# AutonomousVehicleLaboratory/vision_semantic_segmentation

Hardware: AMD Instinct MI355X
Metric: fused frames/sec/GPU (1920x1080 + 120k pts) + max|dlog-odds| vs ref (higher is better)
Workload: dtype f16 hi+lo split, MX-FP4 correction passes, fp32 accumulate

## Files before the change

include/avl_hip.h:

```cpp
#ifndef AVL_HIP_H
#define AVL_HIP_H

#include <stdint.h>

#ifdef __cplusplus
extern "C" {
#endif

#define AVL_OK 0
#define AVL_E_ARG (-1)
#define AVL_E_HIP (-2)
#define AVL_E_UNSUPPORTED (-3)

#define AVL_F32 0
#define AVL_F64 1
#define AVL_BF16 2
#define AVL_F16 3

#define AVL_MAX_MAP_CLASSES 16

const char* avl_version(void);
int avl_last_error(char* buf, int len);


int avl_project_points(const void* pts, int n, int dtype, int64_t point_stride, int64_t comp_stride,
                       const double* P_host, const double* T_host, double range_max,
                       int img_w, int img_h, int32_t* out_ixy, uint8_t* out_mask, void* stream);

int64_t avl_project_pcd_scratch_bytes(int n);

int avl_project_pcd(const void* pts, int n, int dtype, int64_t point_stride, int64_t comp_stride,
                    const double* P_host, const double* T_host, double range_max,
                    const uint8_t* image, int img_w, int img_h,
                    double* out_pcd, uint8_t* out_label, int64_t out_ld, int32_t* out_count,
                    void* scratch, void* stream);


typedef struct avl_grid {
    void* map;
    int map_dtype;
    int Hm, Wm, C;
    double off_x, off_y;
    double b00, b10;
    double resolution;
    uint32_t* cell_mask;
    int32_t* touched;
    int32_t touched_cap;
    int32_t* counter;
    int32_t counter_len;
} avl_grid;
#define AVL_COUNTER_INTS 256

int avl_update_map(const avl_grid* g, const double* pcd, const uint8_t* label, int64_t ld,
                   int m_host, const int32_t* m_dev,
                   const uint8_t* label_colors_host, const double* cm_host, uint32_t bonus_classes,
                   void* stream);

int avl_vote_points(const avl_grid* g, const double* pcd, const uint8_t* label, int64_t ld,
                    int m_host, const int32_t* m_dev, const uint8_t* label_colors_host,
                    uint32_t bonus_classes, void* stream);
int avl_grid_apply(const avl_grid* g, const double* cm_host, void* rows, int rows_dtype, void* stream);


#define AVL_SRC_RGB 0
#define AVL_SRC_CLASSMAP 1

int avl_fused_frame(const avl_grid* g, const void* pts, int n, int dtype, int64_t point_stride,
                    int64_t comp_stride, const double* P_host, const double* T_host, double range_max,
                    int src_kind, const uint8_t* src, int src_w, int src_h, int img_w, int img_h,
                    const uint32_t* lut_host, const uint8_t* label_colors_host,
                    const double* cm_host, uint32_t bonus_classes, void* stream);

int avl_fused_frame_path(const avl_grid* g, int n, uint32_t bonus_classes);


#define AVL_MAX_VIEWS 4
int avl_fused_frame_views(const avl_grid* g, const void* pts, int n, int dtype, int64_t point_stride, int64_t comp_stride,
                          int n_views, const double* P_host , const double* T_host, double range_max,
                          int src_kind, const uint8_t* const* src_host ,
                          int src_w, int src_h, int img_w, int img_h,
                          const uint32_t* lut_host, const uint8_t* label_colors_host,
                          const double* cm_host, uint32_t bonus_classes, void* stream);

int avl_fused_frame_views_path(const avl_grid* g, int n, int n_views, uint32_t bonus_classes);

int avl_colorize_labels(const uint8_t* labels, int lw, int lh, const uint8_t* palette_host,
                        uint8_t* out, int out_w, int out_h, void* stream);


int avl_preprocess_image(const uint8_t* bgr, int h, int w, const double* K_host, const double* dist_host, int factor,
                         uint8_t* rgb_out, void* stream);
int avl_preprocess_image_area(const uint8_t* bgr, int h, int w, const double* K_host, const double* dist_host, int out_h, int out_w,
                              uint8_t* rgb_out, void* stream);

#define AVL_STEM_CAMERA_BYTES 64
int avl_stem_camera_set(void* camera_dev, const double* K_host, const double* dist_host, void* stream);

int avl_pack_semantic_cloud(const double* pcd, const uint8_t* label, int64_t ld, int m_host, const int32_t* m_dev,
                            void* out_records, void* stream);

int avl_planar_update(void* map, int map_dtype, int Hm, int Wm, int C, const uint8_t* image, int img_h, int img_w,
                      const double* Hinv_host, int sep, const uint8_t* label_colors_host, int match_colour, void* stream);

int avl_unpack_pointcloud2(const uint8_t* data, int64_t n_points, int point_step, int off_x, int off_y, int off_z, int off_i,
                           float* out_xyzi, int32_t* n_valid, void* stream);

int avl_render_bev_map(const void* map, int map_dtype, int Hm, int Wm, int C, const uint8_t* colors_host,
                       uint8_t* out, void* stream);
int avl_render_bev_map_thresholds(const void* map, int map_dtype, int Hm, int Wm, int C, const uint8_t* colors_host,
                                  const int32_t* priority_host, const double* thresholds_host, uint8_t* out, void* stream);
int avl_grid_box_filter(const void* src, void* dst, int map_dtype, int Hm, int Wm, int C, void* stream);
int avl_eval_map(const uint8_t* color_map, int H, int W, const uint8_t* mask, int mask_ld, const uint8_t* gt, int gt_ld,
                 uint8_t* labels_out, unsigned long long* counts, void* stream);

int avl_upsample_logits(const float* logits, int h, int w, int K, int64_t ld, float* out, int H, int W, void* stream);
int64_t avl_seg_eval_scratch_bytes(int H, int W);
int avl_seg_eval_full_res(const float* logits, int h, int w, int K, int64_t ld, int H, int W, const uint8_t* gt, int ignore_index,
                          uint8_t* labels_out, unsigned long long* confusion, double* loss_out, unsigned long long* counts_out,
                          void* scratch, void* stream);
int avl_upsample_logits_batch(const float* logits, int n, int64_t image_rows, int h, int w, int K, int64_t ld, float* out, int H, int W,
                              void* stream);
int64_t avl_seg_eval_scratch_bytes_batch(int n, int H, int W);
int avl_seg_eval_full_res_batch(const float* logits, int n, int64_t image_rows, int h, int w, int K, int64_t ld, int H, int W,
                                const uint8_t* gt, int ignore_index, uint8_t* labels_out, unsigned long long* confusion, double* loss_out,
                                unsigned long long* counts_out, double* image_loss_out, unsigned long long* image_counts_out,
                                void* scratch, void* stream);


#define AVL_OP_STEM 1
#define AVL_OP_MAXPOOL 2
#define AVL_OP_GEMM 3
#define AVL_OP_GCONV 4
#define AVL_OP_DWCONV 5
#define AVL_OP_BILINEAR 6
#define AVL_OP_GAP 7
#define AVL_OP_GEMV 8
#define AVL_OP_ARGMAX 9
#define AVL_OP_SUBSAMPLE 10
#define AVL_OP_DWPW 11

#define AVL_OP_BOTTLENECK 12

typedef struct avl_seg_op {
    int32_t kind;
    int32_t dtype;
    const void* in;
    const void* in2;
    void* out;
    const void* weight;
    const float* bias;
    int32_t in_h, in_w, in_c, in_ld, in_rows;
    int32_t out_h, out_w, out_c, out_ld, out_rows;
    int32_t in2_ld;
    int32_t ksize, stride, pad, dil, groups;
    int32_t relu;
    int32_t out_f32;
    int32_t w_rows;
    int32_t w_layout;
    int32_t w_split;
    int32_t mx_flags;
    const void* in_lo;
    const void* in2_lo;
    void* out_lo;
    const void* w_mx;
    const void* in_mx;
    void* out_mx;
    const void* in2_mx;
    const void* in3;
    const void* in3_mx;
    int32_t in3_c, in3_ld;
    int32_t batch;
    int32_t bias_per_image;
    int32_t in_format;
    int32_t raw_batch;
} avl_seg_op;

#define AVL_IN_U8_HWC 0
#define AVL_IN_F32_CHW 1

#define AVL_MX_IN_LO 1
#define AVL_MX_RES_LO 2
#define AVL_MX_OUT_LO 4

typedef struct avl_seg_plan avl_seg_plan;

int avl_seg_plan_create(const avl_seg_op* ops_host, int n_ops, avl_seg_plan** out_plan);
void avl_seg_plan_destroy(avl_seg_plan* plan);
int avl_seg_plan_run(avl_seg_plan* plan, void* stream);
int avl_seg_plan_capture(avl_seg_plan* plan, void* stream);
int avl_seg_plan_profile(avl_seg_plan* plan, void* stream, float* ms_host, double* flops_host, double* bytes_host);
int avl_seg_plan_num_ops(const avl_seg_plan* plan);
int avl_seg_plan_nonfinite(avl_seg_plan* plan, void* stream, unsigned long long* counts_host);

#ifdef __cplusplus
}
#endif
#endif
```

vision_semantic_segmentation_amd/csrc/seg_gemm.hip:

```cpp
#include <cstdlib>
#include <cstring>
#include <type_traits>

#include "seg_types.h"

namespace avl {
namespace {

struct GemmArgs {
    const void* A;
    const void* W;
    const float* bias;
    const void* R;
    void* C;
    int lda, ldr, ldc;
    int M, N, K;
    int relu, out_f32;
    int ntiles;
    int nsub;
    long long a_lo_delta;
    const void* R_lo;
    void* C_lo;
};

template <int NSUB> __device__ __forceinline__ bool sub_needs_a(int j) { return NSUB == 1 || j == 0 || (NSUB == 3 && j == 2); }

__device__ __forceinline__ void glds16(const void* g, void* l) {
    __builtin_amdgcn_global_load_lds((const __attribute__((address_space(1))) void*)g,
                                     (__attribute__((address_space(3))) void*)l, 16, 0, 0);
}

template <typename T, int WM, int WN>
__global__ void __launch_bounds__(WM* WN * 64) k_gemm(GemmArgs p) {
    constexpr int NW = WM * WN, BM = WM * 64, BN = WN * 64;
    constexpr int A_BYTES = BM * 128, W_BYTES = BN * 128, BUF = A_BYTES + W_BYTES;
    constexpr int A_INSTR = BM / 8 / NW, W_INSTR = BN / 8 / NW;
    static_assert(A_INSTR >= 1 && W_INSTR >= 1, "tile too small for the wave count");
    extern __shared__ __attribute__((aligned(16))) char lds[];

    const int tid = threadIdx.x, lane = tid & 63;
    const int wave = __builtin_amdgcn_readfirstlane(tid >> 6);
    const int wm = wave / WN, wn = wave % WN;

    int bid = blockIdx.x;
    {
        const int nwg = gridDim.x, xcd = bid & 7, local = bid >> 3, q = nwg >> 3, r = nwg & 7;
        bid = (xcd < r ? xcd * (q + 1) : r * (q + 1) + (xcd - r) * q) + local;
    }
    const int nt = bid % p.ntiles, mt = bid / p.ntiles;
    const int m0 = mt * BM, n0 = nt * BN;

    const char* a_src[A_INSTR];
    const char* w_src[W_INSTR];
#pragma unroll
    for (int i = 0; i < A_INSTR; ++i) {
        const int r = (i * NW + wave) * 8 + (lane >> 3);
        const int c = (lane & 7) ^ (r & 7);
        a_src[i] = static_cast<const char*>(p.A) + (long long)(m0 + r) * p.lda * (int)sizeof(T) + c * 16;
    }
#pragma unroll
    for (int i = 0; i < W_INSTR; ++i) {
        const int r = (i * NW + wave) * 8 + (lane >> 3);
        const int c = (lane & 7) ^ (r & 7);
        w_src[i] = static_cast<const char*>(p.W) + (long long)(n0 + r) * p.K * p.nsub * (int)sizeof(T) + c * 16;
    }
    auto stage = [&](int buf, int kt) {
        char* base = lds + buf * BUF;
        const int kb = kt / p.nsub, j = kt - kb * p.nsub;
        const long long aoff = (long long)kb * 128 + (j == 2 ? p.a_lo_delta : 0);
#pragma unroll
        for (int i = 0; i < A_INSTR; ++i) glds16(a_src[i] + aoff, base + (i * NW + wave) * 1024);
#pragma unroll
        for (int i = 0; i < W_INSTR; ++i) glds16(w_src[i] + (long long)kt * 128, base + A_BYTES + (i * NW + wave) * 1024);
    };

    const int fr = lane & 15, kq = lane >> 4;
    int a_row[4], w_row[4];
#pragma unroll
    for (int mi = 0; mi < 4; ++mi) a_row[mi] = wm * 64 + mi * 16 + fr;
#pragma unroll
    for (int nj = 0; nj < 4; ++nj) w_row[nj] = wn * 64 + (fr >> 2) * 16 + nj * 4 + (fr & 3);

    f32x4 acc[4][4];
#pragma unroll
    for (int mi = 0; mi < 4; ++mi)
#pragma unroll
        for (int nj = 0; nj < 4; ++nj) acc[mi][nj] = f32x4{0.f, 0.f, 0.f, 0.f};

    const int nk = p.K * (int)sizeof(T) / 128 * p.nsub;
    stage(0, 0);
    int cur = 0;
    for (int kt = 0; kt < nk; ++kt) {
        asm volatile("s_waitcnt vmcnt(0)" ::: "memory");
        __syncthreads();
        if (kt + 1 < nk) stage(cur ^ 1, kt + 1);
        const char* ab = lds + cur * BUF;
        const char* wb = ab + A_BYTES;
        if constexpr (sizeof(T) == 2) {
#pragma unroll
            for (int kk = 0; kk < 2; ++kk) {
                const int chunk = kk * 4 + kq;
                typedef typename Half16<T>::v8 v8;
                v8 af[4], wf[4];
#pragma unroll
                for (int mi = 0; mi < 4; ++mi)
                    af[mi] = *reinterpret_cast<const v8*>(ab + a_row[mi] * 128 + ((chunk ^ (a_row[mi] & 7)) << 4));
#pragma unroll
                for (int nj = 0; nj < 4; ++nj)
                    wf[nj] = *reinterpret_cast<const v8*>(wb + w_row[nj] * 128 + ((chunk ^ (w_row[nj] & 7)) << 4));
#pragma unroll
                for (int mi = 0; mi < 4; ++mi)
#pragma unroll
                    for (int nj = 0; nj < 4; ++nj) acc[mi][nj] = Half16<T>::mfma(wf[nj], af[mi], acc[mi][nj]);
            }
        } else {
            f32x4 af[4][2], wf[4][2];
#pragma unroll
            for (int h = 0; h < 2; ++h) {
                const int chunk = kq * 2 + h;
#pragma unroll
                for (int mi = 0; mi < 4; ++mi)
                    af[mi][h] = *reinterpret_cast<const f32x4*>(ab + a_row[mi] * 128 + ((chunk ^ (a_row[mi] & 7)) << 4));
#pragma unroll
                for (int nj = 0; nj < 4; ++nj)
                    wf[nj][h] = *reinterpret_cast<const f32x4*>(wb + w_row[nj] * 128 + ((chunk ^ (w_row[nj] & 7)) << 4));
            }
#pragma unroll
            for (int s = 0; s < 8; ++s)
#pragma unroll
                for (int mi = 0; mi < 4; ++mi)
#pragma unroll
                    for (int nj = 0; nj < 4; ++nj)
                        acc[mi][nj] = __builtin_amdgcn_mfma_f32_16x16x4f32(wf[nj][s >> 2][s & 3], af[mi][s >> 2][s & 3],
                                                                           acc[mi][nj], 0, 0, 0);
        }
        cur ^= 1;
    }

    const int nbase = n0 + wn * 64 + kq * 16;
    float bias[16];
#pragma unroll
    for (int j = 0; j < 4; ++j) {
        const float4 b = *reinterpret_cast<const float4*>(p.bias + nbase + 4 * j);
        bias[4 * j] = b.x; bias[4 * j + 1] = b.y; bias[4 * j + 2] = b.z; bias[4 * j + 3] = b.w;
    }
    unsigned char* const labels = p.out_f32 ? static_cast<unsigned char*>(p.C_lo) : nullptr;
    if (labels) {
#pragma unroll
        for (int mi = 0; mi < 4; ++mi) {
            const int m = m0 + wm * 64 + mi * 16 + fr;
            float best = acc[mi][0][0] + bias[0];
            int bi = nbase;
#pragma unroll
            for (int i = 1; i < 16; ++i) {
                const float val = acc[mi][i >> 2][i & 3] + bias[i];
                if (nbase + i < p.N && (val > best || (val != val && best == best))) { best = val; bi = nbase + i; }
            }
            const float ob = __shfl_down(best, 16);
            const int oi = __shfl_down(bi, 16);
            if (nbase + 16 < p.N && (ob > best || (ob != ob && best == best))) { best = ob; bi = oi; }
            if (kq == 0 && m < p.M) labels[m] = (unsigned char)bi;
        }
    }
#pragma unroll
    for (int mi = 0; mi < 4; ++mi) {
        const int m = m0 + wm * 64 + mi * 16 + fr;
        if (m >= p.M || nbase >= p.N) continue;
        float v[16];
#pragma unroll
        for (int nj = 0; nj < 4; ++nj)
#pragma unroll
            for (int r = 0; r < 4; ++r) v[nj * 4 + r] = acc[mi][nj][r] + bias[nj * 4 + r];
        const bool full = nbase + 16 <= p.N;
        if (p.R) {
            const T* rp = static_cast<const T*>(p.R) + (long long)m * p.ldr + nbase;
            if (full) {
                float r0[8], r1[8];
                Vec8<T>::load(rp, r0);
                Vec8<T>::load(rp + 8, r1);
#pragma unroll
                for (int i = 0; i < 8; ++i) { v[i] += r0[i]; v[8 + i] += r1[i]; }
            } else {
                for (int i = 0; i < 16; ++i)
                    if (nbase + i < p.N) v[i] += to_f32(rp[i]);
            }
        }
        if (p.relu) {
#pragma unroll
            for (int i = 0; i < 16; ++i) v[i] = fmaxf(v[i], 0.f);
        }
        if (p.out_f32) {
            float* cp = static_cast<float*>(p.C) + (long long)m * p.ldc + nbase;
            for (int i = 0; i < 16; ++i)
                if (nbase + i < p.N) cp[i] = v[i];
        }
        if (!p.out_f32) {
            T* cp = static_cast<T*>(p.C) + (long long)m * p.ldc + nbase;
            if (full) {
                float lo[8], hi[8];
#pragma unroll
                for (int i = 0; i < 8; ++i) { lo[i] = v[i]; hi[i] = v[8 + i]; }
                Vec8<T>::store(cp, lo);
                Vec8<T>::store(cp + 8, hi);
            } else {
                for (int i = 0; i < 16; ++i)
                    if (nbase + i < p.N) cp[i] = from_f32<T>(v[i]);
            }
        }
    }
}

template <typename H, int WM, int WN, int MI, int STAGES, int NSUB = 1, int IO = 0, int AST = STAGES>
__global__ void __launch_bounds__(WM* WN * 64) k_gemm_ring(GemmArgs p, int mtiles) {
    typedef typename Half16<H>::v8 v8;
    constexpr int NW = WM * WN, BM = WM * MI * 16, BN = WN * 64;
    constexpr int A_BYTES = BM * 128, W_BYTES = BN * 128;
    constexpr int W_REGION = AST * A_BYTES;
    static_assert(AST == STAGES || (NSUB == 2 && AST == 2), "activation ring too short for this pass pattern");
    constexpr int A_INSTR = BM / 8 / NW, W_INSTR = BN / 8 / NW;
    extern __shared__ __attribute__((aligned(16))) char lds[];

    const int tid = threadIdx.x, lane = tid & 63;
    const int wave = __builtin_amdgcn_readfirstlane(tid >> 6);
    const int wm = wave / WN, wn = wave % WN;
    const int nwg = gridDim.x;
    int vb;
    {
        const int bid = blockIdx.x, xcd = bid & 7, local = bid >> 3, q = nwg >> 3, r = nwg & 7;
        vb = (xcd < r ? xcd * (q + 1) : r * (q + 1) + (xcd - r) * q) + local;
    }
    const int total = mtiles * p.ntiles;
    const int nkb = p.K / 64;
    const unsigned lds_base = lds_addr(lds);

    const int srow = lane >> 3, schunk = lane & 7;
    const char* a_src[A_INSTR];
    const char* w_src[W_INSTR];
    int pt = vb, pk = 0;
    int issued = 0, issued_a = 0;
    auto set_tile = [&](int t) {
        const int nt = t % p.ntiles, mt = t / p.ntiles;
#pragma unroll
        for (int i = 0; i < A_INSTR; ++i) {
            const int r = (i * NW + wave) * 8 + srow;
            a_src[i] = static_cast<const char*>(p.A) + (long long)(mt * BM + r) * p.lda * 2 + ((schunk ^ (r & 7)) << 4);
        }
#pragma unroll
        for (int i = 0; i < W_INSTR; ++i) {
            const int r = (i * NW + wave) * 8 + srow;
            const int key = ((r >> 1) & 1) | (((r >> 4) & 3) << 1);
            w_src[i] = static_cast<const char*>(p.W) + (long long)(nt * BN + r) * p.K * (2 * NSUB) + ((schunk ^ key) << 4);
        }
    };
    auto issue_part = [&](int h, int np, int jj) {
        const bool na = sub_needs_a<NSUB>(jj);
        if (na) {
            const unsigned abase = lds_base + (issued_a % AST) * A_BYTES + wave * 1024;
            const long long aoff = (long long)pk * 128 + ((NSUB == 3 && jj == 2) ? p.a_lo_delta : 0);
#pragma unroll
            for (int i = 0; i < A_INSTR; ++i)
                if (i * np / A_INSTR == h) glds16_asm(a_src[i] + aoff, abase + i * NW * 1024);
        }
        const unsigned wbase = lds_base + W_REGION + (issued % STAGES) * W_BYTES + wave * 1024;
        const long long woff = (long long)(pk * NSUB + jj) * 128;
#pragma unroll
        for (int i = 0; i < W_INSTR; ++i)
            if (i * np / W_INSTR == h) glds16_asm(w_src[i] + woff, wbase + i * NW * 1024);
        if (h == np - 1) {
            ++issued;
            if (na) ++issued_a;
            if (jj == NSUB - 1) {
                if (++pk == nkb) {
                    pk = 0;
                    pt += nwg;
                    if (pt < total) set_tile(pt);
                }
            }
        }
    };
    if (pt < total) set_tile(pt);
#pragma unroll
    for (int i = 0; i < STAGES - 1; ++i)
        if (pt < total) issue_part(0, 1, i % NSUB);

    const int fr = lane & 15, kq = lane >> 4;
    int a_off[MI], w_off[4], a_key[MI], w_key[4];
#pragma unroll
    for (int mi = 0; mi < MI; ++mi) {
        const int row = wm * (MI * 16) + mi * 16 + fr;
        a_off[mi] = row * 128;
        a_key[mi] = row & 7;
    }
#pragma unroll
    for (int nj = 0; nj < 4; ++nj) {
        const int row = wn * 64 + (fr >> 2) * 16 + nj * 4 + (fr & 3);
        w_off[nj] = W_REGION + row * 128;
        w_key[nj] = ((row >> 1) & 1) | (((row >> 4) & 3) << 1);
    }
    f32x4 acc[MI][4];
    auto init_acc = [&](int t) {
        const int nb = (t % p.ntiles) * BN + wn * 64 + kq * 16;
#pragma unroll
        for (int nj = 0; nj < 4; ++nj) {
            const float4 b = *reinterpret_cast<const float4*>(p.bias + nb + 4 * nj);
#pragma unroll
            for (int mi = 0; mi < MI; ++mi) acc[mi][nj] = f32x4{b.x, b.y, b.z, b.w};
        }
    };
    if (vb < total) init_acc(vb);

    int g = 0;
    int ca = -1;
    for (int t = vb; t < total; t += nwg) {
        const int nt = t % p.ntiles, mt = t / p.ntiles;
        for (int q = 0, j = 0; q < nkb * NSUB; ++q, ++g, j = (NSUB == 1 || j + 1 == NSUB) ? 0 : j + 1) {
            if (sub_needs_a<NSUB>(j)) ++ca;
            const int jn = (j + STAGES - 1) % NSUB;
            if (STAGES >= 3 && issued > g + 1) {
                if (sub_needs_a<NSUB>((j + 1) % NSUB)) asm volatile("s_waitcnt vmcnt(%0)" ::"n"(A_INSTR + W_INSTR) : "memory");
                else asm volatile("s_waitcnt vmcnt(%0)" ::"n"(W_INSTR) : "memory");
            } else asm volatile("s_waitcnt vmcnt(0)" ::: "memory");
            __builtin_amdgcn_s_barrier();
            const bool feed = pt < total;
            const char* abase = lds + (ca % AST) * A_BYTES;
            const char* wbase = lds + (g % STAGES) * W_BYTES;
            auto rd_w = [&](int kk, int nj) { return *reinterpret_cast<const v8*>(wbase + w_off[nj] + (((kk * 4 + kq) ^ w_key[nj]) << 4)); };
            auto rd_a = [&](int kk, int mi) { return *reinterpret_cast<const v8*>(abase + a_off[mi] + (((kk * 4 + kq) ^ a_key[mi]) << 4)); };
            constexpr int HALF = MI / 2;
            const bool early = MI == 8 && NW >= 8 && wave >= NW / 2;
            if (feed && early) { issue_part(0, 2, jn); issue_part(1, 2, jn); }
            v8 wa[4], wb[4], af[MI];
#pragma unroll
            for (int nj = 0; nj < 4; ++nj) wa[nj] = rd_w(0, nj);
#pragma unroll
            for (int mi = 0; mi < MI; ++mi) af[mi] = rd_a(0, mi);
            __builtin_amdgcn_sched_barrier(0);
#pragma unroll
            for (int mi = 0; mi < HALF; ++mi)
#pragma unroll
                for (int nj = 0; nj < 4; ++nj) acc[mi][nj] = Half16<H>::mfma(wa[nj], af[mi], acc[mi][nj]);
            __builtin_amdgcn_sched_barrier(0);
            if (feed && !early) issue_part(0, 2, jn);
#pragma unroll
            for (int nj = 0; nj < 4; ++nj) wb[nj] = rd_w(1, nj);
            __builtin_amdgcn_sched_barrier(0);
#pragma unroll
            for (int mi = HALF; mi < MI; ++mi)
#pragma unroll
                for (int nj = 0; nj < 4; ++nj) acc[mi][nj] = Half16<H>::mfma(wa[nj], af[mi], acc[mi][nj]);
            __builtin_amdgcn_sched_barrier(0);
#pragma unroll
            for (int mi = 0; mi < HALF; ++mi) af[mi] = rd_a(1, mi);
            if (feed && !early) issue_part(1, 2, jn);
            __builtin_amdgcn_sched_barrier(0);
#pragma unroll
            for (int mi = 0; mi < HALF; ++mi)
#pragma unroll
                for (int nj = 0; nj < 4; ++nj) acc[mi][nj] = Half16<H>::mfma(wb[nj], af[mi], acc[mi][nj]);
            __builtin_amdgcn_sched_barrier(0);
#pragma unroll
            for (int mi = HALF; mi < MI; ++mi) af[mi] = rd_a(1, mi);
            __builtin_amdgcn_sched_barrier(0);
#pragma unroll
            for (int mi = HALF; mi < MI; ++mi)
#pragma unroll
                for (int nj = 0; nj < 4; ++nj) acc[mi][nj] = Half16<H>::mfma(wb[nj], af[mi], acc[mi][nj]);
        }
        const int nbase = nt * BN + wn * 64 + kq * 16;
        const bool ncol_ok = nbase + 16 <= p.N;
        constexpr int EB = IO ? 2 : 4;
        const bool rsplit = IO && p.R_lo != nullptr, csplit = IO && p.C_lo != nullptr;
#pragma unroll
        for (int b0 = 0; b0 < MI; b0 += EB) {
            v8 res[EB][2], resl[IO ? EB : 1][2];
            if (p.R) {
#pragma unroll
                for (int e = 0; e < EB; ++e) {
                    const int m = mt * BM + wm * (MI * 16) + (b0 + e) * 16 + fr;
                    if (m < p.M && ncol_ok) {
                        const H* rp = static_cast<const H*>(p.R) + (long long)m * p.ldr + nbase;
                        res[e][0] = *reinterpret_cast<const v8*>(rp);
                        res[e][1] = *reinterpret_cast<const v8*>(rp + 8);
                        if constexpr (IO != 0) {
                            if (rsplit) {
                                const H* rl = static_cast<const H*>(p.R_lo) + (long long)m * p.ldr + nbase;
                                resl[e][0] = *reinterpret_cast<const v8*>(rl);
                                resl[e][1] = *reinterpret_cast<const v8*>(rl + 8);
                            }
                        }
                    }
                }
            }
#pragma unroll
            for (int e = 0; e < EB; ++e) {
                const int mi = b0 + e;
                const int m = mt * BM + wm * (MI * 16) + mi * 16 + fr;
                if (m < p.M && ncol_ok) {
                    float v[16];
#pragma unroll
                    for (int nj = 0; nj < 4; ++nj)
#pragma unroll
                        for (int r = 0; r < 4; ++r) v[nj * 4 + r] = acc[mi][nj][r];
                    if (p.R) {
                        if constexpr (IO != 0) {
                            if (rsplit) {
#pragma unroll
                                for (int i = 0; i < 8; ++i) {
                                    v[i] += (float)res[e][0][i] + (float)resl[e][0][i];
                                    v[8 + i] += (float)res[e][1][i] + (float)resl[e][1][i];
                                }
                            } else {
#pragma unroll
                                for (int i = 0; i < 8; ++i) { v[i] += (float)res[e][0][i]; v[8 + i] += (float)res[e][1][i]; }
                            }
                        } else {
#pragma unroll
                            for (int i = 0; i < 8; ++i) { v[i] += (float)res[e][0][i]; v[8 + i] += (float)res[e][1][i]; }
                        }
                    }
                    if (p.relu) {
#pragma unroll
                        for (int i = 0; i < 16; ++i) v[i] = fmaxf(v[i], 0.f);
                    }
                    H* cp = static_cast<H*>(p.C) + (long long)m * p.ldc + nbase;
                    float lo[8], hi[8];
#pragma unroll
                    for (int i = 0; i < 8; ++i) { lo[i] = v[i]; hi[i] = v[8 + i]; }
                    Vec8<H>::store(cp, lo);
                    Vec8<H>::store(cp + 8, hi);
                    if constexpr (IO != 0) {
                        if (csplit) {
#pragma unroll
                            for (int i = 0; i < 8; ++i) { lo[i] = v[i] - (float)(H)v[i]; hi[i] = v[8 + i] - (float)(H)v[8 + i]; }
                            H* cl = static_cast<H*>(p.C_lo) + (long long)m * p.ldc + nbase;
                            Vec8<H>::store(cl, lo);
                            Vec8<H>::store(cl + 8, hi);
                        }
                    }
                }
            }
        }
        if (t + nwg < total) init_acc(t + nwg);
    }
}

template <typename H, int WM, int WN, int MI, int STAGES, int NSUB = 1, int IO = 0, int AST = STAGES>
int launch_ring(const GemmArgs& a0, int M, hipStream_t s) {
    constexpr int BM = WM * MI * 16, BN = WN * 64, LDS = (AST * BM + STAGES * BN) * 128;
    static_assert(LDS <= 160 * 1024, "ring does not fit LDS");
    AVL_HIP_CHECK(hipFuncSetAttribute(reinterpret_cast<const void*>(&k_gemm_ring<H, WM, WN, MI, STAGES, NSUB, IO, AST>),
                                      hipFuncAttributeMaxDynamicSharedMemorySize, LDS));
    GemmArgs a = a0;
    a.ntiles = (a.N + BN - 1) / BN;
    const int mtiles = (M + BM - 1) / BM;
    const int total = mtiles * a.ntiles;
    const int grid = total < 256 ? total : 256;
    hipLaunchKernelGGL((k_gemm_ring<H, WM, WN, MI, STAGES, NSUB, IO, AST>), dim3(grid), dim3(WM * WN * 64), LDS, s, a, mtiles);
    AVL_LAUNCH_CHECK();
    return AVL_OK;
}

template <typename T, int WM, int WN>
int launch_cfg(const GemmArgs& a, int mtiles, hipStream_t s) {
    constexpr int LDS = 2 * (WM * 64 + WN * 64) * 128;
    AVL_HIP_CHECK(hipFuncSetAttribute(reinterpret_cast<const void*>(&k_gemm<T, WM, WN>),
                                      hipFuncAttributeMaxDynamicSharedMemorySize, LDS));
    hipLaunchKernelGGL((k_gemm<T, WM, WN>), dim3(mtiles * a.ntiles), dim3(WM * WN * 64), LDS, s, a);
    AVL_LAUNCH_CHECK();
    return AVL_OK;
}

struct MxArgs {
    GemmArgs g;
    const char* Aq[2];
    const char* As[2];
    const char* Wq[2];
    const char* Ws[2];
    int ldaq;
    long long a_srows, w_srows;
    char* Cq[2];
    char* Cs[2];
    int ldcq;
    long long c_srows;
    int nmx;
    const char* Rq;
    const char* Rs;
    int ldrq;
    long long r_srows;
    int nmb1;
    const void* A2;
    int lda2, ldaq2;
    const char* Aq2[2];
    const char* As2[2];
    long long a_srows2;
    int stagger;
};

template <int IO, int MI>
__device__ __forceinline__ void mx_epilogue(const MxArgs& q, f32x4 (&acc)[MI][4], int nt, int mt, int wm, int wn, int fr, int kq) {
    typedef f16 H;
    typedef typename Half16<H>::v8 v8;
    constexpr int BM = 2 * MI * 16, BN = 256;
    const GemmArgs& p = q.g;
    const int nbase = nt * BN + wn * 64 + kq * 16;
    const bool ncol_ok = nbase + 16 <= p.N;
    const bool rsplit = p.R_lo != nullptr, csplit = p.C_lo != nullptr;
    const unsigned m0 = (unsigned)(mt * BM + wm * (MI * 16) + fr);
    const unsigned sc_r = (unsigned)(nbase >> 8) * (unsigned)q.r_srows * 8u + (unsigned)((nbase >> 5) & 7);
    const unsigned sc_c = (unsigned)(nbase >> 8) * (unsigned)q.c_srows * 8u + (unsigned)((nbase >> 5) & 7);
    v8 nr0 = {}, nr1 = {};
    uint2 npk = make_uint2(0u, 0u);
    unsigned nsb = 127u;
    auto load_res = [&](int mi) {
        const unsigned m = m0 + mi * 16;
        if (p.R && (int)m < p.M && ncol_ok) {
            const H* rp = static_cast<const H*>(p.R) + (m * (unsigned)p.ldr + (unsigned)nbase);
            nr0 = *reinterpret_cast<const v8*>(rp);
            nr1 = *reinterpret_cast<const v8*>(rp + 8);
            if (q.Rq) {
                npk = *reinterpret_cast<const uint2*>(q.Rq + (m * (unsigned)q.ldrq + (unsigned)(nbase / 2)));
                nsb = (unsigned char)q.Rs[sc_r + m * 8u];
            }
        }
    };
    load_res(0);
#pragma unroll
    for (int mi = 0; mi < MI; ++mi) {
        const unsigned m = m0 + mi * 16;
        const bool live = (int)m < p.M && ncol_ok;
        const v8 r0 = nr0, r1 = nr1;
        const uint2 pk = npk;
        const unsigned sb = nsb;
        if (mi + 1 < MI) load_res(mi + 1);
        float v[16];
#pragma unroll
        for (int nj = 0; nj < 4; ++nj)
#pragma unroll
            for (int r = 0; r < 4; ++r) v[nj * 4 + r] = acc[mi][nj][r];
        if (p.R && live) {
            float rl[16];
#pragma unroll
            for (int i = 0; i < 16; ++i) rl[i] = 0.f;
            if (rsplit) {
                const H* rlp = static_cast<const H*>(p.R_lo) + (m * (unsigned)p.ldr + (unsigned)nbase);
                const v8 l0 = *reinterpret_cast<const v8*>(rlp), l1 = *reinterpret_cast<const v8*>(rlp + 8);
#pragma unroll
                for (int i = 0; i < 8; ++i) { rl[i] = (float)l0[i]; rl[8 + i] = (float)l1[i]; }
            } else if (q.Rq) {
                typedef float v2f __attribute__((ext_vector_type(2)));
                const float sc = __uint_as_float(sb << 23);
#define AVL_FP4_DEC(w, sel, o) { const v2f d = __builtin_amdgcn_cvt_scalef32_pk_f32_fp4(w, sc, sel); rl[o] = d.x; rl[o + 1] = d.y; }
                AVL_FP4_DEC(pk.x, 0, 0) AVL_FP4_DEC(pk.x, 1, 2) AVL_FP4_DEC(pk.x, 2, 4) AVL_FP4_DEC(pk.x, 3, 6)
                AVL_FP4_DEC(pk.y, 0, 8) AVL_FP4_DEC(pk.y, 1, 10) AVL_FP4_DEC(pk.y, 2, 12) AVL_FP4_DEC(pk.y, 3, 14)
#undef AVL_FP4_DEC
            }
#pragma unroll
            for (int i = 0; i < 8; ++i) { v[i] += (float)r0[i] + rl[i]; v[8 + i] += (float)r1[i] + rl[8 + i]; }
        }
        if (p.relu) {
#pragma unroll
            for (int i = 0; i < 16; ++i) v[i] = fmaxf(v[i], 0.f);
        }
        v8 h0, h1;
#pragma unroll
        for (int i = 0; i < 8; ++i) { h0[i] = (H)v[i]; h1[i] = (H)v[8 + i]; }
        float hi[16], lo[16];
#pragma unroll
        for (int i = 0; i < 8; ++i) {
            hi[i] = (float)h0[i];
            hi[8 + i] = (float)h1[i];
            lo[i] = v[i] - hi[i];
            lo[8 + i] = v[8 + i] - hi[8 + i];
        }
        const unsigned coff = m * (unsigned)p.ldc + (unsigned)nbase;
        if (live) {
            H* cp = static_cast<H*>(p.C) + coff;
            *reinterpret_cast<v8*>(cp) = h0;
            *reinterpret_cast<v8*>(cp + 8) = h1;
        }
        if (csplit) {
            v8 l0, l1;
#pragma unroll
            for (int i = 0; i < 8; ++i) { l0[i] = (H)lo[i]; l1[i] = (H)lo[8 + i]; }
            if (live) {
                H* cl = static_cast<H*>(p.C_lo) + coff;
                *reinterpret_cast<v8*>(cl) = l0;
                *reinterpret_cast<v8*>(cl + 8) = l1;
            }
#pragma unroll
            for (int i = 0; i < 8; ++i) { lo[i] = (float)l0[i]; lo[8 + i] = (float)l1[i]; }
        }
        if constexpr (IO != 0) {
#pragma unroll
            for (int pl = 0; pl < 2; ++pl) {
                if (q.Cq[pl] == nullptr) continue;
                unsigned pq[2];
                const unsigned sq = quantize_fp4_block(pl == 0 ? hi : lo, pq);
                if (live) {
                    *reinterpret_cast<uint2*>(q.Cq[pl] + (m * (unsigned)q.ldcq + (unsigned)(nbase / 2))) = make_uint2(pq[0], pq[1]);
                    if ((kq & 1) == 0) q.Cs[pl][sc_c + m * 8u] = (char)sq;
                }
            }
        }
    }
}

template <int IO, int MI>
__global__ void __launch_bounds__(512) k_gemm_ring_mx(MxArgs q, int mtiles) {
    typedef f16 H;
    typedef typename Half16<H>::v8 v8;
    typedef int v8i __attribute__((ext_vector_type(8)));
    constexpr int WM = 2, WN = 4, STAGES = 2;
    constexpr int NW = WM * WN, BM = WM * MI * 16, BN = WN * 64;
    constexpr int A_BYTES = BM * 128, W_BYTES = BN * 128;
    constexpr int W_REGION = STAGES * A_BYTES, S_REGION = W_REGION + STAGES * W_BYTES;
    constexpr int S_BYTES = 4096;
    constexpr int A_INSTR = BM / 8 / NW, W_INSTR = BN / 8 / NW;
    extern __shared__ __attribute__((aligned(16))) char lds[];
    const GemmArgs& p = q.g;

    const int tid = threadIdx.x, lane = tid & 63;
    const int wave = __builtin_amdgcn_readfirstlane(tid >> 6);
    const int wm = wave / WN, wn = wave % WN;
    const int nwg = gridDim.x;
    int vb;
    {
        const int bid = blockIdx.x, xcd = bid & 7, local = bid >> 3, qq = nwg >> 3, r = nwg & 7;
        vb = (xcd < r ? xcd * (qq + 1) : r * (qq + 1) + (xcd - r) * qq) + local;
    }
    const int total = mtiles * p.ntiles;
    const int nmb = p.K / 256;
    const int nsub = 4 + q.nmx;
    const unsigned lds_base = lds_addr(lds);

    const int srow = lane >> 3, schunk = lane & 7;
    const unsigned ct = (unsigned)((schunk ^ srow) << 4);
    const unsigned a_lane16 = (unsigned)srow * (unsigned)(p.lda * 2) + ct, a_laneq = (unsigned)srow * (unsigned)q.ldaq + ct;
    const unsigned a_lane16_2 = (unsigned)srow * (unsigned)(q.lda2 * 2) + ct, a_laneq_2 = (unsigned)srow * (unsigned)q.ldaq2 + ct;
    unsigned w_off16[W_INSTR], w_offq[W_INSTR];
#pragma unroll
    for (int i = 0; i < W_INSTR; ++i) {
        const int r = (i * NW + wave) * 8 + srow;
        const int key = ((r >> 1) & 1) | (((r >> 4) & 3) << 1);
        w_off16[i] = (unsigned)r * (unsigned)(p.K * 2) + ((schunk ^ key) << 4);
        w_offq[i] = (unsigned)r * (unsigned)(p.K / 2) + ((schunk ^ key) << 4);
    }
    int pt = vb, pmb = 0, pj = 0, issued = 0;
    auto issue = [&]() {
        const int nt = pt % p.ntiles, mt = pt / p.ntiles;
        const unsigned abase = lds_base + (issued % STAGES) * A_BYTES + wave * 1024;
        const unsigned wbase = lds_base + W_REGION + (issued % STAGES) * W_BYTES + wave * 1024;
        const bool second = pmb >= q.nmb1;
        const int mbl = second ? pmb - q.nmb1 : pmb;
        if (pj < 4) {
            const long long rowb = second ? (long long)q.lda2 * 2 : (long long)p.lda * 2;
            const char* sa = static_cast<const char*>(second ? q.A2 : p.A) + ((long long)mt * BM + wave * 8) * rowb + (long long)(mbl * 4 + pj) * 128;
            const char* sw = static_cast<const char*>(p.W) + (long long)nt * BN * p.K * 2 + (long long)(pmb * 4 + pj) * 128;
            const unsigned al = second ? a_lane16_2 : a_lane16;
#pragma unroll
            for (int i = 0; i < A_INSTR; ++i) glds16_saddr(sa + (long long)i * (NW * 8) * rowb, al, abase + i * NW * 1024);
#pragma unroll
            for (int i = 0; i < W_INSTR; ++i) glds16_saddr(sw, w_off16[i], wbase + i * NW * 1024);
        } else {
            const int t = pj - 4;
            const long long rowb = second ? q.ldaq2 : q.ldaq;
            const char* sa = (second ? q.Aq2[t] : q.Aq[t]) + ((long long)mt * BM + wave * 8) * rowb + (long long)mbl * 128;
            const char* sw = q.Wq[t] + (long long)nt * BN * (p.K / 2) + (long long)pmb * 128;
            const unsigned al = second ? a_laneq_2 : a_laneq;
#pragma unroll
            for (int i = 0; i < A_INSTR; ++i) glds16_saddr(sa + (long long)i * (NW * 8) * rowb, al, abase + i * NW * 1024);
#pragma unroll
            for (int i = 0; i < W_INSTR; ++i) glds16_saddr(sw, w_offq[i], wbase + i * NW * 1024);
            if (wave < 4 && (wave >= 2 || wave * 128 < BM)) {
                const char* as = second ? q.As2[t] + ((long long)mbl * q.a_srows2 + (long long)mt * BM) * 8
                                        : q.As[t] + ((long long)mbl * q.a_srows + (long long)mt * BM) * 8;
                const char* ss = wave < 2 ? as + wave * 1024
                                          : q.Ws[t] + ((long long)pmb * q.w_srows + (long long)nt * BN) * 8 + (wave - 2) * 1024;
                glds16_saddr(ss, (unsigned)lane * 16u, lds_base + S_REGION + (issued % STAGES) * S_BYTES + wave * 1024);
            }
        }
        ++issued;
        if (++pj == nsub) {
            pj = 0;
            if (++pmb == nmb) { pmb = 0; pt += nwg; }
        }
    };
    if (pt < total) issue();

    const int fr = lane & 15, kq = lane >> 4;
    const int a_row0 = wm * (MI * 16) + fr;
    int w_off[4], w_key[4];
#pragma unroll
    for (int nj = 0; nj < 4; ++nj) {
        const int row = wn * 64 + (fr >> 2) * 16 + nj * 4 + (fr & 3);
        w_off[nj] = W_REGION + row * 128;
        w_key[nj] = ((row >> 1) & 1) | (((row >> 4) & 3) << 1);
    }
    const int a_key = a_row0 & 7;
    f32x4 acc[MI][4];
    auto init_acc = [&](int t) {
        const int nb = (t % p.ntiles) * BN + wn * 64 + kq * 16;
#pragma unroll
        for (int nj = 0; nj < 4; ++nj) {
            const float4 b = *reinterpret_cast<const float4*>(p.bias + nb + 4 * nj);
#pragma unroll
            for (int mi = 0; mi < MI; ++mi) acc[mi][nj] = f32x4{b.x, b.y, b.z, b.w};
        }
    };
    if (vb < total) init_acc(vb);

    int g = 0;
    static_assert(NW == 8, "the DMA stagger assumes waves w and w + 4 on one SIMD");
    const int late = (wave >= 4 || q.stagger == 0) ? 0 : 1;
    for (int t = vb; t < total; t += nwg) {
        const int nt = t % p.ntiles, mt = t / p.ntiles;
        for (int mb = 0; mb < nmb; ++mb) {
            for (int j = 0; j < 4; ++j, ++g) {
                asm volatile("s_waitcnt vmcnt(0)" ::: "memory");
                __builtin_amdgcn_s_barrier();
                const char* abase = lds + (g % STAGES) * A_BYTES + a_row0 * 128;
                const char* wbase = lds + (g % STAGES) * W_BYTES;
#pragma unroll
                for (int kk = 0; kk < 2; ++kk) {
                    if (kk == late && pt < total) issue();
                    v8 wf[4];
#pragma unroll
                    for (int nj = 0; nj < 4; ++nj) wf[nj] = *reinterpret_cast<const v8*>(wbase + w_off[nj] + (((kk * 4 + kq) ^ w_key[nj]) << 4));
                    const int achunk = ((kk * 4 + kq) ^ a_key) << 4;
                    v8 af = *reinterpret_cast<const v8*>(abase + achunk);
#pragma unroll
                    for (int mi = 0; mi < MI; ++mi) {
                        const v8 cur = af;
                        if (mi + 1 < MI) af = *reinterpret_cast<const v8*>(abase + (mi + 1) * 2048 + achunk);
#pragma unroll
                        for (int nj = 0; nj < 4; ++nj) acc[mi][nj] = Half16<H>::mfma(wf[nj], cur, acc[mi][nj]);
                    }
                }
            }
            for (int u = 0; u < q.nmx; ++u, ++g) {
                asm volatile("s_waitcnt vmcnt(0)" ::: "memory");
                __builtin_amdgcn_s_barrier();
                const char* abase = lds + (g % STAGES) * A_BYTES + a_row0 * 128;
                const char* wbase = lds + (g % STAGES) * W_BYTES;
                const char* sbase = lds + (g % STAGES) * S_BYTES + S_REGION;
#pragma unroll
                for (int kk = 0; kk < 2; ++kk) {
                    if (kk == late && pt < total) issue();
                    int4 wf[4];
                    int ws[4];
#pragma unroll
                    for (int nj = 0; nj < 4; ++nj) {
                        wf[nj] = *reinterpret_cast<const int4*>(wbase + w_off[nj] + (((kk * 4 + kq) ^ w_key[nj]) << 4));
                        {
                            const uint2 w8 = *reinterpret_cast<const uint2*>(sbase + 2048 + (wn * 4 + (fr >> 2)) * 128 + ((fr & 3) * 4 + kq) * 8);
                            ws[nj] = (int)(((nj < 2 ? w8.x : w8.y) >> (8 * ((nj & 1) * 2 + kk))) & 0xffu);
                        }
                    }
                    const int achunk = ((kk * 4 + kq) ^ a_key) << 4;
                    int4 af = *reinterpret_cast<const int4*>(abase + achunk);
                    unsigned asw = *reinterpret_cast<const unsigned*>(sbase + a_row0 * 8 + kk * 4);
#pragma unroll
                    for (int mi = 0; mi < MI; ++mi) {
                        const int4 cur = af;
                        const int as = (int)((asw >> (8 * kq)) & 0xffu);
                        if (mi + 1 < MI) {
                            af = *reinterpret_cast<const int4*>(abase + (mi + 1) * 2048 + achunk);
                            asw = *reinterpret_cast<const unsigned*>(sbase + (a_row0 + (mi + 1) * 16) * 8 + kk * 4);
                        }
                        const v8i xa = {cur.x, cur.y, cur.z, cur.w, 0, 0, 0, 0};
#pragma unroll
                        for (int nj = 0; nj < 4; ++nj) {
                            const v8i wa = {wf[nj].x, wf[nj].y, wf[nj].z, wf[nj].w, 0, 0, 0, 0};
                            acc[mi][nj] = __builtin_amdgcn_mfma_scale_f32_16x16x128_f8f6f4(wa, xa, acc[mi][nj], 4, 4, 0, ws[nj], 0, as);
                        }
                    }
                }
            }
        }
        mx_epilogue<IO, MI>(q, acc, nt, mt, wm, wn, fr, kq);
        if (t + nwg < total) init_acc(t + nwg);
    }
}

template <int IO, int MI, int LATE>
__global__ void __launch_bounds__(512) k_gemm_mx_pipe(MxArgs q, int mtiles) {
    typedef f16 H;
    typedef typename Half16<H>::v8 v8;
    typedef int v8i __attribute__((ext_vector_type(8)));
    constexpr int WM = 2, WN = 4, STAGES = 2;
    constexpr int NW = WM * WN, BM = WM * MI * 16, BN = WN * 64;
    constexpr int A_BYTES = BM * 128, W_BYTES = BN * 128;
    constexpr int W_REGION = STAGES * A_BYTES, S_REGION = W_REGION + STAGES * W_BYTES;
    constexpr int S_BYTES = 4096;
    constexpr int A_INSTR = BM / 8 / NW, W_INSTR = BN / 8 / NW;
    constexpr int NS = 2 * MI, D = 3, EV = NS - D;
    constexpr int EW = MI == 8 ? 5 : EV;
    extern __shared__ __attribute__((aligned(16))) char lds[];
    const GemmArgs& p = q.g;

    const int tid = threadIdx.x, lane = tid & 63;
    const int wave = __builtin_amdgcn_readfirstlane(tid >> 6);
    const int wm = wave / WN, wn = wave % WN;
    const int nwg = gridDim.x;
    int vb;
    {
        const int bid = blockIdx.x, xcd = bid & 7, local = bid >> 3, qq = nwg >> 3, r = nwg & 7;
        vb = (xcd < r ? xcd * (qq + 1) : r * (qq + 1) + (xcd - r) * qq) + local;
    }
    const int ntiles = p.ntiles, nmx = q.nmx;
    const int total = mtiles * ntiles;
    const int nmb = p.K / 256;
    const int nsub = 4 + nmx;
    const unsigned lds_base = lds_addr(lds);

    auto lane_now = [&]() __attribute__((always_inline)) {
        unsigned l;
        asm volatile("v_mbcnt_lo_u32_b32 %0, -1, 0\n\tv_mbcnt_hi_u32_b32 %0, -1, %0" : "=v"(l));
        return l;
    };
    int pt = vb, pmb = 0, pj = 0, issued = 0, pmbl = 0;
    long long cur_rowb16 = 0, cur_rowbq = 0, cur_asrows = 0;
    const char *cur_a16 = nullptr, *cur_aq = nullptr, *cur_as = nullptr, *cur_w16 = nullptr, *cur_wq = nullptr, *cur_ws = nullptr;
    long long cur_aps = 0, cur_wps = 0;
    int p_mt = 0;
    auto set_input = [&](bool second) __attribute__((always_inline)) {
        const long long rows0 = (long long)p_mt * BM + wave * 8;
        if (!second) {
            cur_rowb16 = (long long)p.lda * 2; cur_rowbq = q.ldaq; cur_asrows = q.a_srows;
            cur_a16 = static_cast<const char*>(p.A) + rows0 * cur_rowb16;
            cur_aq = q.Aq[0] + rows0 * cur_rowbq;
            cur_as = q.As[0] + (long long)p_mt * BM * 8;
            cur_aps = q.Aq[1] - q.Aq[0];
        } else {
            cur_rowb16 = (long long)q.lda2 * 2; cur_rowbq = q.ldaq2; cur_asrows = q.a_srows2;
            cur_a16 = static_cast<const char*>(q.A2) + rows0 * cur_rowb16;
            cur_aq = q.Aq2[0] + rows0 * cur_rowbq;
            cur_as = q.As2[0] + (long long)p_mt * BM * 8;
            cur_aps = q.Aq2[1] - q.Aq2[0];
        }
        pmbl = 0;
    };
    auto set_tile = [&]() __attribute__((always_inline)) {
        const int nt_ = pt % ntiles;
        p_mt = pt / ntiles;
        cur_w16 = static_cast<const char*>(p.W) + (long long)nt_ * BN * p.K * 2;
        cur_wq = q.Wq[0] + (long long)nt_ * BN * (p.K / 2);
        cur_ws = q.Ws[0] + (long long)nt_ * BN * 8;
        cur_wps = q.Wq[1] - q.Wq[0];
        set_input(false);
    };
    auto issue_w = [&]() __attribute__((always_inline)) {
        const unsigned wbase = lds_base + W_REGION + (issued & 1) * W_BYTES + wave * 1024;
        const unsigned l = lane_now(), srow = l >> 3, cw = ((l & 7u) ^ (((srow >> 1) & 1u) | (((unsigned)(wave >> 1) & 3u) << 1))) << 4;
        const unsigned wr0 = (unsigned)wave * 8u + srow;
        if (pj < 4) {
            const char* sw = cur_w16 + (long long)(pmb * 4 + pj) * 128;
            const unsigned wl = wr0 * (unsigned)(p.K * 2) + cw;
#pragma unroll
            for (int i = 0; i < W_INSTR; ++i)
                glds16_saddr(sw + (long long)i * (NW * 8) * p.K * 2, wl, wbase + i * NW * 1024);
        } else {
            const char* sw = cur_wq + (pj == 4 ? 0 : cur_wps) + (long long)pmb * 128;
            const unsigned wl = wr0 * (unsigned)(p.K / 2) + cw;
#pragma unroll
            for (int i = 0; i < W_INSTR; ++i)
                glds16_saddr(sw + (long long)i * (NW * 8) * (p.K / 2), wl, wbase + i * NW * 1024);
        }
    };
    auto issue_a = [&]() __attribute__((always_inline)) {
        const unsigned abase = lds_base + (issued & 1) * A_BYTES + wave * 1024;
        const unsigned l = lane_now(), srow = l >> 3, ct = ((l & 7u) ^ srow) << 4;
        if (pj < 4) {
            const char* sa = cur_a16 + (long long)(pmbl * 4 + pj) * 128;
            const unsigned al = srow * (unsigned)cur_rowb16 + ct;
#pragma unroll
            for (int i = 0; i < A_INSTR; ++i)
                glds16_saddr(sa + (long long)i * (NW * 8) * cur_rowb16, al, abase + i * NW * 1024);
        } else {
            const long long ta = pj == 4 ? 0 : cur_aps, tw = pj == 4 ? 0 : cur_wps;
            const char* sa = cur_aq + ta + (long long)pmbl * 128;
            const unsigned a_lq = srow * (unsigned)cur_rowbq + ct;
#pragma unroll
            for (int i = 0; i < A_INSTR; ++i)
                glds16_saddr(sa + (long long)i * (NW * 8) * cur_rowbq, a_lq, abase + i * NW * 1024);
            if (wave < 4 && (wave >= 2 || wave * 128 < BM)) {
                const char* ss = wave < 2 ? cur_as + ta + (long long)pmbl * cur_asrows * 8 + wave * 1024
                                          : cur_ws + tw + (long long)pmb * q.w_srows * 8 + (wave - 2) * 1024;
                glds16_saddr(ss, l * 16u, lds_base + S_REGION + (issued & 1) * S_BYTES + wave * 1024);
            }
        }
        ++issued;
        if (++pj == nsub) {
            pj = 0;
            ++pmbl;
            if (++pmb == nmb) {
                pmb = 0;
                pt += nwg;
                if (pt < total) set_tile();
            } else if (pmb == q.nmb1) set_input(true);
        }
    };
    if (pt < total) set_tile();
    static_assert(NW == 8, "the DMA stagger assumes waves w and w + 4 on one SIMD");
    const bool early = wave >= 4 || q.stagger == 0;
    if (pt < total) { issue_w(); issue_a(); }
    if (pt < total) { issue_w(); issue_a(); }

    const int fr = lane & 15, kq = lane >> 4;
    const int a_row0 = wm * (MI * 16) + fr;
    const int wrow0 = wn * 64 + (fr >> 2) * 16 + (fr & 3);
    const int wkey_r = ((wrow0 >> 1) & 1) | (((wrow0 >> 4) & 3) << 1);
    const unsigned a_v0 = (unsigned)(a_row0 * 128 + ((kq ^ (a_row0 & 7)) << 4));
    const unsigned w_v0 = (unsigned)(W_REGION + wrow0 * 128 + ((kq ^ wkey_r) << 4));
    const unsigned sa_v = (unsigned)(S_REGION + a_row0 * 8 + kq);
    const unsigned sw_v = (unsigned)(S_REGION + 2048 + (wn * 4 + (fr >> 2)) * 128 + ((fr & 3) * 4 + kq) * 8);

    f32x4 acc[MI][4];
    auto init_acc = [&](int t) {
        const int nb = (t % ntiles) * BN + wn * 64 + kq * 16;
#pragma unroll
        for (int nj = 0; nj < 4; ++nj) {
            const float4 b = *reinterpret_cast<const float4*>(p.bias + nb + 4 * nj);
#pragma unroll
            for (int mi = 0; mi < MI; ++mi) acc[mi][nj] = f32x4{b.x, b.y, b.z, b.w};
        }
    };
    if (vb < total) init_acc(vb);

    int4 Af[NS], Wf[2][4];
    unsigned As[NS];
    uint2 Wsc = make_uint2(0u, 0u), Wsn = make_uint2(0u, 0u);
    auto rdA = [&](const char* slot, int kk, int mi) { return *reinterpret_cast<const int4*>(slot + (a_v0 ^ (unsigned)(kk * 64)) + mi * 2048); };
    auto rdW = [&](const char* slot, int kk, int nj) { return *reinterpret_cast<const int4*>(slot + (w_v0 ^ (unsigned)(kk * 64)) + nj * 512); };
    auto rdAs = [&](const char* slot, int kk, int mi) { return (unsigned)*reinterpret_cast<const unsigned char*>(slot + sa_v + mi * 128 + kk * 4); };
    auto rdWs = [&](const char* slot) { return *reinterpret_cast<const uint2*>(slot + sw_v); };

    int g = 0;
    bool w_sent = false;
    auto step = [&](auto kind_c, auto s_c, const bool next_q) __attribute__((always_inline)) {
        constexpr int KIND = decltype(kind_c)::value, S = decltype(s_c)::value;
        constexpr int kk = S / MI, mi = S % MI;
        const char* ab = lds + (g & 1) * A_BYTES;
        const char* wb = lds + (g & 1) * W_BYTES;
        const char* sb = lds + (g & 1) * S_BYTES;
        const char* abn = lds + ((g + 1) & 1) * A_BYTES;
        const char* wbn = lds + ((g + 1) & 1) * W_BYTES;
        const char* sbn = lds + ((g + 1) & 1) * S_BYTES;
        auto readA = [&](int t) {
            Af[t] = rdA(ab, t / MI, t % MI);
            if (KIND == 1) As[t] = rdAs(sb, t / MI, t % MI);
        };
        auto readAn = [&](int t) {
            Af[t] = rdA(abn, t / MI, t % MI);
            As[t] = rdAs(sbn, t / MI, t % MI);
        };
        if (EW != EV && S == EW) {
            if (LATE == 0 && !early && g > 0 && pt < total) issue_a();
            if (KIND == 0) asm volatile("s_waitcnt lgkmcnt(1)\n\ts_barrier" ::: "memory");
            else asm volatile("s_waitcnt lgkmcnt(2)\n\ts_barrier" ::: "memory");
            __builtin_amdgcn_sched_barrier(0);
            if (early && pt < total) { issue_w(); w_sent = true; }
        }
        if (EW != EV && LATE != 0 && !early && S == EW + LATE && pt < total) {
            issue_w();
            w_sent = true;
        }
        if (S == EV) {
            if (EW != EV && LATE == 0 && !early && pt < total) {
                issue_w();
                w_sent = true;
            }
            if (EW != EV && w_sent) asm volatile("s_waitcnt vmcnt(%0)\n\ts_waitcnt lgkmcnt(0)\n\ts_barrier" ::"n"(W_INSTR) : "memory");
            else asm volatile("s_waitcnt vmcnt(0)\n\ts_waitcnt lgkmcnt(0)\n\ts_barrier" ::: "memory");
            w_sent = false;
            __builtin_amdgcn_sched_barrier(0);
            if (early && pt < total) { if (EW == EV) issue_w(); issue_a(); }
#pragma unroll
            for (int nj = 0; nj < 4; ++nj) Wf[0][nj] = rdW(wbn, 0, nj);
            Wsn = rdWs(sbn);
            readAn(0);
        }
        if (!early && (EW == EV || LATE != 0) && S == EV + LATE && pt < total) {
            if (EW == EV) issue_w();
            issue_a();
        }
        if (S + D < NS) readA(S + D);
        if (S >= EV && S + 1 < NS) readAn(S - EV + 1);
        if constexpr (MI == 8 && S < 4) Wf[1][S] = rdW(wb, 1, S);
        if constexpr (MI == 4 && S < 2) { Wf[1][2 * S] = rdW(wb, 1, 2 * S); Wf[1][2 * S + 1] = rdW(wb, 1, 2 * S + 1); }
        if (KIND == 0) {
            const v8 af = __builtin_bit_cast(v8, Af[S]);
#pragma unroll
            for (int nj = 0; nj < 4; ++nj) acc[mi][nj] = Half16<H>::mfma(__builtin_bit_cast(v8, Wf[kk][nj]), af, acc[mi][nj]);
        } else {
            const v8i xa = {Af[S].x, Af[S].y, Af[S].z, Af[S].w, 0, 0, 0, 0};
            const int as = (int)As[S];
#define AVL_QMFMA(NJ)                                                                                                              \
    do {                                                                                                                           \
        const v8i wa = {Wf[kk][NJ].x, Wf[kk][NJ].y, Wf[kk][NJ].z, Wf[kk][NJ].w, 0, 0, 0, 0};                                       \
        const int ws = (int)((NJ) < 2 ? Wsc.x : Wsc.y);                                                                            \
        acc[mi][NJ] = __builtin_amdgcn_mfma_scale_f32_16x16x128_f8f6f4(wa, xa, acc[mi][NJ], 4, 4, ((NJ) & 1) * 2 + kk, ws, 0, as);      \
    } while (0)
            AVL_QMFMA(0); AVL_QMFMA(1); AVL_QMFMA(2); AVL_QMFMA(3);
#undef AVL_QMFMA
        }
        __builtin_amdgcn_sched_barrier(0);
    };
    auto substep = [&](auto kind_c, const bool next_q) __attribute__((always_inline)) {
#define AVL_STEP(N) step(kind_c, std::integral_constant<int, N>(), next_q)
        AVL_STEP(0); AVL_STEP(1); AVL_STEP(2); AVL_STEP(3); AVL_STEP(4); AVL_STEP(5); AVL_STEP(6); AVL_STEP(7);
        if constexpr (NS == 16) { AVL_STEP(8); AVL_STEP(9); AVL_STEP(10); AVL_STEP(11); AVL_STEP(12); AVL_STEP(13); AVL_STEP(14); AVL_STEP(15); }
#undef AVL_STEP
        Wsc = Wsn;
        ++g;
    };
    typedef std::integral_constant<int, 0> F16;
    typedef std::integral_constant<int, 1> FP4;

    asm volatile("s_waitcnt vmcnt(0)" ::: "memory");
    __builtin_amdgcn_s_barrier();
    for (int t = vb; t < total; t += nwg) {
        const int nt = t % ntiles, mt = t / ntiles;
        {
            const char* ab = lds + (g & 1) * A_BYTES;
            const char* wb = lds + (g & 1) * W_BYTES;
#pragma unroll
            for (int nj = 0; nj < 4; ++nj) Wf[0][nj] = rdW(wb, 0, nj);
#pragma unroll
            for (int s = 0; s < D; ++s) Af[s] = rdA(ab, 0, s);
        }
        for (int mb = 0; mb < nmb; ++mb) {
            for (int j = 0; j < 4; ++j) substep(F16(), j == 3);
            for (int u = 0; u < nmx; ++u) substep(FP4(), u + 1 < nmx);
        }
        mx_epilogue<IO, MI>(q, acc, nt, mt, wm, wn, fr, kq);
        if (t + nwg < total) init_acc(t + nwg);
    }
}

template <int IO, int MI>
int launch_ring_mx_t(const MxArgs& a0, hipStream_t s) {
    constexpr int BM = 2 * MI * 16, LDS = 2 * (BM + 256) * 128 + 2 * 4096;
    MxArgs a = a0;
    a.stagger = 1;
    a.g.ntiles = a.g.N / 256;
    const int mtiles = (a.g.M + BM - 1) / BM;
    const int total = mtiles * a.g.ntiles;
    const int grid = total < 256 ? total : 256;
    if (a.g.K >= 1024) {
        constexpr int LATE = MI == 8 ? 0 : 1;
        AVL_HIP_CHECK(hipFuncSetAttribute(reinterpret_cast<const void*>(&k_gemm_mx_pipe<IO, MI, LATE>), hipFuncAttributeMaxDynamicSharedMemorySize, LDS));
        hipLaunchKernelGGL((k_gemm_mx_pipe<IO, MI, LATE>), dim3(grid), dim3(512), LDS, s, a, mtiles);
    } else {
        AVL_HIP_CHECK(hipFuncSetAttribute(reinterpret_cast<const void*>(&k_gemm_ring_mx<IO, MI>), hipFuncAttributeMaxDynamicSharedMemorySize, LDS));
        hipLaunchKernelGGL((k_gemm_ring_mx<IO, MI>), dim3(grid), dim3(512), LDS, s, a, mtiles);
    }
    AVL_LAUNCH_CHECK();
    return AVL_OK;
}

int launch_ring_mx(const MxArgs& a, int m_image, bool quantize_out, hipStream_t s) {
    const long long t256 = (long long)((m_image + 255) / 256) * (a.g.N / 256);
    const bool small = t256 < 192 || (t256 > 256 && t256 < 384);
    if (small) return quantize_out ? launch_ring_mx_t<1, 4>(a, s) : launch_ring_mx_t<0, 4>(a, s);
    return quantize_out ? launch_ring_mx_t<1, 8>(a, s) : launch_ring_mx_t<0, 8>(a, s);
}

struct TileCfg { int bm, bn; };
inline TileCfg pick_tile(const avl_seg_op& op);
inline bool ring_eligible(const avl_seg_op& op) {
    const int M = op.out_h * op.out_w * op_batch(op);
    return is_half(op.dtype) && op.w_layout != 1 && op.out_c > 64 && !op.out_f32 && op.out_c % 128 == 0 && op.in_rows >= (M + 255) / 256 * 256;
}
inline TileCfg pick_tile(const avl_seg_op& op) {
    if (op.out_c <= 64) return {256, 64};
    return {128, 128};
}

}

static avl_seg_op gemm_image_op(const avl_seg_op& op, int n) {
    avl_seg_op v = op;
    const long long m = (long long)op.out_h * op.out_w * n;
    const int es = elem_size(op.dtype), oes = op.out_f32 ? 4 : es;
    auto at = [](const void* p, long long bytes) -> const void* { return p ? static_cast<const char*>(p) + bytes : p; };
    v.in = at(op.in, m * op.in_ld * es);
    v.in_lo = at(op.in_lo, m * op.in_ld * es);
    v.in2 = at(op.in2, m * op.in2_ld * es);
    v.in2_lo = at(op.in2_lo, m * op.in2_ld * es);
    v.out = const_cast<void*>(at(op.out, m * op.out_ld * oes));
    v.out_lo = const_cast<void*>(at(op.out_lo, m * op.out_ld * es));
    if (op.out_f32) v.out_mx = const_cast<void*>(at(op.out_mx, m));
    v.bias = op.bias + (long long)n * op.w_rows;
    v.in_rows = (int)(op.in_rows - m);
    v.out_rows = (int)(op.out_rows - m);
    v.batch = 1;
    v.bias_per_image = 0;
    return v;
}

int validate_gemm(const avl_seg_op& op) {
    const int es = elem_size(op.dtype);
    AVL_REQUIRE(is_half(op.dtype) || op.dtype == AVL_F32, "GEMM dtype %d", op.dtype);
    AVL_REQUIRE(op.in && op.out && op.weight && op.bias, "GEMM has NULL buffers");
    AVL_REQUIRE(op.w_layout >= 0 && op.w_layout <= 4, "GEMM w_layout %d (0 = by shape, 1 .. 4 = a forced 16-bit tile configuration)", op.w_layout);
    AVL_REQUIRE(op.w_layout == 0 || is_half(op.dtype), "GEMM w_layout %d forces a tile configuration of the 16-bit kernels: dtype %d", op.w_layout, op.dtype);
    if (op.bias_per_image && op_batch(op) > 1) {
        AVL_REQUIRE(op.w_split != 2 && !op.in3, "GEMM: a per-image bias is not supported by the MX GEMM");
        for (int n = 0; n < op.batch; ++n) {
            const avl_seg_op v = gemm_image_op(op, n);
            AVL_REQUIRE(v.in_rows >= (op.out_h * op.out_w + 255) / 256 * 256,
                        "GEMM with a per-image bias: image %d has %d input rows behind its first (the last image needs whole 256-row tiles)", n, v.in_rows);
            const int rc = validate_gemm(v);
            if (rc) return rc;
        }
        return AVL_OK;
    }
    const int M = op.out_h * op.out_w * op_batch(op), K = op.in_c, N = op.out_c;
    AVL_REQUIRE(M > 0 && N > 0 && K > 0, "GEMM M/N/K = %d/%d/%d", M, N, K);
    AVL_REQUIRE(op.in_h * op.in_w == op.out_h * op.out_w, "GEMM in/out pixel counts differ (%d vs %d)", op.in_h * op.in_w, op.out_h * op.out_w);
    AVL_REQUIRE((K * es) % 128 == 0, "GEMM K = %d is not a multiple of %d", K, 128 / es);
    AVL_REQUIRE(op.in_ld >= K && (op.in_ld * es) % 16 == 0, "GEMM in_ld %d", op.in_ld);
    AVL_REQUIRE(op.out_ld >= N, "GEMM out_ld %d < N %d", op.out_ld, N);
    const TileCfg t = pick_tile(op);
    const int mtiles = (M + t.bm - 1) / t.bm, ntiles = (N + t.bn - 1) / t.bn;
    AVL_REQUIRE(op.in_rows >= mtiles * t.bm, "GEMM reads %d rows, input has %d allocated", mtiles * t.bm, op.in_rows);
    AVL_REQUIRE(op.w_rows >= ntiles * t.bn, "GEMM reads %d weight rows, %d allocated", ntiles * t.bn, op.w_rows);
    AVL_REQUIRE(op.out_rows >= M, "GEMM writes %d rows, output has %d", M, op.out_rows);
    if (!op.out_f32) AVL_REQUIRE((op.out_ld * es) % 16 == 0 && N % 16 == 0, "GEMM out_ld %d / N %d not 16-aligned", op.out_ld, N);
    if (op.in2) AVL_REQUIRE(op.in2_ld >= N && (op.in2_ld * es) % 16 == 0, "GEMM residual ld %d", op.in2_ld);
    if (op.out_f32) AVL_REQUIRE(!op.out_lo, "GEMM: an fp32 output has no low plane");
    if (op.out_f32 && op.out_mx)
        AVL_REQUIRE(N <= 32 && !op.in2 && !op.relu && op.w_split != 2 && t.bn == 64 && !ring_eligible(op),
                    "GEMM: an arg-max output (out_f32 with out_mx = uint8 labels[rows]) needs N <= 32, no residual, no ReLU (N %d)", N);
    if (op.w_split == 2) {
        AVL_REQUIRE(op.dtype == AVL_F16 && op.w_mx && op.in_mx, "MX GEMM needs AVL_F16 activations and the w_mx / in_mx bundles");
        AVL_REQUIRE(K % 256 == 0 && N % 256 == 0 && op.w_rows % 256 == 0 && op.w_rows >= N, "MX GEMM: K %d, N %d, w_rows %d must be multiples of 256", K, N, op.w_rows);
        AVL_REQUIRE(op.in_ld == K && op.in_rows % 256 == 0 && op.in_rows >= M, "MX GEMM input must be dense rows padded to 256 (ld %d, rows %d)", op.in_ld, op.in_rows);
        AVL_REQUIRE(!op.out_f32 && op.out_ld >= N && (op.out_ld * 2) % 16 == 0, "MX GEMM output");
        AVL_REQUIRE(!op.out_mx || op.out_ld == N, "MX GEMM can only quantise a dense output (out_ld %d, N %d)", op.out_ld, N);
        AVL_REQUIRE(!(op.mx_flags & AVL_MX_RES_LO) || (op.in2 && op.in2_mx && !op.in2_lo && op.in2_ld == N),
                    "AVL_MX_RES_LO needs in2, in2_mx (bundle of a dense [out_rows][N] residual) and no in2_lo");
        AVL_REQUIRE(!(op.mx_flags & AVL_MX_OUT_LO) || op.out_mx, "AVL_MX_OUT_LO without out_mx");
        AVL_REQUIRE(!(op.mx_flags & AVL_MX_IN_LO) || !op.in_lo, "AVL_MX_IN_LO together with in_lo");
        if (op.in3) {
            AVL_REQUIRE(op.in3_mx && op.in3_c > 0 && op.in3_c % 256 == 0 && op.in3_ld == op.in3_c,
                        "second GEMM input: in3_mx, in3_c %d (multiple of 256), dense rows (in3_ld %d)", op.in3_c, op.in3_ld);
            AVL_REQUIRE(!op.in_lo || (op.mx_flags & AVL_MX_IN_LO), "a second GEMM input needs both inputs' lo parts in their bundles (AVL_MX_IN_LO) or none");
            AVL_REQUIRE((reinterpret_cast<uintptr_t>(op.in3) | reinterpret_cast<uintptr_t>(op.in3_mx)) % 16 == 0, "second GEMM input must be 16-byte aligned");
        }
        AVL_REQUIRE((long long)op.in_rows * K * 2 < 0xffffff00LL && (long long)op.w_rows * K * 2 < 0xffffff00LL, "MX GEMM operand larger than 4 GB");
        AVL_REQUIRE((long long)op.out_rows * op.out_ld * 2 < (1LL << 31) && (!op.in2 || (long long)op.out_rows * op.in2_ld * 2 < (1LL << 31)) &&
                    (long long)(N / 256 + 1) * op.out_rows * 8 < (1LL << 31), "MX GEMM output / residual plane beyond 2 GB (32-bit epilogue addressing)");
        AVL_REQUIRE((reinterpret_cast<uintptr_t>(op.w_mx) | reinterpret_cast<uintptr_t>(op.in_mx) | reinterpret_cast<uintptr_t>(op.out_mx) |
                     reinterpret_cast<uintptr_t>(op.in_lo) | reinterpret_cast<uintptr_t>(op.in2_lo) | reinterpret_cast<uintptr_t>(op.out_lo)) % 16 == 0,
                    "MX GEMM bundles / low planes must be 16-byte aligned");
    } else if (op.w_split || op.in_lo || op.in2_lo || op.out_lo) {
        AVL_REQUIRE(op.dtype == AVL_F16 && op.w_split == 1, "split (hi + lo) operands need AVL_F16 activations and w_split = 1");
        AVL_REQUIRE(!op.in2_lo || op.in2, "in2_lo without in2");
        AVL_REQUIRE((reinterpret_cast<uintptr_t>(op.in_lo) | reinterpret_cast<uintptr_t>(op.in2_lo) | reinterpret_cast<uintptr_t>(op.out_lo)) % 16 == 0,
                    "GEMM low planes must be 16-byte aligned");
        if (op.in2_lo || op.out_lo)
            AVL_REQUIRE(ring_eligible(op), "split residual / output need the ring GEMM (N %% 128 == 0, 16-bit output, rows padded to 256)");
    }
    AVL_REQUIRE((reinterpret_cast<uintptr_t>(op.in) | reinterpret_cast<uintptr_t>(op.weight) | reinterpret_cast<uintptr_t>(op.out) |
                 reinterpret_cast<uintptr_t>(op.bias) | reinterpret_cast<uintptr_t>(op.in2)) % 16 == 0,
                "GEMM buffers must be 16-byte aligned");
    return AVL_OK;
}

int launch_gemm(const avl_seg_op& op, hipStream_t s) {
    if (op.bias_per_image && op_batch(op) > 1) {
        for (int n = 0; n < op.batch; ++n) {
            const int rc = launch_gemm(gemm_image_op(op, n), s);
            if (rc) return rc;
        }
        return AVL_OK;
    }
    AVL_REQUIRE(op.w_layout != 5, "GEMM w_layout 5 is not supported");
    GemmArgs a;
    a.A = op.in; a.W = op.weight; a.bias = op.bias; a.R = op.in2; a.C = op.out;
    a.lda = op.in_ld; a.ldr = op.in2_ld; a.ldc = op.out_ld;
    a.M = op.out_h * op.out_w * op_batch(op); a.N = op.out_c; a.K = op.in_c;
    a.relu = op.relu; a.out_f32 = op.out_f32;
    const int m_image = op.out_h * op.out_w;
    if (op.w_split == 2) {
        MxArgs mx;
        memset(&mx, 0, sizeof(mx));
        a.nsub = 1;
        a.a_lo_delta = 0;
        a.R_lo = op.in2_lo; a.C_lo = op.out_lo;
        mx.g = a;
        const long long K1 = op.in_c, K2 = op.in3 ? op.in3_c : 0;
        auto abundle = [&](const void* base, long long rows, long long kk, const char** plane, const char** scales) {
            const char* b = static_cast<const char*>(base);
            const long long P = rows * (kk / 2), S = (kk / 256) * rows * 8;
            plane[0] = b; scales[0] = b + P; plane[1] = b + P + S; scales[1] = b + 2 * P + S;
        };
        abundle(op.in_mx, op.in_rows, K1, mx.Aq, mx.As);
        mx.nmb1 = (int)(K1 / 256);
        mx.lda2 = mx.g.lda; mx.ldaq2 = (int)(K1 / 2);
        if (K2) {
            a.K = (int)(K1 + K2);
            mx.g.K = a.K;
            mx.A2 = op.in3; mx.lda2 = op.in3_ld; mx.ldaq2 = (int)(K2 / 2);
            abundle(op.in3_mx, op.in_rows, K2, mx.Aq2, mx.As2);
            mx.a_srows2 = op.in_rows;
        }
        {
            const long long KT = K1 + K2;
            const char* b = static_cast<const char*>(op.w_mx);
            const long long P = (long long)op.w_rows * (KT / 2), S = (KT / 256) * op.w_rows * 8;
            mx.Wq[0] = b; mx.Ws[0] = b + P; mx.Wq[1] = b + P + S; mx.Ws[1] = b + 2 * P + S;
        }
        mx.ldaq = (int)(K1 / 2);
        mx.a_srows = op.in_rows;
        mx.w_srows = op.w_rows;
        mx.nmx = (op.in_lo || (op.mx_flags & AVL_MX_IN_LO)) ? 2 : 1;
        if (op.mx_flags & AVL_MX_RES_LO) {
            const char* b = static_cast<const char*>(op.in2_mx);
            const long long rows = op.out_rows, P = rows * (a.N / 2), S = (long long)(a.N / 256) * rows * 8;
            mx.Rq = b + P + S; mx.Rs = b + 2 * P + S;
            mx.ldrq = a.N / 2;
            mx.r_srows = rows;
        }
        if (op.out_mx) {
            char* b = static_cast<char*>(op.out_mx);
            const long long rows = op.out_rows, P = rows * (a.N / 2), S = (long long)(a.N / 256) * rows * 8;
            mx.Cq[0] = b; mx.Cs[0] = b + P;
            if (op.out_lo || (op.mx_flags & AVL_MX_OUT_LO)) { mx.Cq[1] = b + P + S; mx.Cs[1] = b + 2 * P + S; }
            mx.ldcq = a.N / 2;
            mx.c_srows = rows;
        }
        return launch_ring_mx(mx, m_image, op.out_mx != nullptr, s);
    }
    a.nsub = op.w_split ? (op.in_lo ? 3 : 2) : 1;
    a.a_lo_delta = op.in_lo ? static_cast<const char*>(op.in_lo) - static_cast<const char*>(op.in) : 0;
    a.R_lo = op.in2_lo;
    a.C_lo = op.out_f32 ? op.out_mx : op.out_lo;
    const TileCfg t = pick_tile(op);
    const int mtiles = (a.M + t.bm - 1) / t.bm;
    a.ntiles = (a.N + t.bn - 1) / t.bn;
    if (ring_eligible(op)) {
        const bool can256 = a.N % 256 == 0 && op.w_rows % 256 == 0;
        int v = op.w_layout;
        if (v == 0) v = (can256 && ((m_image + 255) / 256) * (a.N / 256) >= 192) ? 3 : 2;
        if (a.nsub == 2) {
            if (v == 3 && can256) return launch_ring<f16, 2, 4, 8, 3, 2, 1, 2>(a, a.M, s);
            return launch_ring<f16, 4, 2, 4, 3, 2, 1>(a, a.M, s);
        }
        if (a.nsub == 3) {
            if (v == 3 && can256) return launch_ring<f16, 2, 4, 8, 2, 3, 1>(a, a.M, s);
            return launch_ring<f16, 4, 2, 4, 3, 3, 1>(a, a.M, s);
        }
        const bool bf = op.dtype == AVL_BF16;
        if (v == 3 && can256) return bf ? launch_ring<bf16, 2, 4, 8, 2>(a, a.M, s) : launch_ring<f16, 2, 4, 8, 2>(a, a.M, s);
        if (v == 4) return bf ? launch_ring<bf16, 2, 2, 8, 3>(a, a.M, s) : launch_ring<f16, 2, 2, 8, 3>(a, a.M, s);
        return bf ? launch_ring<bf16, 4, 2, 4, 3>(a, a.M, s) : launch_ring<f16, 4, 2, 4, 3>(a, a.M, s);
    }
    if (op.dtype == AVL_BF16) {
        if (t.bn == 64) return launch_cfg<bf16, 4, 1>(a, mtiles, s);
        return launch_cfg<bf16, 2, 2>(a, mtiles, s);
    }
    if (op.dtype == AVL_F16) {
        if (t.bn == 64) return launch_cfg<f16, 4, 1>(a, mtiles, s);
        return launch_cfg<f16, 2, 2>(a, mtiles, s);
    }
    if (t.bn == 64) return launch_cfg<float, 4, 1>(a, mtiles, s);
    return launch_cfg<float, 2, 2>(a, mtiles, s);
}

}
```

vision_semantic_segmentation_amd/csrc/seg_plan.hip:

```cpp
#include <vector>

#include "seg_types.h"

struct avl_seg_plan {
    std::vector<avl_seg_op> ops;
    std::vector<hipEvent_t> ev;
    hipGraph_t graph = nullptr;
    hipGraphExec_t exec = nullptr;
};

namespace avl {
namespace {

int validate(const avl_seg_op& op, int index) {
    int rc;
    if (op.batch < 0) rc = set_error(AVL_E_ARG, "batch %d (0 or 1 = one image)", op.batch);
    else if (op.bias_per_image && op.kind != AVL_OP_GEMM) rc = set_error(AVL_E_ARG, "bias_per_image is a GEMM field");
    else if (op.in_format != AVL_IN_U8_HWC && op.in_format != AVL_IN_F32_CHW) rc = set_error(AVL_E_ARG, "in_format %d is not an AVL_IN_* value", op.in_format);
    else if (op.in_format != AVL_IN_U8_HWC && op.kind != AVL_OP_STEM) rc = set_error(AVL_E_ARG, "in_format %d is a stem field (other ops leave it 0)", op.in_format);
    else if (op.in_format == AVL_IN_F32_CHW && op.in2)
        rc = set_error(AVL_E_UNSUPPORTED, op.raw_batch ? "in_format AVL_IN_F32_CHW with raw_batch = 1: a batch of raw frames is uint8 [batch][src_h][src_w][3]"
                                                       : "in_format AVL_IN_F32_CHW with a pre-processing stem (in2 set): that stem reads the raw uint8 frame");
    else if (op.raw_batch != 0 && op.raw_batch != 1) rc = set_error(AVL_E_ARG, "raw_batch %d (0 = one raw frame, 1 = every image of the batch is a raw frame)", op.raw_batch);
    else if (op.raw_batch && op.kind != AVL_OP_STEM) rc = set_error(AVL_E_ARG, "raw_batch is a stem field (other ops leave it 0)");
    else if (op.raw_batch && !op.in2) rc = set_error(AVL_E_ARG, "raw_batch needs a pre-processing stem: in2 (the camera blocks) is NULL");
    else if (op.kind == AVL_OP_GEMM) rc = validate_gemm(op);
    else if (op.kind == AVL_OP_DWPW) rc = validate_dwpw(op);
    else if (op.kind == AVL_OP_BOTTLENECK) rc = validate_bottleneck(op);
    else rc = validate_conv_op(op);
    if (rc != AVL_OK) {
        char msg[400];
        snprintf(msg, sizeof(msg), "%s", err_buf());
        return set_error(rc, "op %d (kind %d): %s", index, op.kind, msg);
    }
    return AVL_OK;
}

int launch(const avl_seg_op& op, hipStream_t s) {
    if (op.kind == AVL_OP_GEMM) return launch_gemm(op, s);
    if (op.kind == AVL_OP_DWPW) return launch_dwpw(op, s);
    if (op.kind == AVL_OP_BOTTLENECK) return launch_bottleneck(op, s);
    return launch_conv_op(op, s);
}

static double act_bytes(double es, bool lo_plane, bool mx, bool mx_lo) {
    double b = es + (lo_plane ? es : 0.0);
    if (mx) b += (mx_lo ? 2.0 : 1.0) * (0.5 + 1.0 / 32.0);
    return b;
}

void work(const avl_seg_op& op, double& flops, double& bytes) {
    const double es = elem_size(op.dtype), nb = op_batch(op);
    const double in_pix = (double)op.in_h * op.in_w * nb, out_pix = (double)op.out_h * op.out_w * nb;
    const double e_in = act_bytes(es, op.in_lo != nullptr, op.in_mx != nullptr, (op.mx_flags & AVL_MX_IN_LO) || op.in_lo);
    const double e_out = act_bytes(es, op.out_lo != nullptr, op.out_mx != nullptr, (op.mx_flags & AVL_MX_OUT_LO) || op.out_lo);
    flops = 0;
    bytes = in_pix * op.in_c * e_in + out_pix * op.out_c * e_out;
    switch (op.kind) {
        case AVL_OP_STEM:
            flops = 2.0 * out_pix * 64 * 147;
            bytes = (op.in2 ? (double)op.in_rows : in_pix) * (op.in_format == AVL_IN_F32_CHW ? 12 : 3) + out_pix * 64 * es;
            break;
        case AVL_OP_GEMM:
            flops = 2.0 * out_pix * op.out_c * (op.in_c + (op.in3 ? op.in3_c : 0));
            {
                const double k_all = op.in_c + (op.in3 ? op.in3_c : 0);
                const double e_w = op.w_split == 2 ? es + 2.0 * (0.5 + 1.0 / 32.0) : es * (op.w_split ? 2.0 : 1.0);
                const double e_res = act_bytes(es, op.in2_lo != nullptr, (op.mx_flags & AVL_MX_RES_LO) != 0, false);
                bytes += (double)op.out_c * k_all * e_w + (op.in2 ? out_pix * op.out_c * e_res : 0.0) + (op.in3 ? in_pix * op.in3_c * e_in : 0.0);
            }
            if (op.out_f32) {
                bytes += out_pix * op.out_c * (4 - es);
                if (op.out_mx) bytes += out_pix - out_pix * op.out_c * (0.5 + 1.0 / 32.0);
            }
            break;
        case AVL_OP_GCONV:
            flops = 2.0 * out_pix * op.out_c * (op.in_c / op.groups) * 9;
            bytes += (double)op.out_c * (op.in_c / op.groups) * 9 * es * (op.w_split ? 2.0 : 1.0);
            break;
        case AVL_OP_DWCONV:
            flops = 2.0 * out_pix * op.out_c * op.ksize * op.ksize;
            break;
        case AVL_OP_DWPW:
            flops = 2.0 * out_pix * op.in_c * 9 + 2.0 * out_pix * op.out_c * op.in_c;
            bytes += (double)op.out_c * op.in_c * es;
            if (op.out_f32) {
                flops += 2.0 * out_pix * op.out_c * op.in3_c;
                bytes += out_pix * (op.in3_c * 4.0 + 1.0) - out_pix * op.out_c * e_out;
            }
            break;
        case AVL_OP_BILINEAR:
            flops = 8.0 * out_pix * op.out_c;
            break;
        case AVL_OP_BOTTLENECK: {
            const double width = op.in3_c, cg = width / op.groups;
            const double macs = op.in_c * width + width * cg * 9 + width * op.out_c + (op.w_layout ? (double)op.in_c * op.out_c : 0.0);
            flops = 2.0 * out_pix * macs;
            bytes += 2.0 * es * macs;
            break;
        }
        case AVL_OP_GAP:
            flops = in_pix * op.in_c;
            bytes = in_pix * op.in_c * es;
            break;
        case AVL_OP_GEMV:
            flops = 2.0 * op.in_c * op.out_c * nb;
            bytes = 4.0 * op.in_c * op.out_c + 4.0 * (op.in_c + op.out_c) * nb;
            break;
        case AVL_OP_ARGMAX:
            bytes = in_pix * op.in_c * 4 + in_pix;
            break;
        default:
            break;
    }
}

}
}

extern "C" int avl_seg_plan_create(const avl_seg_op* ops_host, int n_ops, avl_seg_plan** out_plan) {
    AVL_REQUIRE(ops_host && n_ops > 0 && out_plan, "avl_seg_plan_create: bad arguments");
    for (int i = 0; i < n_ops; ++i) {
        int rc = avl::validate(ops_host[i], i);
        if (rc) return rc;
    }
    avl_seg_plan* p = new avl_seg_plan();
    p->ops.assign(ops_host, ops_host + n_ops);
    *out_plan = p;
    return AVL_OK;
}

extern "C" void avl_seg_plan_destroy(avl_seg_plan* plan) {
    if (!plan) return;
    if (plan->exec) (void)hipGraphExecDestroy(plan->exec);
    if (plan->graph) (void)hipGraphDestroy(plan->graph);
    for (hipEvent_t e : plan->ev) (void)hipEventDestroy(e);
    delete plan;
}

extern "C" int avl_seg_plan_num_ops(const avl_seg_plan* plan) { return plan ? (int)plan->ops.size() : 0; }

extern "C" int avl_seg_plan_capture(avl_seg_plan* plan, void* stream) {
    AVL_REQUIRE(plan && stream, "avl_seg_plan_capture needs a plan and a non-NULL stream");
    hipStream_t s = avl::as_stream(stream);
    if (plan->exec) { (void)hipGraphExecDestroy(plan->exec); plan->exec = nullptr; }
    if (plan->graph) { (void)hipGraphDestroy(plan->graph); plan->graph = nullptr; }
    AVL_HIP_CHECK(hipStreamBeginCapture(s, hipStreamCaptureModeThreadLocal));
    int rc = AVL_OK;
    for (const avl_seg_op& op : plan->ops) {
        rc = avl::launch(op, s);
        if (rc) break;
    }
    hipGraph_t g = nullptr;
    hipError_t e = hipStreamEndCapture(s, &g);
    if (rc) { if (g) (void)hipGraphDestroy(g); return rc; }
    if (e != hipSuccess) return avl::set_error(AVL_E_HIP, "hipStreamEndCapture failed: %s", hipGetErrorString(e));
    plan->graph = g;
    AVL_HIP_CHECK(hipGraphInstantiate(&plan->exec, plan->graph, nullptr, nullptr, 0));
    return AVL_OK;
}

extern "C" int avl_seg_plan_run(avl_seg_plan* plan, void* stream) {
    AVL_REQUIRE(plan, "plan is NULL");
    hipStream_t s = avl::as_stream(stream);
    if (plan->exec) {
        AVL_HIP_CHECK(hipGraphLaunch(plan->exec, s));
        return AVL_OK;
    }
    for (const avl_seg_op& op : plan->ops) {
        int rc = avl::launch(op, s);
        if (rc) return rc;
    }
    return AVL_OK;
}

extern "C" int avl_seg_plan_profile(avl_seg_plan* plan, void* stream, float* ms_host, double* flops_host, double* bytes_host) {
    AVL_REQUIRE(plan && ms_host, "avl_seg_plan_profile: bad arguments");
    hipStream_t s = avl::as_stream(stream);
    const size_t n = plan->ops.size();
    while (plan->ev.size() < 2 * n) {
        hipEvent_t e;
        AVL_HIP_CHECK(hipEventCreate(&e));
        plan->ev.push_back(e);
    }
    for (size_t i = 0; i < n; ++i) {
        AVL_HIP_CHECK(hipEventRecord(plan->ev[2 * i], s));
        int rc = avl::launch(plan->ops[i], s);
        if (rc) return rc;
        AVL_HIP_CHECK(hipEventRecord(plan->ev[2 * i + 1], s));
    }
    AVL_HIP_CHECK(hipStreamSynchronize(s));
    for (size_t i = 0; i < n; ++i) {
        AVL_HIP_CHECK(hipEventElapsedTime(&ms_host[i], plan->ev[2 * i], plan->ev[2 * i + 1]));
        double f, b;
        avl::work(plan->ops[i], f, b);
        if (flops_host) flops_host[i] = f;
        if (bytes_host) bytes_host[i] = b;
    }
    return AVL_OK;
}

namespace avl {
namespace {
template <typename T>
__global__ void k_count_nonfinite(const T* x, long long rows, int cols, int ld, unsigned long long* counter) {
    const long long n = rows * cols;
    unsigned long long bad = 0;
    for (long long i = (long long)blockIdx.x * blockDim.x + threadIdx.x; i < n; i += (long long)gridDim.x * blockDim.x) {
        const float v = (float)x[(i / cols) * ld + (i % cols)];
        bad += (__builtin_isfinite(v) ? 0u : 1u);
    }
    for (int o = 32; o > 0; o >>= 1) bad += __shfl_down(bad, o, 64);
    if ((threadIdx.x & 63) == 0 && bad) atomicAdd(counter, bad);
}
template <typename T>
void count_plane(const void* ptr, long long rows, int cols, int ld, unsigned long long* counter, hipStream_t s) {
    if (!ptr || rows <= 0 || cols <= 0) return;
    hipLaunchKernelGGL((k_count_nonfinite<T>), dim3(512), dim3(256), 0, s, static_cast<const T*>(ptr), rows, cols, ld, counter);
}
}
}

extern "C" int avl_seg_plan_nonfinite(avl_seg_plan* plan, void* stream, unsigned long long* counts_host) {
    AVL_REQUIRE(plan && counts_host, "avl_seg_plan_nonfinite: bad arguments");
    hipStream_t s = avl::as_stream(stream);
    hipStreamCaptureStatus cap = hipStreamCaptureStatusNone;
    AVL_HIP_CHECK(hipStreamIsCapturing(s, &cap));
    AVL_REQUIRE(cap == hipStreamCaptureStatusNone, "avl_seg_plan_nonfinite synchronises the stream: not while it is being captured");
    const size_t n = plan->ops.size();
    unsigned long long* dev = nullptr;
    AVL_HIP_CHECK(hipMalloc(reinterpret_cast<void**>(&dev), n * sizeof(unsigned long long)));
    int rc = AVL_OK;
    hipError_t e = hipMemsetAsync(dev, 0, n * sizeof(unsigned long long), s);
    for (size_t i = 0; i < n && rc == AVL_OK && e == hipSuccess; ++i) {
        const avl_seg_op& op = plan->ops[i];
        rc = avl::launch(op, s);
        if (rc) break;
        if (op.kind == AVL_OP_ARGMAX) continue;
        const long long rows = (op.kind == AVL_OP_GAP || op.kind == AVL_OP_GEMV) ? avl::op_batch(op) : (long long)op.out_h * op.out_w * avl::op_batch(op);
        const bool f32 = op.dtype == AVL_F32 || op.out_f32 || op.kind == AVL_OP_GAP || op.kind == AVL_OP_GEMV;
        if (f32) avl::count_plane<float>(op.out, rows, (op.kind == AVL_OP_DWPW && op.out_f32) ? op.in3_c : op.out_c, op.out_ld, dev + i, s);
        else if (op.dtype == AVL_F16) {
            avl::count_plane<avl::f16>(op.out, rows, op.out_c, op.out_ld, dev + i, s);
            avl::count_plane<avl::f16>(op.out_lo, rows, op.out_c, op.out_ld, dev + i, s);
        } else avl::count_plane<avl::bf16>(op.out, rows, op.out_c, op.out_ld, dev + i, s);
        e = hipGetLastError();
    }
    if (rc == AVL_OK && e == hipSuccess) e = hipMemcpyAsync(counts_host, dev, n * sizeof(unsigned long long), hipMemcpyDeviceToHost, s);
    if (rc == AVL_OK && e == hipSuccess) e = hipStreamSynchronize(s);
    (void)hipFree(dev);
    if (rc) return rc;
    if (e != hipSuccess) return avl::set_error(AVL_E_HIP, "avl_seg_plan_nonfinite: %s", hipGetErrorString(e));
    return AVL_OK;
}

namespace avl {
int launch_preprocess(const unsigned char*, int, int, const double*, const double*, int, unsigned char*, hipStream_t);
int launch_set_camera(void*, const double*, const double*, hipStream_t);
int launch_preprocess_area(const unsigned char*, int, int, const double*, const double*, int, int, unsigned char*, hipStream_t);
}
extern "C" int avl_preprocess_image_area(const uint8_t* bgr, int h, int w, const double* K_host, const double* dist_host, int out_h, int out_w,
                                         uint8_t* rgb_out, void* stream) {
    AVL_REQUIRE(bgr && rgb_out && h > 0 && w > 0, "bad image buffers");
    AVL_REQUIRE(out_h > 0 && out_w > 0 && out_h <= h && out_w <= w, "INTER_AREA shrinks: output %d x %d from %d x %d", out_h, out_w, h, w);
    AVL_REQUIRE((K_host == nullptr) == (dist_host == nullptr), "K_host and dist_host go together");
    return avl::launch_preprocess_area(bgr, h, w, K_host, dist_host, out_h, out_w, rgb_out, avl::as_stream(stream));
}
extern "C" int avl_stem_camera_set(void* camera_dev, const double* K_host, const double* dist_host, void* stream) {
    AVL_REQUIRE(camera_dev && reinterpret_cast<uintptr_t>(camera_dev) % 4 == 0, "bad camera block");
    AVL_REQUIRE((K_host == nullptr) == (dist_host == nullptr), "K_host and dist_host go together");
    return avl::launch_set_camera(camera_dev, K_host, dist_host, avl::as_stream(stream));
}
extern "C" int avl_preprocess_image(const uint8_t* bgr, int h, int w, const double* K_host, const double* dist_host, int factor,
                                    uint8_t* rgb_out, void* stream) {
    AVL_REQUIRE(bgr && rgb_out && h > 0 && w > 0, "bad image buffers");
    AVL_REQUIRE(factor >= 1 && h / factor > 0 && w / factor > 0, "downscale factor %d", factor);
    AVL_REQUIRE((K_host == nullptr) == (dist_host == nullptr), "K_host and dist_host go together");
    return avl::launch_preprocess(bgr, h, w, K_host, dist_host, factor, rgb_out, avl::as_stream(stream));
}
```

vision_semantic_segmentation_amd/network.py:

```python
import collections
import ctypes as C
import hashlib
import math

import numpy as np
import torch

from . import _lib

BN_EPS = 1e-5

OP_STEM, OP_MAXPOOL, OP_GEMM, OP_GCONV, OP_DWCONV, OP_BILINEAR, OP_GAP, OP_GEMV, OP_ARGMAX, OP_SUBSAMPLE, OP_DWPW, OP_BOTTLENECK = range(1, 13)
OP_NAMES = {1: "stem", 2: "maxpool", 3: "gemm", 4: "gconv", 5: "dwconv", 6: "bilinear", 7: "gap", 8: "gemv", 9: "argmax", 10: "subsample", 11: "dwpw",
            12: "bottleneck"}


class AvlSegOp(C.Structure):
    _fields_ = [
        ("kind", C.c_int32), ("dtype", C.c_int32),
        ("in_", C.c_void_p), ("in2", C.c_void_p), ("out", C.c_void_p), ("weight", C.c_void_p), ("bias", C.c_void_p),
        ("in_h", C.c_int32), ("in_w", C.c_int32), ("in_c", C.c_int32), ("in_ld", C.c_int32), ("in_rows", C.c_int32),
        ("out_h", C.c_int32), ("out_w", C.c_int32), ("out_c", C.c_int32), ("out_ld", C.c_int32), ("out_rows", C.c_int32),
        ("in2_ld", C.c_int32),
        ("ksize", C.c_int32), ("stride", C.c_int32), ("pad", C.c_int32), ("dil", C.c_int32), ("groups", C.c_int32),
        ("relu", C.c_int32), ("out_f32", C.c_int32), ("w_rows", C.c_int32), ("w_layout", C.c_int32), ("w_split", C.c_int32), ("mx_flags", C.c_int32),
        ("in_lo", C.c_void_p), ("in2_lo", C.c_void_p), ("out_lo", C.c_void_p),
        ("w_mx", C.c_void_p), ("in_mx", C.c_void_p), ("out_mx", C.c_void_p), ("in2_mx", C.c_void_p),
        ("in3", C.c_void_p), ("in3_mx", C.c_void_p), ("in3_c", C.c_int32), ("in3_ld", C.c_int32),
        ("batch", C.c_int32), ("bias_per_image", C.c_int32),
        ("in_format", C.c_int32),
        ("raw_batch", C.c_int32),
    ]


AVL_IN_U8_HWC, AVL_IN_F32_CHW = 0, 1
INPUT_FORMATS = {"u8_hwc": AVL_IN_U8_HWC, "f32_nchw": AVL_IN_F32_CHW}


AVL_MX_IN_LO, AVL_MX_RES_LO, AVL_MX_OUT_LO = 1, 2, 4


_vp, _i = C.c_void_p, C.c_int
_lib._register_seg({
    "avl_seg_plan_create": (_i, [C.POINTER(AvlSegOp), _i, C.POINTER(C.c_void_p)]),
    "avl_seg_plan_destroy": (None, [_vp]),
    "avl_seg_plan_run": (_i, [_vp, _vp]),
    "avl_seg_plan_capture": (_i, [_vp, _vp]),
    "avl_seg_plan_profile": (_i, [_vp, _vp, _vp, _vp, _vp]),
    "avl_seg_plan_num_ops": (_i, [_vp]),
    "avl_seg_plan_nonfinite": (_i, [_vp, _vp, _vp]),
})


PLANES = (64, 128, 256, 512)
EXPANSION = 4
BACKBONES = {
    "resnet50": ((3, 4, 6, 3), 1, 64),
    "resnet101": ((3, 4, 23, 3), 1, 64),
    "resnet152": ((3, 8, 36, 3), 1, 64),
    "resnext50_32x4d": ((3, 4, 6, 3), 32, 4),
    "resnext101_32x8d": ((3, 4, 23, 3), 32, 8),
    "wide_resnet50_2": ((3, 4, 6, 3), 1, 128),
    "wide_resnet101_2": ((3, 4, 23, 3), 1, 128),
}
DEFAULT_BACKBONE = "resnext50_32x4d"
UNBUILDABLE_BACKBONES = ("ResNet", "resnet18", "resnet34")
LAYERS, GROUPS, WIDTH_PER_GROUP = BACKBONES[DEFAULT_BACKBONE]


def backbone_arch(name):
    if name in BACKBONES:
        return BACKBONES[name]
    if name in UNBUILDABLE_BACKBONES:
        raise NotImplementedError("MODEL.BACKBONE %r is a BasicBlock ResNet: the reference's MyResNet (backbone/resnet.py:17-18) "
                                  "hard-codes 2048 output and 256 low-level channels, so it cannot build either; supported: %s"
                                  % (name, ", ".join(sorted(BACKBONES))))
    raise NotImplementedError("MODEL.BACKBONE %r is not supported; supported: %s" % (name, ", ".join(sorted(BACKBONES))))


REFINE_KERNEL_SIZES = (1, 2, 3, 4, 5, 6, 7)


def refine_kernel_sizes(refine_kernel_size, refine_channels):
    n = len(refine_channels)
    if refine_kernel_size is None:
        return (3,) * n
    ks = tuple(int(k) for k in refine_kernel_size)
    if len(ks) != n:
        if all(k == 3 for k in ks):
            return (3,) * n
        raise ValueError("MODEL.DECODER.REFINE_KERNEL_SIZE %s has %d entries, REFINE_CHANNELS %d: one kernel size per refine block "
                         "(decoder.py:20)" % (list(ks), len(ks), n))
    bad = [k for k in ks if k not in REFINE_KERNEL_SIZES]
    if bad:
        raise ValueError("MODEL.DECODER.REFINE_KERNEL_SIZE %s: depthwise kernels are built for sizes %s" % (list(ks), ", ".join(map(str, REFINE_KERNEL_SIZES))))
    return ks


def _bn_keys(prefix, c):
    return [(prefix + ".weight", (c,)), (prefix + ".bias", (c,)), (prefix + ".running_mean", (c,)),
            (prefix + ".running_var", (c,))]


def state_spec(num_classes=19, in_channels=3, aspp_out=256, atrous_channels=(256, 256, 256, 256), low_level_out=256,
               refine_channels=(256, 256), backbone=DEFAULT_BACKBONE, refine_kernel_size=None):
    refine_kernel_size = refine_kernel_sizes(refine_kernel_size, refine_channels)
    layers, groups, wpg = backbone_arch(backbone)
    spec = [("backbone.conv1.weight", (64, in_channels, 7, 7))] + _bn_keys("backbone.bn1", 64)
    inplanes = 64
    for li, (planes, nblocks) in enumerate(zip(PLANES, layers), start=1):
        width = int(planes * (wpg / 64.0)) * groups
        for b in range(nblocks):
            p = "backbone.layer%d.%d" % (li, b)
            spec += [(p + ".conv1.weight", (width, inplanes, 1, 1))] + _bn_keys(p + ".bn1", width)
            spec += [(p + ".conv2.weight", (width, width // groups, 3, 3))] + _bn_keys(p + ".bn2", width)
            spec += [(p + ".conv3.weight", (planes * EXPANSION, width, 1, 1))] + _bn_keys(p + ".bn3", planes * EXPANSION)
            if b == 0:
                spec += [(p + ".downsample.0.weight", (planes * EXPANSION, inplanes, 1, 1))] + _bn_keys(p + ".downsample.1", planes * EXPANSION)
            inplanes = planes * EXPANSION
    feat, low = inplanes, PLANES[0] * EXPANSION
    spec += [("aspp.module_pyramid.0.conv.weight", (atrous_channels[0], feat, 1, 1))] + _bn_keys("aspp.module_pyramid.0.bn", atrous_channels[0])
    for i in range(1, len(atrous_channels)):
        p = "aspp.module_pyramid.%d" % i
        spec += [(p + ".depthwise_cnn.conv.weight", (feat, 1, 3, 3))] + _bn_keys(p + ".depthwise_cnn.bn", feat)
        spec += [(p + ".pointwise_cnn.conv.weight", (atrous_channels[i], feat, 1, 1))] + _bn_keys(p + ".pointwise_cnn.bn", atrous_channels[i])
    spec += [("aspp.global_avg_pool.1.conv.weight", (256, feat, 1, 1))] + _bn_keys("aspp.global_avg_pool.1.bn", 256)
    spec += [("aspp.conv.conv.weight", (aspp_out, sum(atrous_channels) + 256, 1, 1))] + _bn_keys("aspp.conv.bn", aspp_out)
    spec += [("decoder.low_level_conv.conv.weight", (low_level_out, low, 1, 1))] + _bn_keys("decoder.low_level_conv.bn", low_level_out)
    cin = low_level_out + aspp_out
    for i, rc in enumerate(refine_channels):
        p = "decoder.refine_layers.%d" % i
        k = refine_kernel_size[i]
        spec += [(p + ".depthwise_cnn.conv.weight", (cin, 1, k, k))] + _bn_keys(p + ".depthwise_cnn.bn", cin)
        spec += [(p + ".pointwise_cnn.conv.weight", (rc, cin, 1, 1))] + _bn_keys(p + ".pointwise_cnn.bn", rc)
        cin = rc
    p = "decoder.refine_layers.%d" % len(refine_channels)
    spec += [(p + ".conv.weight", (num_classes, cin, 1, 1)), (p + ".conv.bias", (num_classes,))]
    return spec


def random_state_dict(seed=0, **kw):
    g = torch.Generator().manual_seed(seed)
    backbone = kw.get("backbone", DEFAULT_BACKBONE)
    depth = sum(backbone_arch(backbone)[0])
    st = {}
    for key, shape in state_spec(**kw):
        if key.endswith("running_var"):
            t = torch.rand(shape, generator=g) * 0.5 + 0.75
        elif key.endswith("running_mean"):
            t = torch.randn(shape, generator=g) * 0.1
        elif key.endswith(".weight") and len(shape) == 1:
            t = torch.rand(shape, generator=g) * 0.4 + 0.8
            if ".bn3." in key or "downsample.1" in key:
                t = t * 0.6
                if backbone != DEFAULT_BACKBONE and depth > 16 and ".bn3." in key:
                    t = t * math.sqrt(16.0 / depth)
        elif key.endswith(".bias"):
            t = torch.randn(shape, generator=g) * 0.05
        else:
            fan_in = shape[1] * shape[2] * shape[3]
            t = torch.randn(shape, generator=g) * math.sqrt(2.0 / fan_in)
        st[key] = t.to(torch.float32)
    return st


def load_checkpoint(path):
    ckpt = torch.load(path, map_location="cpu", weights_only=True)
    state = ckpt["model"] if isinstance(ckpt, dict) and "model" in ckpt else ckpt
    return {(k[7:] if k.startswith("module.") else k): v.to(torch.float32) for k, v in state.items()
            if not k.endswith("num_batches_tracked")}


def check_state_dict(state, **kw):
    missing = [k for k, s in state_spec(**kw) if k not in state or tuple(state[k].shape) != tuple(s)]
    if missing:
        raise KeyError("state dict lacks / mis-shapes %d tensors, e.g. %s" % (len(missing), missing[:3]))
    bad = [k for k, _ in state_spec(**kw) if not bool(torch.isfinite(state[k]).all())]
    if bad:
        raise ValueError("state dict holds Inf / NaN in %d tensors, e.g. %s" % (len(bad), bad[:3]))



def fold_bn(state, conv_key, bn_prefix):
    w = state[conv_key].to(torch.float64)
    if bn_prefix is None:
        b = state.get(conv_key[:-6] + "bias")
        return w, (b.to(torch.float64) if b is not None else torch.zeros(w.shape[0], dtype=torch.float64))
    s = state[bn_prefix + ".weight"].to(torch.float64) / torch.sqrt(state[bn_prefix + ".running_var"].to(torch.float64) + BN_EPS)
    b = state[bn_prefix + ".bias"].to(torch.float64) - state[bn_prefix + ".running_mean"].to(torch.float64) * s
    return w * s.view(-1, 1, 1, 1), b


def pack_stem_mfma(w):
    out = torch.zeros((4, 6, 16, 32), dtype=torch.float64)
    for nj in range(4):
        for i in range(16):
            n = (i >> 2) * 16 + nj * 4 + (i & 3)
            for st in range(6):
                for k in range(32):
                    q, j = st * 4 + k // 8, k % 8
                    t = (q % 3) * 8 + j
                    if q < 21 and t < 21:
                        out[nj, st, i, k] = w[n, t % 3, q // 3, t // 3]
    return out.reshape(-1)


def pack_gconv_windows(w, groups):
    C_ = w.shape[0]
    cg = C_ // groups
    nwin = C_ // 32
    dense = torch.zeros((nwin, 32, 9, 32), dtype=torch.float64)
    wt = w.reshape(C_, cg, 9)
    co = torch.arange(C_)
    win, col = co // 32, co % 32
    gbase = (col // cg) * cg
    for ci in range(cg):
        dense[win, col, :, gbase + ci] = wt[co, ci, :]
    i = torch.arange(16)
    out = torch.empty((nwin, 2, 9, 16, 32), dtype=torch.float64)
    for nj in range(2):
        rows = (i >> 2) * 8 + nj * 4 + (i & 3)
        out[:, nj] = dense[:, rows].permute(0, 2, 1, 3)
    return out.reshape(-1)


def gconv_dense_windows(w, groups):
    C_ = w.shape[0]
    cg = C_ // groups
    nwin = C_ // 32
    dense = torch.zeros((nwin, 32, 9, 32), dtype=torch.float64)
    wt = w.reshape(C_, cg, 9).to(torch.float64)
    co = torch.arange(C_)
    win, col = co // 32, co % 32
    gbase = (col // cg) * cg
    for ci in range(cg):
        dense[win, col, :, gbase + ci] = wt[co, ci, :]
    return dense


def pack_gconv_mx(w, groups):
    whi, wlo = split_f16(w)
    nwin = w.shape[0] // 32
    frag_hi = pack_gconv_windows(whi.to(torch.float64), groups).to(torch.float16)
    i = torch.arange(16)
    w4 = torch.zeros((nwin, 2, 2, 3, 64, 16), dtype=torch.uint8)
    w4s = torch.zeros((nwin, 64, 12), dtype=torch.uint8)
    for pair, part in ((0, wlo), (1, whi)):
        dense = gconv_dense_windows(part.to(torch.float64), groups)
        for nj in range(2):
            rows = (i >> 2) * 8 + nj * 4 + (i & 3)
            d = torch.zeros((nwin, 16, 12, 32), dtype=torch.float64)
            d[:, :, :9] = dense[:, rows]
            codes, sbyte = fp4_quant_blocks(d.reshape(nwin, 16, 3, 4, 32))
            w4[:, nj, pair] = codes.permute(0, 2, 3, 1, 4).reshape(nwin, 3, 64, 16)
            sb = sbyte.permute(0, 3, 1, 2).reshape(nwin, 64, 3).to(torch.uint8)
            w4s[:, :, nj * 6 + pair * 3:nj * 6 + pair * 3 + 3] = sb
    return frag_hi, torch.cat([w4.reshape(-1), w4s.reshape(-1)])


def pack_conv3x3(w, groups, elem=8, split=False):
    C_, cg = w.shape[0], w.shape[1]
    assert C_ == cg * groups and cg % 64 == 0 and elem in (4, 8)
    ck = 8 * elem
    i, kq, h, e = torch.arange(16), torch.arange(4), torch.arange(2), torch.arange(elem)
    rows = torch.stack([(i >> 2) * 8 + nj * 4 + (i & 3) for nj in range(2)])
    rows = (torch.arange(cg // 32).view(-1, 1, 1) * 32 + rows).reshape(-1)
    cols = ((4 * h.view(2, 1, 1) + kq.view(1, 4, 1)) * elem + e.view(1, 1, elem))
    cols = (torch.arange(cg // ck).view(-1, 1, 1, 1) * ck + cols).reshape(-1)
    parts = list(split_f16(w)) if split else [w.to(torch.float64)]
    out = []
    for part in parts:
        wt = part.reshape(groups, cg, cg, 9).permute(0, 3, 1, 2)
        m = wt[:, :, rows][:, :, :, cols]
        m = m.reshape(groups, 9, cg // 32, 2, 16, cg // ck, 2, 4, elem)
        out.append(m.permute(0, 5, 1, 2, 3, 6, 7, 4, 8))
    return torch.stack(out, dim=5).reshape(-1).contiguous()


def pack_dw_f32(w, b):
    c = w.shape[0]
    assert c % 64 == 0
    out = torch.empty((c // 64, 8, 10, 8), dtype=torch.float32)
    out[:, :, 0:9, :] = w.reshape(c // 64, 8, 8, 9).permute(0, 1, 3, 2).to(torch.float32)
    out[:, :, 9, :] = b.to(torch.float32).reshape(c // 64, 8, 8)
    return out.view(torch.int32).reshape(-1)


def pack_dw_pairs(w, b, act_dtype):
    c = w.shape[0]
    assert c % 64 == 0
    w9 = w.reshape(c, 9).to(torch.float32)
    w16 = torch.cat([w9, torch.zeros((c, 1), dtype=torch.float32)], dim=1).to(act_dtype)
    bits = w16.view(torch.int16).to(torch.int32) & 0xFFFF
    pairs = bits[:, 0::2] | (bits[:, 1::2] << 16)
    bias_bits = b.to(torch.float32).view(torch.int32)
    out = torch.empty((c // 64, 8, 6, 8), dtype=torch.int32)
    pc = pairs.reshape(c // 64, 8, 8, 5)
    out[:, :, :5, :] = pc.permute(0, 1, 3, 2)
    out[:, :, 5, :] = bias_bits.reshape(c // 64, 8, 8)
    return out.reshape(-1)


def dwpw_tile_order(h, w, dilation, tile=128):
    n = (h * w + tile - 1) // tile
    period = dilation * w
    keys = sorted(range(n), key=lambda t: ((tile * t + tile // 2) % period, t))
    return torch.tensor(keys, dtype=torch.int32)


def dwpw_block_order(h, w, band=4):
    ty, tx = (h + 7) // 8, (w + 15) // 16
    order = [r * tx + c for b in range(0, ty, band) for c in range(tx) for r in range(b, min(b + band, ty))]
    return torch.tensor(order, dtype=torch.int32)


def _round_up(x, m):
    return (x + m - 1) // m * m


def split_f16(w):
    hi = w.to(torch.float16)
    lo = (w - hi.to(torch.float64)).to(torch.float16)
    return hi, lo


def pack_split_rows(w, nsub):
    rows, k = w.shape
    assert k % 64 == 0 and nsub in (2, 3)
    hi, lo = split_f16(w)
    parts = [hi.reshape(rows, k // 64, 1, 64), lo.reshape(rows, k // 64, 1, 64)]
    if nsub == 3:
        parts.append(parts[0])
    return torch.cat(parts, dim=2).reshape(rows, k * nsub).contiguous()


def _mfma_a_fragments(m):
    rows, k = m.shape
    return m.reshape(rows // 16, 16, k // 32, 4, 8).permute(0, 2, 3, 1, 4).reshape(rows // 16, k // 32, 64, 8)


def pack_bottleneck(w1, w2, w3, wd, groups):
    width, cin = w1.shape
    cout = w3.shape[0]
    cg = width // groups
    assert width % 16 == 0 and cin % 32 == 0 and cout in (256, 512) and 16 % cg == 0

    def pair(m):
        hi, lo = split_f16(m)
        return torch.stack([_mfma_a_fragments(hi), _mfma_a_fragments(lo)], dim=2)

    p1 = pair(w1.to(torch.float64))
    nwin = width // 16
    dense = torch.zeros((nwin, 16, 10, 16), dtype=torch.float64)
    wt = w2.reshape(width, cg, 9).to(torch.float64)
    co = torch.arange(width)
    win, col = co // 16, co % 16
    gbase = (col // cg) * cg
    for ci in range(cg):
        dense[win, col, :9, gbase + ci] = wt[co, ci, :]
    p2 = pair(dense.reshape(nwin * 16, 160))
    w3k = w3.to(torch.float64) if wd is None else torch.cat([w3.to(torch.float64), wd.to(torch.float64)], dim=1)
    i = torch.arange(16)
    nj_ = cout // 128
    rows = torch.cat([16 * nj_ * wv + (i >> 2) * 4 * nj_ + nj * 4 + (i & 3) for wv in range(8) for nj in range(nj_)])
    p3 = pair(w3k[rows])
    ks3 = w3k.shape[1] // 32
    p3 = p3.reshape(8, nj_, ks3, 2, 64, 8).permute(0, 2, 1, 3, 4, 5)
    return p1.reshape(-1).contiguous(), p2.reshape(-1).contiguous(), p3.reshape(-1).contiguous()


_FP4_GRID = torch.tensor([0.0, 0.5, 1.0, 1.5, 2.0, 3.0, 4.0, 6.0], dtype=torch.float64)


def fp4_quant_blocks(b):
    b = b.to(torch.float64)
    amax = b.abs().amax(dim=-1)
    e = (torch.floor(torch.log2(amax.clamp_min(2.0 ** -200))).to(torch.int64) + 127).clamp_min(0)
    sbyte = torch.where(e >= 3, e - 2, torch.ones_like(e))
    mant = amax.to(torch.float32).view(torch.int32).to(torch.int64) & 0x7FFFFF
    sbyte = (sbyte + (mant > 0x500000).to(torch.int64)).clamp(1, 254)
    scale = torch.exp2((sbyte - 127).to(torch.float64)).unsqueeze(-1)
    mag = (b.abs() / scale).clamp_max(6.0)
    mid = (_FP4_GRID[1:] + _FP4_GRID[:-1]) / 2
    code = torch.bucketize(mag, mid, right=False)
    tie = mag == mid[code.clamp(0, 6)]
    code = torch.where(tie & (code % 2 == 1), code + 1, code)
    code = code.clamp(0, 7) | ((b < 0).to(torch.int64) << 3)
    code = code.reshape(*code.shape[:-1], 16, 2)
    return (code[..., 0] | (code[..., 1] << 4)).to(torch.uint8), sbyte


def mx_quant_fp4(w):
    rows, k = w.shape
    assert k % 256 == 0
    packed, sbyte = fp4_quant_blocks(w.reshape(rows, k // 32, 32))
    scales = sbyte.reshape(rows, k // 256, 8).permute(1, 0, 2).contiguous().to(torch.uint8)
    return packed.reshape(rows, k // 2), scales


def mx_dequant_fp4(packed, scales):
    rows, k2 = packed.shape
    p = packed.to(torch.int64)
    code = torch.stack([p & 15, p >> 4], dim=2).reshape(rows, k2 * 2)
    val = _FP4_GRID[code & 7] * torch.where((code & 8) != 0, -1.0, 1.0)
    sc = scales.permute(1, 0, 2).reshape(rows, -1).to(torch.float64)
    return (val.reshape(rows, -1, 32) * torch.exp2(sc - 127).unsqueeze(2)).reshape(rows, k2 * 2)


def mx_bundle_bytes(rows, c):
    return rows * (c // 2) + (c // 256) * rows * 8


def permute_w_scales(scales):
    nb, rows, _ = scales.shape
    assert rows % 16 == 0
    s = scales.reshape(nb, rows // 16, 4, 4, 2, 4)
    return s.permute(0, 1, 3, 5, 2, 4).contiguous().reshape(nb, rows, 8)


def pack_mx_weights(w):
    hi, lo = split_f16(w)
    ql, sl = mx_quant_fp4(lo.to(torch.float64))
    qh, sh = mx_quant_fp4(hi.to(torch.float64))
    return hi, torch.cat([ql.reshape(-1), permute_w_scales(sl).reshape(-1), qh.reshape(-1), permute_w_scales(sh).reshape(-1)])


_PACK_CACHE = {}
_PACK_CACHE_BYTES = [0]
PACK_CACHE_LIMIT = 3 << 30


def state_digest(state):
    h = hashlib.blake2b(digest_size=16)
    for k in sorted(state):
        t = state[k]
        if torch.is_tensor(t) and t.is_floating_point():
            h.update(("%s %s %s;" % (k, t.dtype, tuple(t.shape))).encode())
            h.update(t.detach().cpu().contiguous().reshape(-1).view(torch.uint8).numpy())
    return h.hexdigest()


def _cached_pack(key, fn):
    hit = _PACK_CACHE.get(key)
    if hit is not None:
        return hit
    out = fn()
    ts = out if isinstance(out, (tuple, list)) else (out,)
    nbytes = sum(t.numel() * t.element_size() for t in ts if torch.is_tensor(t))
    if _PACK_CACHE_BYTES[0] + nbytes > PACK_CACHE_LIMIT:
        _PACK_CACHE.clear()
        _PACK_CACHE_BYTES[0] = 0
    _PACK_CACHE[key] = out
    _PACK_CACHE_BYTES[0] += nbytes
    return out


class Act(object):
    __slots__ = ("hi", "lo", "pool_key", "mx", "mx_valid", "lo_fp4")

    def __init__(self, hi, lo=None, pool_key=None, mx=None):
        self.hi, self.lo, self.pool_key = hi, lo, pool_key
        self.mx = mx
        self.mx_valid = False
        self.lo_fp4 = False

    @property
    def shape(self):
        return self.hi.shape

    def mx_ready(self, ch):
        return self.mx is not None and self.mx_valid and self.hi.shape[1] == ch


def _zero_pad(t, n, dim=0):
    shape = list(t.shape)
    shape[dim] = n - shape[dim]
    return torch.cat([t.to(torch.float64), torch.zeros(shape, dtype=torch.float64)], dim=dim)


Block = collections.namedtuple("Block", "p hw ohw cin width cout s d has_ds trunk_lo")


class SegNet(object):

    ROW_PAD = 256
    MIXED_OPTS = ("conv1_split", "conv2_split", "mx", "trunk_fp4", "fuse_ds", "gconv_mx", "dw_exact", "layer1_lo", "fuse_block", "full_split", "fuse_decoder", "fuse_classifier")

    def __init__(self, state, height, width, precision="bf16", device=None, num_classes=19, output_stride=8, fuse_dwpw=True, raw_frame=None,
                 part=None, backbone=DEFAULT_BACKBONE, batch=1, input_format="u8_hwc", raw_batch=False, **mixed_opts):
        if input_format not in INPUT_FORMATS:
            raise ValueError("SegNet: input_format %r (known: %s)" % (input_format, ", ".join(INPUT_FORMATS)))
        if input_format != "u8_hwc" and (raw_frame is not None or part is not None):
            raise NotImplementedError("SegNet: input_format %r is the network input itself; a raw_frame plan (pre-processing stem) or a "
                                      "sub-plan (part) takes no such input" % input_format)
        self.input_format = input_format
        batch = int(batch)
        if batch < 1:
            raise ValueError("SegNet: batch %d < 1" % batch)
        self.raw_batch = bool(raw_batch)
        if self.raw_batch and raw_frame is None:
            raise ValueError("SegNet: raw_batch=True asks for a batch of raw camera frames and needs raw_frame=(src_h, src_w)")
        if self.raw_batch and (part is not None or input_format != "u8_hwc"):
            raise NotImplementedError("SegNet: raw_batch=True takes uint8 camera frames through the whole network; not with part=%r or "
                                      "input_format %r" % (part, input_format))
        if batch > 1 and raw_frame is not None and not self.raw_batch:
            raise NotImplementedError("SegNet: a raw_frame plan (pre-processing stem) takes one camera frame unless raw_batch=True; "
                                      "batch %d" % batch)
        if batch > 1 and part is not None:
            raise NotImplementedError("SegNet: sub-plans (part=%r) take one image; batch %d" % (part, batch))
        self.batch = batch
        assert output_stride in (8, 16), "deeplab_v3_plus.py:30-36 / backbone/build.py:11-16 know output strides 8 (the reference configuration, base_cfg.py:106) and 16"
        self.output_stride = int(output_stride)
        self.backbone = backbone
        self.layers, self.groups, self.width_per_group = backbone_arch(backbone)
        assert precision in ("bf16", "f16", "f32", "mixed")
        self.device = torch.device("cuda", torch.cuda.current_device()) if device is None else torch.device(device)
        self.H, self.W = int(height), int(width)
        self.raw_frame = None if raw_frame is None else (int(raw_frame[0]), int(raw_frame[1]))
        if self.raw_frame is not None:
            f = self.raw_frame[1] // self.W
            if f < 1 or (self.raw_frame[0] // f, self.raw_frame[1] // f) != (self.H, self.W):
                raise ValueError("raw_frame %r does not scale to %dx%d by an integer factor" % (self.raw_frame, self.H, self.W))
        self.precision = precision
        self.mixed = precision == "mixed"
        unknown = sorted(set(mixed_opts) - set(self.MIXED_OPTS))
        if unknown:
            raise TypeError("SegNet: unknown mixed-mode option(s) %s (known: %s)" % (unknown, ", ".join(self.MIXED_OPTS)))
        self.mixed_conv1_split = self.mixed and mixed_opts.get("conv1_split", True)
        self.mixed_conv2_split = self.mixed and mixed_opts.get("conv2_split", True)
        self.mixed_mx = self.mixed and mixed_opts.get("mx", True)
        self.mixed_trunk_fp4 = mixed_opts.get("trunk_fp4", True)
        self.mixed_fuse_ds = mixed_opts.get("fuse_ds", True)
        self.mixed_fuse_classifier = mixed_opts.get("fuse_classifier", True)
        self.mixed_fuse_decoder = mixed_opts.get("fuse_decoder", True)
        self.mixed_dw_exact = mixed_opts.get("dw_exact", True)
        self.mixed_layer1_lo = mixed_opts.get("layer1_lo", True)
        self.mixed_fuse_block = self.mixed and mixed_opts.get("fuse_block", True)
        self.full_split = self.mixed and bool(mixed_opts.get("full_split", False))
        if self.full_split:
            self.mixed_mx = False
            self.mixed_trunk_fp4 = False
            self.mixed_layer1_lo = True
            self.mixed_fuse_block = False
        self.mixed_gconv_mx = mixed_opts.get("gconv_mx", True) and not self.full_split
        self.act_dtype = {"bf16": torch.bfloat16, "f16": torch.float16, "f32": torch.float32, "mixed": torch.float16}[precision]
        self.avl_dtype = {"bf16": _lib.AVL_BF16, "f16": _lib.AVL_F16, "f32": _lib.AVL_F32, "mixed": _lib.AVL_F16}[precision]
        self.half = precision != "f32"
        self.fuse_dwpw = bool(fuse_dwpw)
        self.num_classes = num_classes
        self._keep = []
        self._free = {}
        self.ops = []
        self.op_names = []
        self._plan = C.c_void_p()
        self._fp = state_digest(state)
        self.part = part
        if part is None:
            self._check_decoder_size(state)
            self._build(state)
        else:
            self._build_part(state)
        arr = (AvlSegOp * len(self.ops))(*self.ops)
        _lib.check(_lib.lib().avl_seg_plan_create(arr, len(self.ops), C.byref(self._plan)), "avl_seg_plan_create")

    def __del__(self):
        try:
            if self._plan:
                _lib.lib().avl_seg_plan_destroy(self._plan)
        except Exception:
            pass

    def _check_decoder_size(self, state):
        shrink, i = 0, 0
        while ("decoder.refine_layers.%d.depthwise_cnn.conv.weight" % i) in state:
            shrink += state["decoder.refine_layers.%d.depthwise_cnn.conv.weight" % i].shape[-1] - 1
            i += 1
        low = lambda n: ((n + 6 - 7) // 2 + 1 + 2 - 3) // 2 + 1
        if min(low(self.H), low(self.W)) - shrink >= 1:
            return
        need = 1
        while low(need) - shrink < 1:
            need += 1
        raise ValueError("SegNet: a %dx%d input is too small for the decoder: its low-level map is %dx%d and the refine blocks' depthwise "
                         "convs take %d pixels off each side; the smallest input that works is %dx%d"
                         % (self.H, self.W, low(self.H), low(self.W), shrink, max(need, self.H), max(need, self.W)))

    def _act(self, rows, ch, split=False, mx=False, lo_fp4=False):
        prow = _round_up(rows * self.batch, self.ROW_PAD) + (self.ROW_PAD if self.batch > 1 else 0)
        mx = bool(mx and self.mixed_mx and ch % 256 == 0)
        lo_fp4 = bool(lo_fp4 and mx)
        split = bool(split and not lo_fp4)
        key = (prow, ch, bool(split), mx, lo_fp4)
        if self._free.get(key):
            a = self._free[key].pop()
            a.mx_valid = False
            return a
        if split:
            t = torch.zeros((2, prow, ch), dtype=self.act_dtype, device=self.device)
            a = Act(t[0], t[1], key)
        else:
            t = torch.zeros((prow, ch), dtype=self.act_dtype, device=self.device)
            a = Act(t, None, key)
        self._keep.append(t)
        if mx:
            a.mx = torch.zeros(2 * mx_bundle_bytes(prow, ch), dtype=torch.uint8, device=self.device)
            self._keep.append(a.mx)
        a.lo_fp4 = lo_fp4
        return a

    def _release(self, a):
        self._free.setdefault(a.pool_key, []).append(a)

    def _dev(self, t, dtype):
        t = t.to(dtype).contiguous().to(self.device)
        self._keep.append(t)
        return t

    def _op(self, name, kind, **f):
        op = AvlSegOp()
        op.kind = kind
        op.dtype = self.avl_dtype
        op.batch = self.batch
        for k, v in f.items():
            setattr(op, k, v)
        self.ops.append(op)
        self.op_names.append(name)

    @staticmethod
    def _view(t, col=0):
        t = t.hi if isinstance(t, Act) else t
        return t.data_ptr() + col * t.element_size(), t.shape[1], t.shape[0]

    @staticmethod
    def _lo(a, col=0):
        return 0 if (not isinstance(a, Act) or a.lo is None) else a.lo.data_ptr() + col * a.lo.element_size()

    def _mx_gemm(self, src, cin, cout):
        return self.mixed_mx and cin % 256 == 0 and cout % 256 == 0 and (src is None or (isinstance(src, Act) and src.mx_ready(cin)))

    @staticmethod
    def _writes_mx(dst, cout, dst_col=0, flags=0):
        if isinstance(dst, Act) and dst.mx is not None and dst_col == 0 and dst.hi.shape[1] == cout:
            dst.mx_valid = True
            return dict(out_mx=dst.mx.data_ptr(), mx_flags=flags | (AVL_MX_OUT_LO if dst.lo_fp4 else 0))
        return dict(mx_flags=flags)

    def _gemm(self, name, src, hw, cin, w, b, dst, dst_col=0, relu=True, res=None, out_f32=False, bias_dev=None,
              read_lo=True, src2=None, w2=None, b2=None, labels=None, bias_per_image=False):
        h, wd = hw
        cout = w.shape[0]
        w_rows = _round_up(cout, 256)
        wp = _zero_pad(w.reshape(cout, cin), w_rows)
        if src2 is not None:
            wp = torch.cat([wp, _zero_pad(w2, w_rows)], dim=1)
            b = b + b2
        in_lo = self._lo(src) if (self.mixed and read_lo) else 0
        use_mx = not out_f32 and self._mx_gemm(src, cin, cout)
        assert src2 is None or use_mx, "%s: a second input needs the MX GEMM" % name
        if use_mx:
            whi, bundle = _cached_pack((self._fp, self.backbone, name, "mx", tuple(wp.shape)), lambda: pack_mx_weights(wp))
            wdev, w_mx = self._dev(whi, torch.float16), self._dev(bundle, torch.uint8)
        elif self.mixed:
            nsub = 3 if in_lo else 2
            wdev = self._dev(_cached_pack((self._fp, self.backbone, name, "split", nsub, tuple(wp.shape)), lambda: pack_split_rows(wp, nsub)), torch.float16)
        else:
            wdev = self._dev(wp, self.act_dtype)
        if bias_dev is None:
            bias_dev = self._dev(_zero_pad(b, w_rows), torch.float32)
        ip, ild, irows = self._view(src)
        op_, old, orows = self._view(dst, dst_col)
        f = dict(in_=ip, out=op_, weight=wdev.data_ptr(), bias=bias_dev.data_ptr(), in_h=h, in_w=wd, in_c=cin, in_ld=ild,
                 in_rows=irows, out_h=h, out_w=wd, out_c=cout, out_ld=old, out_rows=orows, relu=int(relu), out_f32=int(out_f32),
                 w_rows=w_rows, ksize=1, stride=1, dil=1, groups=1)
        if res is not None:
            rp, rld, _ = self._view(res)
            f.update(in2=rp, in2_ld=rld)
        if self.mixed:
            f.update(w_split=1, in_lo=in_lo, out_lo=self._lo(dst, dst_col), in2_lo=self._lo(res))
        if use_mx:
            flags = AVL_MX_IN_LO if (src.lo_fp4 and read_lo) else 0
            f.update(w_split=2, w_mx=w_mx.data_ptr(), in_mx=src.mx.data_ptr())
            if src2 is not None:
                assert src2.mx_ready(w2.shape[1]) and src2.lo_fp4 == src.lo_fp4 and src2.lo is None and src.lo is None
                f.update(in3=src2.hi.data_ptr(), in3_mx=src2.mx.data_ptr(), in3_c=src2.hi.shape[1], in3_ld=src2.hi.shape[1])
            if isinstance(res, Act) and res.lo_fp4:
                f.update(in2_mx=res.mx.data_ptr())
                flags |= AVL_MX_RES_LO
            f.update(self._writes_mx(dst, cout, dst_col, flags))
        else:
            for t_, what in ((src if read_lo else None, "input"), (res, "residual"), (dst, "output")):
                if isinstance(t_, Act) and t_.lo_fp4:
                    raise RuntimeError("%s: the %s keeps its lo part as FP4 only, which needs the MX GEMM" % (name, what))
        if labels is not None:
            assert out_f32 and not use_mx and res is None and not relu
            f["out_mx"] = labels.data_ptr()
        if bias_per_image and self.batch > 1:
            assert not use_mx and bias_dev.shape == (self.batch, w_rows)
            f["bias_per_image"] = 1
        self._op(name, OP_GEMM, **f)

    def _bottleneck(self, st, blk, x, y):
        p, cin, width, cout = blk.p, blk.cin, blk.width, blk.cout
        w1, b1 = fold_bn(st, p + ".conv1.weight", p + ".bn1")
        w2, b2 = fold_bn(st, p + ".conv2.weight", p + ".bn2")
        w3, b3 = fold_bn(st, p + ".conv3.weight", p + ".bn3")
        wd = None
        if blk.has_ds:
            wd, bd = fold_bn(st, p + ".downsample.0.weight", p + ".downsample.1")
            wd, b3 = wd.reshape(cout, cin), b3 + bd
        p1, p2, p3 = (self._dev(t, torch.float16) for t in _cached_pack(
            (self._fp, self.backbone, p, "bottleneck"), lambda: pack_bottleneck(w1.reshape(width, cin), w2, w3.reshape(cout, width), wd, self.groups)))
        bias = self._dev(torch.cat([b1, b2, b3]), torch.float32)
        ip, ild, irows = self._view(x)
        op_, old, orows = self._view(y)
        mx = dict(in_mx=x.mx.data_ptr(), **self._writes_mx(y, cout, flags=AVL_MX_IN_LO)) if x.lo_fp4 else {}
        self._op(p, OP_BOTTLENECK, **mx, in_=ip, in_lo=self._lo(x), out=op_, out_lo=self._lo(y), weight=p1.data_ptr(), in2=p2.data_ptr(), in3=p3.data_ptr(),
                 in3_c=width, bias=bias.data_ptr(), in_h=blk.hw[0], in_w=blk.hw[1], in_c=cin, in_ld=ild, in_rows=irows, out_h=blk.hw[0], out_w=blk.hw[1],
                 out_c=cout, out_ld=old, out_rows=orows, ksize=3, stride=1, pad=1, dil=1, groups=self.groups, relu=1, w_layout=int(wd is not None),
                 w_split=int(wd is not None))

    def _dwpw(self, name, src, hw, cin, w_dw, b_dw, w_pw, b_pw, dst, dst_col, dilation, padding=None, classifier=None):
        h, wd = hw
        padding = dilation if padding is None else padding
        oh, ow = h + 2 * padding - 2 * dilation, wd + 2 * padding - 2 * dilation
        cout = w_pw.shape[0]
        w_rows = _round_up(cout, 256)
        wp = _zero_pad(w_pw.reshape(cout, cin), w_rows)
        wdev = self._dev(pack_split_rows(wp, 2), torch.float16) if self.mixed else self._dev(wp, self.act_dtype)
        bdev = self._dev(_zero_pad(b_pw, w_rows), torch.float32)
        exact = self.mixed and self.mixed_dw_exact
        in_lo = self._lo(src) if exact else 0
        dwp = pack_dw_f32(w_dw, b_dw) if exact else pack_dw_pairs(w_dw, b_dw, self.act_dtype)
        blocks = bool(in_lo) and dilation == 1
        params = torch.cat([dwp, dwpw_block_order(oh, ow) if blocks else dwpw_tile_order(oh, ow, dilation)]).to(self.device)
        self._keep.append(params)
        ip, ild, irows = self._view(src)
        f = dict(in_=ip, in_lo=in_lo, in2=params.data_ptr(), weight=wdev.data_ptr(), bias=bdev.data_ptr(), in_h=h, in_w=wd, in_c=cin, in_ld=ild,
                 in_rows=irows, out_h=oh, out_w=ow, out_c=cout, relu=1, w_rows=w_rows, ksize=3, stride=1, pad=padding, dil=dilation, groups=cin,
                 w_split=(3 if exact else int(self.mixed)), w_layout=int(blocks))
        if classifier is not None:
            wc, bc, logits, labels = classifier
            ncls = wc.shape[0]
            assert in_lo and cout == 256 and ncls <= 32 and wc.shape[1] == cout
            wcd = self._dev(torch.stack(split_f16(_zero_pad(wc, 32))), torch.float16)
            bcd = self._dev(_zero_pad(bc, 32), torch.float32)
            f.update(in2_lo=bcd.data_ptr(), in3=wcd.data_ptr(), in3_c=ncls, out=logits.data_ptr(), out_mx=labels.data_ptr(), out_f32=1, out_ld=ncls,
                     out_rows=logits.shape[0])
        else:
            op_, old, orows = self._view(dst, dst_col)
            f.update(out=op_, out_ld=old, out_rows=orows, out_lo=self._lo(dst, dst_col) if self.mixed else 0)
        self._op(name, OP_DWPW, **f)

    def _spatial(self, name, kind, src, in_hw, cin, dst, out_hw, cout, weight=None, bias=None, **extra):
        ip, ild, irows = self._view(src)
        op_, old, orows = self._view(dst)
        f = dict(in_=ip, out=op_, in_h=in_hw[0], in_w=in_hw[1], in_c=cin, in_ld=ild, in_rows=irows, out_h=out_hw[0],
                 out_w=out_hw[1], out_c=cout, out_ld=old, out_rows=orows)
        if weight is not None:
            f["weight"] = weight.data_ptr()
        if bias is not None:
            f["bias"] = bias.data_ptr()
        f.update(extra)
        self._op(name, kind, **f)

    def _build(self, st):
        x, hw = self._emit_stem(st)
        dilated = (False, False, True, True) if self.output_stride == 8 else (False, False, False, True)
        cin, dilation, low = 64, 1, None
        for li, (planes, nblocks, stride, dilate) in enumerate(zip(PLANES, self.layers, (1, 2, 2, 2), dilated), start=1):
            width = int(planes * (self.width_per_group / 64.0)) * self.groups
            cg = width // self.groups
            assert cg % 64 == 0 or (cg <= 32 and 32 % cg == 0), "%s: %d channels per group" % (self.backbone, cg)
            previous_dilation = dilation
            if dilate:
                dilation, stride = dilation * stride, 1
            for bi in range(nblocks):
                s, d = (stride, previous_dilation) if bi == 0 else (1, dilation)
                p = "backbone.layer%d.%d" % (li, bi)
                ohw = ((hw[0] - 1) // s + 1, (hw[1] - 1) // s + 1)
                trunk_lo = self.mixed_layer1_lo or li != 1 or bi == nblocks - 1
                blk = Block(p, hw, ohw, cin, width, planes * EXPANSION, s, d, (p + ".downsample.0.weight") in st, trunk_lo)
                y = self._emit_block(st, blk, x)
                if x is not low:
                    self._release(x)
                x, hw, cin = y, ohw, blk.cout
            if li == 1:
                low, low_hw, low_c = x, hw, cin
        aspp, aspp_out = self._emit_aspp(st, x, hw, cin)
        self._emit_decoder(st, aspp, hw, aspp_out, low, low_hw, low_c)

    def _emit_stem(self, st):
        H, W = self.H, self.W
        dev = self.device
        f32_in = self.input_format == "f32_nchw"
        shape = (3, H, W) if f32_in else ((H, W, 3) if self.raw_frame is None else self.raw_frame + (3,))
        self.image = torch.zeros(((self.batch,) if self.batch > 1 else ()) + shape, dtype=torch.float32 if f32_in else torch.uint8, device=dev)
        self.zero_page = torch.zeros(64, dtype=torch.uint8, device=dev)
        self.camera_block = torch.zeros(_lib.AVL_STEM_CAMERA_BYTES * (self.batch if self.raw_batch else 1), dtype=torch.uint8, device=dev)
        self._keep += [self.image, self.zero_page, self.camera_block]

        h2, w2 = (H + 6 - 7) // 2 + 1, (W + 6 - 7) // 2 + 1
        w, b = fold_bn(st, "backbone.conv1.weight", "backbone.bn1")
        if self.full_split:
            whi, wlo = split_f16(w)
            w_stem, stem_layout = self._dev(torch.cat([pack_stem_mfma(whi.to(torch.float64)), pack_stem_mfma(wlo.to(torch.float64))]), torch.float16), 1
        elif self.half:
            w_stem, stem_layout = self._dev(pack_stem_mfma(w), self.act_dtype), 1
        else:
            w_stem, stem_layout = self._dev(w.permute(2, 3, 1, 0).reshape(-1), torch.float32), 0
        b_stem = self._dev(b, torch.float32)
        stem = self._act(h2 * w2, 64, split=self.full_split)
        raw = {} if self.raw_frame is None else dict(in2=self.camera_block.data_ptr(), in2_ld=self.raw_frame[1], raw_batch=int(self.raw_batch))
        self._op("backbone.conv1", OP_STEM, in_=self.image.data_ptr(), out=stem.hi.data_ptr(), weight=w_stem.data_ptr(),
                 bias=b_stem.data_ptr(), in_h=H, in_w=W, in_c=3, in_ld=3, in_rows=self.image.numel() // 3, out_h=h2, out_w=w2,
                 out_c=64, out_ld=64, out_rows=stem.shape[0], ksize=7, stride=2, pad=3, dil=1, groups=1, relu=1, w_layout=stem_layout,
                 w_split=int(self.full_split), out_lo=self._lo(stem), in_format=INPUT_FORMATS[self.input_format], **raw)
        h4, w4 = (h2 + 2 - 3) // 2 + 1, (w2 + 2 - 3) // 2 + 1
        x = self._act(h4 * w4, 64, split=self.full_split)
        self._spatial("backbone.maxpool", OP_MAXPOOL, stem, (h2, w2), 64, x, (h4, w4), 64, ksize=3, stride=2, pad=1, dil=1,
                      in_lo=self._lo(stem), out_lo=self._lo(x))
        self._release(stem)
        return x, (h4, w4)

    def _emit_block(self, st, blk, x):
        route = self._fused_route(blk, x)
        if route is None:
            return self._emit_block_unfused(st, blk, x)
        mx = route == "layer2"
        y = self._act(blk.ohw[0] * blk.ohw[1], blk.cout, split=blk.trunk_lo, mx=mx, lo_fp4=mx)
        self._bottleneck(st, blk, x, y)
        return y

    def _fused_route(self, blk, x):
        if not (self.mixed_fuse_block and blk.s == 1 and blk.d == 1 and self.groups == 32 and x.hi.shape[1] == blk.cin):
            return None
        cg = blk.width // self.groups
        if (blk.width == 128 and blk.cout == 256 and blk.cin in (64, 256) and 16 % cg == 0 and blk.has_ds == (blk.cin == 64)
                and (blk.cin == 256 or x.lo is None)):
            return "layer1"
        if blk.width == 256 and blk.cout == 512 and blk.cin == 512 and cg == 8 and not blk.has_ds and x.lo_fp4 and x.mx_ready(blk.cin):
            return "layer2"
        return None

    def _emit_block_unfused(self, st, blk, x):
        p, hw, ohw, cin, width, cout = blk.p, blk.hw, blk.ohw, blk.cin, blk.width, blk.cout
        dense = (width // self.groups) % 64 == 0
        w, b = fold_bn(st, p + ".conv1.weight", p + ".bn1")
        t1_c = _round_up(width, 128) if self.full_split else width
        conv1_mx = self.mixed_gconv_mx and not dense and self._mx_gemm(x, cin, t1_c)
        t1 = self._act(hw[0] * hw[1], t1_c, split=self.full_split, mx=conv1_mx, lo_fp4=conv1_mx)
        self._gemm(p + ".conv1", x, hw, cin, _zero_pad(w, t1_c), _zero_pad(b, t1_c), t1, read_lo=self.mixed_conv1_split)
        wg, bg, conv2 = self._conv2_weights(st, blk, t1, dense)
        t2_fp4 = self.mixed_conv2_split and self.mixed_trunk_fp4 and conv2["w_layout"] == 1 and self._mx_gemm(None, width, cout)
        t2 = self._act(ohw[0] * ohw[1], width, split=self.mixed_conv2_split, mx=not dense, lo_fp4=t2_fp4)
        conv2.update(ksize=3, pad=blk.d, dil=blk.d, groups=self.groups, relu=1, in_lo=self._lo(t1))
        if self.full_split:
            assert conv2["w_layout"] in (1, 2) and conv2["w_split"] == 1 and t1.lo is not None, "full_split needs the MFMA grouped conv with split weights"
        if self.full_split and blk.s != 1 and not dense:
            t2f = self._act(hw[0] * hw[1], width, split=True)
            self._spatial(p + ".conv2", OP_GCONV, t1, hw, width, t2f, hw, width, wg, bg, stride=1, out_lo=self._lo(t2f), **conv2)
            self._spatial(p + ".conv2.sub", OP_SUBSAMPLE, t2f, hw, width, t2, ohw, width, stride=blk.s)
            self._spatial(p + ".conv2.sub[lo]", OP_SUBSAMPLE, t2f.lo, hw, width, t2.lo, ohw, width, stride=blk.s)
            self._release(t2f)
        else:
            conv2.update(self._writes_mx(t2, width, flags=conv2.get("mx_flags", 0)))
            self._spatial(p + ".conv2", OP_GCONV, t1, hw, width, t2, ohw, width, wg, bg, stride=blk.s, out_lo=self._lo(t2), **conv2)
        self._release(t1)
        idn = self._emit_identity(st, blk, x, t2)
        w, b = fold_bn(st, p + ".conv3.weight", p + ".bn3")
        trunk_fp4 = self.mixed_trunk_fp4 and self._mx_gemm(t2, width, cout)
        y = self._act(ohw[0] * ohw[1], cout, split=self.mixed and blk.trunk_lo, mx=True, lo_fp4=trunk_fp4)
        if idn is None:
            wd, bd = fold_bn(st, p + ".downsample.0.weight", p + ".downsample.1")
            self._gemm(p + ".conv3+downsample", t2, ohw, width, w, b, y, relu=True, src2=x, w2=wd.reshape(cout, cin), b2=bd)
        else:
            self._gemm(p + ".conv3", t2, ohw, width, w, b, y, relu=True, res=idn)
        self._release(t2)
        if idn is not x and idn is not None:
            self._release(idn)
        return y

    def _conv2_weights(self, st, blk, t1, dense):
        p, width, groups = blk.p, blk.width, self.groups
        w, b = fold_bn(st, p + ".conv2.weight", p + ".bn2")
        key = (self._fp, self.backbone, p + ".conv2")
        f = dict(w_split=int(self.mixed))
        if dense:
            if self.mixed:
                wg = self._dev(_cached_pack(key + ("dense_split",), lambda: pack_conv3x3(w, groups, 8, split=True)), torch.float16)
            else:
                wg = self._dev(_cached_pack(key + ("dense", self.half), lambda: pack_conv3x3(w, groups, 8 if self.half else 4)), self.act_dtype)
            f["w_layout"] = 2
        elif t1.mx_ready(width):
            frag_hi, bundle = _cached_pack(key + ("gconv_mx",), lambda: pack_gconv_mx(w, groups))
            wg, wb = self._dev(frag_hi.reshape(-1), torch.float16), self._dev(bundle, torch.uint8)
            f.update(w_layout=1, w_split=2, w_mx=wb.data_ptr(), in_mx=t1.mx.data_ptr(), mx_flags=AVL_MX_IN_LO)
        elif self.half and width % 64 == 0:
            if self.mixed:
                nwin = width // 32
                wg = self._dev(torch.cat([pack_gconv_windows(part.to(torch.float64), groups).reshape(nwin, 2, 9, 16, 32) for part in split_f16(w)],
                                         dim=2).reshape(-1), torch.float16)
            else:
                wg = self._dev(pack_gconv_windows(w, groups), self.act_dtype)
            f["w_layout"] = 1
        else:
            cg = width // groups
            wg = self._dev(w.reshape(groups, cg, cg, 3, 3).permute(0, 3, 4, 2, 1).reshape(-1), torch.float32)
            f["w_layout"] = 0
        return wg, self._dev(b, torch.float32), f

    def _emit_identity(self, st, blk, x, t2):
        p, ohw, cin, cout = blk.p, blk.ohw, blk.cin, blk.cout
        if not blk.has_ds:
            return x
        if (blk.s == 1 and self.mixed_fuse_ds and x.lo_fp4 and t2.lo_fp4 and self._mx_gemm(x, cin, cout)
                and self._mx_gemm(t2, blk.width, cout)):
            return None
        w, b = fold_bn(st, p + ".downsample.0.weight", p + ".downsample.1")
        src = x
        if blk.s != 1:
            keep_lo = self.mixed_conv1_split and x.lo is not None
            src = self._act(ohw[0] * ohw[1], cin, split=keep_lo)
            self._spatial(p + ".downsample.sub", OP_SUBSAMPLE, x, blk.hw, cin, src, ohw, cin, stride=blk.s)
            if keep_lo:
                self._spatial(p + ".downsample.sub[lo]", OP_SUBSAMPLE, x.lo, blk.hw, cin, src.lo, ohw, cin, stride=blk.s)
        idn = self._act(ohw[0] * ohw[1], cout, split=self.mixed and blk.trunk_lo)
        self._gemm(p + ".downsample", src, ohw, cin, w, b, idn, relu=False, read_lo=self.mixed_conv1_split)
        if src is not x:
            self._release(src)
        return idn

    def _part_input(self, rows, ch):
        a = self._act(rows, ch, split=self.mixed)

        def put(x):
            m = x.permute(1, 2, 0).reshape(rows, ch).to(torch.float64)
            hi = m.to(self.act_dtype)
            a.hi[:rows].copy_(hi.to(self.device))
            if a.lo is not None:
                a.lo[:rows].copy_((m - hi.to(torch.float64)).to(self.act_dtype).to(self.device))
        return a, put

    def _build_part(self, st):
        H, W = self.H, self.W
        self.zero_page = torch.zeros(64, dtype=torch.uint8, device=self.device)
        self._keep.append(self.zero_page)
        feat, self.set_feature = self._part_input(H * W, self.part[1])
        if self.part[0] == "aspp":
            self.part_out, self.part_out_c = self._emit_aspp(st, feat, (H, W), self.part[1])
            self.out_h, self.out_w = H, W
        else:
            low, self.set_low = self._part_input(4 * H * W, self.part[2])
            self._emit_decoder(st, feat, (H, W), self.part[1], low, (2 * H, 2 * W), self.part[2])

    def part_output(self):
        a, rows = self.part_out, self.out_h * self.out_w
        y = a.hi[:rows, :self.part_out_c].float()
        if a.lo is not None:
            y = y + a.lo[:rows, :self.part_out_c].float()
        return y.reshape(self.out_h, self.out_w, self.part_out_c).permute(2, 0, 1)

    def _emit_aspp(self, st, feat, fhw, fc):
        dev = self.device
        M = fhw[0] * fhw[1]
        dil = (1, 12, 24, 36) if self.output_stride == 8 else (1, 6, 12, 18)
        branches = []
        i = 0
        while ("aspp.module_pyramid.%d.conv.weight" % i) in st or ("aspp.module_pyramid.%d.depthwise_cnn.conv.weight" % i) in st:
            branches.append(i)
            i += 1
        bch = [st["aspp.module_pyramid.0.conv.weight"].shape[0]] + [st["aspp.module_pyramid.%d.pointwise_cnn.conv.weight" % k].shape[0]
                                                                    for k in branches[1:]]
        ncat = sum(bch)
        cat = self._act(M, ncat, split=self.mixed)
        w, b = fold_bn(st, "aspp.module_pyramid.0.conv.weight", "aspp.module_pyramid.0.bn")
        self._gemm("aspp.module_pyramid.0", feat, fhw, fc, w, b, cat, dst_col=0)
        col = bch[0]
        for k in branches[1:]:
            p = "aspp.module_pyramid.%d" % k
            w, b = fold_bn(st, p + ".depthwise_cnn.conv.weight", p + ".depthwise_cnn.bn")
            w2, b2 = fold_bn(st, p + ".pointwise_cnn.conv.weight", p + ".pointwise_cnn.bn")
            if self.half and self.fuse_dwpw and fc % 64 == 0 and fc <= 2048:
                self._dwpw(p, feat, fhw, fc, w, b, w2, b2, cat, col, dil[k])
            else:
                wd_, bd_ = self._dev(w.reshape(fc, 9).t().reshape(-1), torch.float32), self._dev(b, torch.float32)
                t = self._act(M, fc, split=self.mixed)
                self._spatial(p + ".depthwise_cnn", OP_DWCONV, feat, fhw, fc, t, fhw, fc, wd_, bd_, ksize=3, stride=1, pad=dil[k],
                              dil=dil[k], groups=fc, relu=1, in2=self.zero_page.data_ptr(), in_lo=self._lo(feat), out_lo=self._lo(t))
                self._gemm(p + ".pointwise_cnn", t, fhw, fc, w2, b2, cat, dst_col=col)
                self._release(t)
            col += bch[k]
        wg_, bg_ = fold_bn(st, "aspp.global_avg_pool.1.conv.weight", "aspp.global_avg_pool.1.bn")
        wp_, bp_ = fold_bn(st, "aspp.conv.conv.weight", "aspp.conv.bn")
        npool = wg_.shape[0]
        aspp_out = wp_.shape[0]
        wp_ = wp_.reshape(aspp_out, ncat + npool)
        B = self.batch
        bshape = (lambda *s: (B,) + s) if B > 1 else (lambda *s: s)
        gap_partial = torch.zeros(bshape(256, fc), dtype=torch.float32, device=dev)
        gap_vec = torch.zeros(bshape(fc), dtype=torch.float32, device=dev)
        pool_vec = torch.zeros(bshape(npool), dtype=torch.float32, device=dev)
        proj_bias = torch.zeros(bshape(_round_up(aspp_out, 256)), dtype=torch.float32, device=dev)
        self._keep += [gap_partial, gap_vec, pool_vec, proj_bias]
        fp, fld, frows = self._view(feat)
        self._op("aspp.global_avg_pool.0", OP_GAP, in_=fp, in2=gap_partial.data_ptr(), out=gap_vec.data_ptr(), in_h=fhw[0], in_w=fhw[1],
                 in_c=fc, in_ld=fld, in_rows=frows, out_h=1, out_w=1, out_c=fc, out_ld=fc, out_rows=1)
        wgd, bgd = self._dev(wg_.reshape(npool, fc), torch.float32), self._dev(bg_, torch.float32)
        self._op("aspp.global_avg_pool.1", OP_GEMV, dtype=_lib.AVL_F32, in_=gap_vec.data_ptr(), out=pool_vec.data_ptr(), weight=wgd.data_ptr(),
                 bias=bgd.data_ptr(), in_h=1, in_w=1, in_c=fc, in_ld=fc, in_rows=1, out_h=1, out_w=1, out_c=npool, out_ld=npool,
                 out_rows=1, relu=1)
        wpd, bpd = self._dev(wp_[:, ncat:], torch.float32), self._dev(bp_, torch.float32)
        self._op("aspp.conv[pool slice]", OP_GEMV, dtype=_lib.AVL_F32, in_=pool_vec.data_ptr(), out=proj_bias.data_ptr(), weight=wpd.data_ptr(),
                 bias=bpd.data_ptr(), in_h=1, in_w=1, in_c=npool, in_ld=npool, in_rows=1, out_h=1, out_w=1, out_c=aspp_out,
                 out_ld=proj_bias.shape[-1] if B > 1 else aspp_out, out_rows=1, relu=0)
        aspp = self._act(M, aspp_out, split=self.mixed)
        self._gemm("aspp.conv", cat, fhw, ncat, wp_[:, :ncat], None, aspp, bias_dev=proj_bias, bias_per_image=True)
        self._release(cat)
        self._release(feat)
        return aspp, aspp_out

    def _emit_decoder(self, st, aspp, fhw, aspp_out, low, low_hw, low_c):
        w, b = fold_bn(st, "decoder.low_level_conv.conv.weight", "decoder.low_level_conv.bn")
        low_out = _round_up(w.shape[0], 128 if self.mixed else 64)
        cat2 = self._act(low_hw[0] * low_hw[1], aspp_out + low_out, split=self.mixed)
        self._gemm("decoder.low_level_conv", low, low_hw, low_c, _zero_pad(w, low_out), _zero_pad(b, low_out), cat2, dst_col=aspp_out)
        self._spatial("decoder.interpolate", OP_BILINEAR, aspp, fhw, aspp_out, cat2, low_hw, aspp_out, in_lo=self._lo(aspp), out_lo=self._lo(cat2))
        self._release(aspp)
        self._release(low)
        x, hw, cin = cat2, low_hw, aspp_out + low_out
        k = 0
        while ("decoder.refine_layers.%d.depthwise_cnn.conv.weight" % k) in st:
            p = "decoder.refine_layers.%d" % k
            w, b = fold_bn(st, p + ".depthwise_cnn.conv.weight", p + ".depthwise_cnn.bn")
            ks = w.shape[-1]
            ohw = (hw[0] - (ks - 1), hw[1] - (ks - 1))
            w2, b2 = fold_bn(st, p + ".pointwise_cnn.conv.weight", p + ".pointwise_cnn.bn")
            if k == 0:
                w, b, w2 = _zero_pad(w, cin), _zero_pad(b, cin), _zero_pad(w2, cin, dim=1)
            cout = w2.shape[0]
            fused = (ks == 3 and self.half and self.fuse_dwpw and cin % 64 == 0 and cin <= 2048
                     and (not self.mixed or (self.mixed_fuse_decoder and self.mixed_dw_exact)))
            last = ("decoder.refine_layers.%d.depthwise_cnn.conv.weight" % (k + 1)) not in st
            if fused and last and self.mixed_fuse_classifier and x.lo is not None and cout == 256 and self.num_classes <= 32:
                wc, bc = fold_bn(st, "decoder.refine_layers.%d.conv.weight" % (k + 1), None)
                self._outputs(ohw)
                self._dwpw(p + "+classifier", x, hw, cin, w, b, w2, b2, None, 0, 1, padding=0,
                           classifier=(wc.reshape(self.num_classes, cout), bc, self.logits_buf, self.labels_buf))
                self._release(x)
                return
            y = self._act(ohw[0] * ohw[1], cout, split=self.mixed)
            if fused:
                self._dwpw(p, x, hw, cin, w, b, w2, b2, y, 0, 1, padding=0)
                self._release(x)
            else:
                wd_, bd_ = self._dev(w.reshape(cin, ks * ks).t().reshape(-1), torch.float32), self._dev(b, torch.float32)
                t_fp4 = ks == 3 and self.mixed_trunk_fp4 and x.lo is not None and self._mx_gemm(None, cin, cout)
                t = self._act(ohw[0] * ohw[1], cin, split=self.mixed, mx=t_fp4, lo_fp4=t_fp4)
                self._spatial(p + ".depthwise_cnn", OP_DWCONV, x, hw, cin, t, ohw, cin, wd_, bd_, ksize=ks, stride=1, pad=0, dil=1, groups=cin, relu=1,
                              in2=self.zero_page.data_ptr() if ks == 3 else 0, in_lo=self._lo(x), out_lo=self._lo(t), **self._writes_mx(t, cin))
                self._release(x)
                self._gemm(p + ".pointwise_cnn", t, ohw, cin, w2, b2, y)
                self._release(t)
            x, hw, cin = y, ohw, cout
            k += 1
        w, b = fold_bn(st, "decoder.refine_layers.%d.conv.weight" % k, None)
        self._outputs(hw)
        self._gemm("decoder.refine_layers.%d" % k, x, hw, cin, w, b, Act(self.logits_buf), relu=False, out_f32=True,
                   labels=self.labels_buf if self.num_classes <= 32 else None)
        if self.num_classes > 32:
            self._op("argmax", OP_ARGMAX, dtype=_lib.AVL_F32, in_=self.logits_buf.data_ptr(), out=self.labels_buf.data_ptr(), in_h=hw[0], in_w=hw[1],
                     in_c=self.num_classes, in_ld=self.num_classes, in_rows=self.logits_buf.shape[0], out_h=hw[0], out_w=hw[1], out_c=1,
                     out_ld=1, out_rows=self.labels_buf.shape[0])

    def _outputs(self, hw):
        self.out_h, self.out_w = hw
        rows = _round_up(hw[0] * hw[1] * self.batch, self.ROW_PAD)
        self.logits_buf = torch.zeros((rows, self.num_classes), dtype=torch.float32, device=self.device)
        self.labels_buf = torch.zeros(rows, dtype=torch.uint8, device=self.device)
        self._keep += [self.logits_buf, self.labels_buf]

    @property
    def labels(self):
        n = self.out_h * self.out_w
        if self.batch > 1:
            return self.labels_buf[:self.batch * n].view(self.batch, self.out_h, self.out_w)
        return self.labels_buf[:n].view(self.out_h, self.out_w)

    @property
    def logits(self):
        n = self.out_h * self.out_w
        if self.batch > 1:
            return self.logits_buf[:self.batch * n].view(self.batch, self.out_h, self.out_w, self.num_classes)
        return self.logits_buf[:n].view(self.out_h, self.out_w, self.num_classes)

    def set_camera(self, K=None, dist=None, stream=None, image=None):
        assert self.raw_frame is not None, "set_camera needs a plan built with raw_frame"
        assert (K is None) == (dist is None)
        blocks = self.camera_block.numel() // _lib.AVL_STEM_CAMERA_BYTES
        if image is None:
            which = range(blocks)
        else:
            if not 0 <= int(image) < blocks:
                raise IndexError("set_camera: image %d of a plan with %d camera block(s)" % (image, blocks))
            which = (int(image),)
        k = d = None
        if K is not None:
            k = (C.c_double * 9)(*np.asarray(K, dtype=np.float64).ravel().tolist())
            d = (C.c_double * 5)(*np.asarray(dist, dtype=np.float64).ravel()[:5].tolist())
        s = torch.cuda.current_stream(self.device).cuda_stream if stream is None else stream
        for n in which:
            _lib.check(_lib.lib().avl_stem_camera_set(C.c_void_p(self.camera_block.data_ptr() + n * _lib.AVL_STEM_CAMERA_BYTES), k, d, C.c_void_p(s)),
                       "avl_stem_camera_set")

    def forward(self, image_u8=None, stream=None):
        if image_u8 is not None:
            assert self.part is None, "a sub-plan takes its inputs through set_feature / set_low"
            if not isinstance(image_u8, torch.Tensor):
                image_u8 = torch.from_numpy(np.ascontiguousarray(image_u8))
            if self.input_format == "f32_nchw":
                if tuple(image_u8.shape) != tuple(self.image.shape) or not image_u8.dtype.is_floating_point:
                    raise ValueError("this plan takes a float tensor of shape %s, not %s %s" % (tuple(self.image.shape), image_u8.dtype,
                                                                                               tuple(image_u8.shape)))
            else:
                if self.raw_batch and self.batch == 1 and image_u8.dim() == 4:
                    image_u8 = image_u8[0]
                assert tuple(image_u8.shape) == tuple(self.image.shape) and image_u8.dtype == torch.uint8
            self.image.copy_(image_u8, non_blocking=True)
        s = torch.cuda.current_stream(self.device).cuda_stream if stream is None else stream
        _lib.check(_lib.lib().avl_seg_plan_run(self._plan, C.c_void_p(s)), "avl_seg_plan_run")
        return self.labels if hasattr(self, "labels_buf") else None

    def capture_graph(self):
        side = torch.cuda.Stream(device=self.device)
        side.wait_stream(torch.cuda.current_stream(self.device))
        with torch.cuda.stream(side):
            _lib.check(_lib.lib().avl_seg_plan_run(self._plan, C.c_void_p(side.cuda_stream)), "avl_seg_plan_run")
            side.synchronize()
            _lib.check(_lib.lib().avl_seg_plan_capture(self._plan, C.c_void_p(side.cuda_stream)), "avl_seg_plan_capture")
        torch.cuda.current_stream(self.device).wait_stream(side)
        self.graphed = True

    def profile(self):
        n = len(self.ops)
        ms, fl, by = (C.c_float * n)(), (C.c_double * n)(), (C.c_double * n)()
        s = torch.cuda.current_stream(self.device).cuda_stream
        _lib.check(_lib.lib().avl_seg_plan_profile(self._plan, C.c_void_p(s), ms, fl, by), "avl_seg_plan_profile")
        return [dict(name=self.op_names[i], kind=OP_NAMES[self.ops[i].kind], ms=ms[i], flops=fl[i], bytes=by[i]) for i in range(n)]

    def op_output(self, i):
        op = self.ops[i]
        rows, cols = op.out_h * op.out_w * self.batch, (op.in3_c if (op.kind == OP_DWPW and op.out_f32) else op.out_c)
        dt = torch.float32 if (op.out_f32 or op.dtype == _lib.AVL_F32) else self.act_dtype

        def plane(ptr):
            for t in self._keep + ([self.logits_buf] if hasattr(self, "logits_buf") else []):
                lo, hi = t.data_ptr(), t.data_ptr() + t.numel() * t.element_size()
                if lo <= ptr < hi:
                    flat = t.reshape(-1).view(torch.uint8)[ptr - lo:].view(dt)
                    return torch.as_strided(flat, (rows, cols), (op.out_ld, 1)).float().cpu()
            raise KeyError("op %d: output pointer not in the plan's buffers" % i)
        y = plane(op.out)
        return y + plane(op.out_lo) if op.out_lo else y

    def run_prefix(self, n_ops, stream=None):
        plan = C.c_void_p()
        arr = (AvlSegOp * n_ops)(*self.ops[:n_ops])
        _lib.check(_lib.lib().avl_seg_plan_create(arr, n_ops, C.byref(plan)), "avl_seg_plan_create")
        try:
            s = torch.cuda.current_stream(self.device).cuda_stream if stream is None else stream
            _lib.check(_lib.lib().avl_seg_plan_run(plan, C.c_void_p(s)), "avl_seg_plan_run")
            torch.cuda.synchronize(self.device)
        finally:
            _lib.lib().avl_seg_plan_destroy(plan)

    def nonfinite_counts(self):
        n = len(self.ops)
        cnt = (C.c_ulonglong * n)()
        s = torch.cuda.current_stream(self.device).cuda_stream
        _lib.check(_lib.lib().avl_seg_plan_nonfinite(self._plan, C.c_void_p(s), cnt), "avl_seg_plan_nonfinite")
        return {self.op_names[i]: int(cnt[i]) for i in range(n) if cnt[i]}

    def total_flops(self):
        n = len(self.ops)
        return sum(r["flops"] for r in self.profile()) if n else 0.0
```

Baseline: 222.7.

## Fuse strided downsample into GEMM via row gather and plane-form second input

```diff
diff --git a/include/avl_hip.h b/include/avl_hip.h
--- a/include/avl_hip.h
+++ b/include/avl_hip.h
@@ -173,6 +173,9 @@
     int32_t bias_per_image;
     int32_t in_format;
     int32_t raw_batch;
+    const void* in3_lo;
+    int32_t in3_rows;
+    int32_t gather_stride, gather_h, gather_w;
 } avl_seg_op;
 
 #define AVL_IN_U8_HWC 0
diff --git a/vision_semantic_segmentation_amd/csrc/seg_gemm.hip b/vision_semantic_segmentation_amd/csrc/seg_gemm.hip
--- a/vision_semantic_segmentation_amd/csrc/seg_gemm.hip
+++ b/vision_semantic_segmentation_amd/csrc/seg_gemm.hip
@@ -23,6 +23,16 @@
     void* C_lo;
 };
 
+struct GatherArgs {
+    int s, ow, ohw, iw, ihw;
+};
+__device__ __forceinline__ long long gather_row(const GatherArgs& ga, int m, int M) {
+    m = m < M ? m : M - 1;
+    const int b = m / ga.ohw, rem = m - b * ga.ohw;
+    const int y = rem / ga.ow, x = rem - y * ga.ow;
+    return (long long)b * ga.ihw + (long long)(ga.s * y) * ga.iw + ga.s * x;
+}
+
 template <int NSUB> __device__ __forceinline__ bool sub_needs_a(int j) { return NSUB == 1 || j == 0 || (NSUB == 3 && j == 2); }
 
 __device__ __forceinline__ void glds16(const void* g, void* l) {
@@ -210,8 +220,8 @@
     }
 }
 
-template <typename H, int WM, int WN, int MI, int STAGES, int NSUB = 1, int IO = 0, int AST = STAGES>
-__global__ void __launch_bounds__(WM* WN * 64) k_gemm_ring(GemmArgs p, int mtiles) {
+template <typename H, int WM, int WN, int MI, int STAGES, int NSUB = 1, int IO = 0, int AST = STAGES, bool GATHER = false>
+__global__ void __launch_bounds__(WM* WN * 64) k_gemm_ring(GemmArgs p, int mtiles, GatherArgs ga) {
     typedef typename Half16<H>::v8 v8;
     constexpr int NW = WM * WN, BM = WM * MI * 16, BN = WN * 64;
     constexpr int A_BYTES = BM * 128, W_BYTES = BN * 128;
@@ -243,7 +253,8 @@
 #pragma unroll
         for (int i = 0; i < A_INSTR; ++i) {
             const int r = (i * NW + wave) * 8 + srow;
-            a_src[i] = static_cast<const char*>(p.A) + (long long)(mt * BM + r) * p.lda * 2 + ((schunk ^ (r & 7)) << 4);
+            const long long row = GATHER ? gather_row(ga, mt * BM + r, p.M) : (long long)(mt * BM + r);
+            a_src[i] = static_cast<const char*>(p.A) + row * p.lda * 2 + ((schunk ^ (r & 7)) << 4);
         }
 #pragma unroll
         for (int i = 0; i < W_INSTR; ++i) {
@@ -444,18 +455,18 @@
     }
 }
 
-template <typename H, int WM, int WN, int MI, int STAGES, int NSUB = 1, int IO = 0, int AST = STAGES>
-int launch_ring(const GemmArgs& a0, int M, hipStream_t s) {
+template <typename H, int WM, int WN, int MI, int STAGES, int NSUB = 1, int IO = 0, int AST = STAGES, bool GATHER = false>
+int launch_ring(const GemmArgs& a0, int M, const GatherArgs& ga, hipStream_t s) {
     constexpr int BM = WM * MI * 16, BN = WN * 64, LDS = (AST * BM + STAGES * BN) * 128;
     static_assert(LDS <= 160 * 1024, "ring does not fit LDS");
-    AVL_HIP_CHECK(hipFuncSetAttribute(reinterpret_cast<const void*>(&k_gemm_ring<H, WM, WN, MI, STAGES, NSUB, IO, AST>),
+    AVL_HIP_CHECK(hipFuncSetAttribute(reinterpret_cast<const void*>(&k_gemm_ring<H, WM, WN, MI, STAGES, NSUB, IO, AST, GATHER>),
                                       hipFuncAttributeMaxDynamicSharedMemorySize, LDS));
     GemmArgs a = a0;
     a.ntiles = (a.N + BN - 1) / BN;
     const int mtiles = (M + BM - 1) / BM;
     const int total = mtiles * a.ntiles;
     const int grid = total < 256 ? total : 256;
-    hipLaunchKernelGGL((k_gemm_ring<H, WM, WN, MI, STAGES, NSUB, IO, AST>), dim3(grid), dim3(WM * WN * 64), LDS, s, a, mtiles);
+    hipLaunchKernelGGL((k_gemm_ring<H, WM, WN, MI, STAGES, NSUB, IO, AST, GATHER>), dim3(grid), dim3(WM * WN * 64), LDS, s, a, mtiles, ga);
     AVL_LAUNCH_CHECK();
     return AVL_OK;
 }
@@ -494,6 +505,9 @@
     const char* As2[2];
     long long a_srows2;
     int stagger;
+    const void* A2lo;
+    int ldw16, ldwq;
+    GatherArgs ga;
 };
 
 template <int IO, int MI>
@@ -605,7 +619,7 @@
     }
 }
 
-template <int IO, int MI>
+template <int IO, int MI, bool A2P = false>
 __global__ void __launch_bounds__(512) k_gemm_ring_mx(MxArgs q, int mtiles) {
     typedef f16 H;
     typedef typename Half16<H>::v8 v8;
@@ -642,20 +656,45 @@
     for (int i = 0; i < W_INSTR; ++i) {
         const int r = (i * NW + wave) * 8 + srow;
         const int key = ((r >> 1) & 1) | (((r >> 4) & 3) << 1);
-        w_off16[i] = (unsigned)r * (unsigned)(p.K * 2) + ((schunk ^ key) << 4);
-        w_offq[i] = (unsigned)r * (unsigned)(p.K / 2) + ((schunk ^ key) << 4);
+        w_off16[i] = (unsigned)r * (unsigned)(A2P ? q.ldw16 : p.K * 2) + ((schunk ^ key) << 4);
+        w_offq[i] = (unsigned)r * (unsigned)(A2P ? q.ldwq : p.K / 2) + ((schunk ^ key) << 4);
     }
     int pt = vb, pmb = 0, pj = 0, issued = 0;
+    unsigned a2_off[A2P ? A_INSTR : 1];
+    int a2_mt = -1;
     auto issue = [&]() {
         const int nt = pt % p.ntiles, mt = pt / p.ntiles;
         const unsigned abase = lds_base + (issued % STAGES) * A_BYTES + wave * 1024;
         const unsigned wbase = lds_base + W_REGION + (issued % STAGES) * W_BYTES + wave * 1024;
         const bool second = pmb >= q.nmb1;
         const int mbl = second ? pmb - q.nmb1 : pmb;
+        if constexpr (A2P) {
+            if (second) {
+                if (a2_mt != mt) {
+                    a2_mt = mt;
+#pragma unroll
+                    for (int i = 0; i < A_INSTR; ++i)
+                        a2_off[i] = (unsigned)gather_row(q.ga, mt * BM + (i * NW + wave) * 8 + srow, p.M) * (unsigned)(q.lda2 * 2) + ct;
+                }
+                const int kb = mbl * 4 + pj / 3, pass = pj % 3;
+                const char* sa = static_cast<const char*>(pass == 2 ? q.A2lo : q.A2) + (long long)kb * 128;
+                const char* sw = static_cast<const char*>(p.W) + (long long)nt * BN * q.ldw16 + (long long)(q.nmb1 * 4 + mbl * 12 + pj) * 128;
+#pragma unroll
+                for (int i = 0; i < A_INSTR; ++i) glds16_saddr(sa, a2_off[i], abase + i * NW * 1024);
+#pragma unroll
+                for (int i = 0; i < W_INSTR; ++i) glds16_saddr(sw, w_off16[i], wbase + i * NW * 1024);
+                ++issued;
+                if (++pj == 12) {
+                    pj = 0;
+                    if (++pmb == nmb) { pmb = 0; pt += nwg; }
+                }
+                return;
+            }
+        }
         if (pj < 4) {
             const long long rowb = second ? (long long)q.lda2 * 2 : (long long)p.lda * 2;
             const char* sa = static_cast<const char*>(second ? q.A2 : p.A) + ((long long)mt * BM + wave * 8) * rowb + (long long)(mbl * 4 + pj) * 128;
-            const char* sw = static_cast<const char*>(p.W) + (long long)nt * BN * p.K * 2 + (long long)(pmb * 4 + pj) * 128;
+            const char* sw = static_cast<const char*>(p.W) + (A2P ? (long long)nt * BN * q.ldw16 : (long long)nt * BN * p.K * 2) + (long long)(pmb * 4 + pj) * 128;
             const unsigned al = second ? a_lane16_2 : a_lane16;
 #pragma unroll
             for (int i = 0; i < A_INSTR; ++i) glds16_saddr(sa + (long long)i * (NW * 8) * rowb, al, abase + i * NW * 1024);
@@ -665,7 +704,7 @@
             const int t = pj - 4;
             const long long rowb = second ? q.ldaq2 : q.ldaq;
             const char* sa = (second ? q.Aq2[t] : q.Aq[t]) + ((long long)mt * BM + wave * 8) * rowb + (long long)mbl * 128;
-            const char* sw = q.Wq[t] + (long long)nt * BN * (p.K / 2) + (long long)pmb * 128;
+            const char* sw = q.Wq[t] + (A2P ? (long long)nt * BN * q.ldwq : (long long)nt * BN * (p.K / 2)) + (long long)pmb * 128;
             const unsigned al = second ? a_laneq_2 : a_laneq;
 #pragma unroll
             for (int i = 0; i < A_INSTR; ++i) glds16_saddr(sa + (long long)i * (NW * 8) * rowb, al, abase + i * NW * 1024);
@@ -715,7 +754,11 @@
     for (int t = vb; t < total; t += nwg) {
         const int nt = t % p.ntiles, mt = t / p.ntiles;
         for (int mb = 0; mb < nmb; ++mb) {
-            for (int j = 0; j < 4; ++j, ++g) {
+            int nf16 = 4, nfp4 = q.nmx;
+            if constexpr (A2P) {
+                if (mb >= q.nmb1) { nf16 = 12; nfp4 = 0; }
+            }
+            for (int j = 0; j < nf16; ++j, ++g) {
                 asm volatile("s_waitcnt vmcnt(0)" ::: "memory");
                 __builtin_amdgcn_s_barrier();
                 const char* abase = lds + (g % STAGES) * A_BYTES + a_row0 * 128;
@@ -737,7 +780,7 @@
                     }
                 }
             }
-            for (int u = 0; u < q.nmx; ++u, ++g) {
+            for (int u = 0; u < nfp4; ++u, ++g) {
                 asm volatile("s_waitcnt vmcnt(0)" ::: "memory");
                 __builtin_amdgcn_s_barrier();
                 const char* abase = lds + (g % STAGES) * A_BYTES + a_row0 * 128;
@@ -1038,7 +1081,7 @@
     }
 }
 
-template <int IO, int MI>
+template <int IO, int MI, bool A2P = false>
 int launch_ring_mx_t(const MxArgs& a0, hipStream_t s) {
     constexpr int BM = 2 * MI * 16, LDS = 2 * (BM + 256) * 128 + 2 * 4096;
     MxArgs a = a0;
@@ -1047,13 +1090,13 @@
     const int mtiles = (a.g.M + BM - 1) / BM;
     const int total = mtiles * a.g.ntiles;
     const int grid = total < 256 ? total : 256;
-    if (a.g.K >= 1024) {
+    if (!A2P && a.g.K >= 1024) {
         constexpr int LATE = MI == 8 ? 0 : 1;
         AVL_HIP_CHECK(hipFuncSetAttribute(reinterpret_cast<const void*>(&k_gemm_mx_pipe<IO, MI, LATE>), hipFuncAttributeMaxDynamicSharedMemorySize, LDS));
         hipLaunchKernelGGL((k_gemm_mx_pipe<IO, MI, LATE>), dim3(grid), dim3(512), LDS, s, a, mtiles);
     } else {
-        AVL_HIP_CHECK(hipFuncSetAttribute(reinterpret_cast<const void*>(&k_gemm_ring_mx<IO, MI>), hipFuncAttributeMaxDynamicSharedMemorySize, LDS));
-        hipLaunchKernelGGL((k_gemm_ring_mx<IO, MI>), dim3(grid), dim3(512), LDS, s, a, mtiles);
+        AVL_HIP_CHECK(hipFuncSetAttribute(reinterpret_cast<const void*>(&k_gemm_ring_mx<IO, MI, A2P>), hipFuncAttributeMaxDynamicSharedMemorySize, LDS));
+        hipLaunchKernelGGL((k_gemm_ring_mx<IO, MI, A2P>), dim3(grid), dim3(512), LDS, s, a, mtiles);
     }
     AVL_LAUNCH_CHECK();
     return AVL_OK;
@@ -1062,6 +1105,10 @@
 int launch_ring_mx(const MxArgs& a, int m_image, bool quantize_out, hipStream_t s) {
     const long long t256 = (long long)((m_image + 255) / 256) * (a.g.N / 256);
     const bool small = t256 < 192 || (t256 > 256 && t256 < 384);
+    if (a.A2lo) {
+        if (small) return quantize_out ? launch_ring_mx_t<1, 4, true>(a, s) : launch_ring_mx_t<0, 4, true>(a, s);
+        return quantize_out ? launch_ring_mx_t<1, 8, true>(a, s) : launch_ring_mx_t<0, 8, true>(a, s);
+    }
     if (small) return quantize_out ? launch_ring_mx_t<1, 4>(a, s) : launch_ring_mx_t<0, 4>(a, s);
     return quantize_out ? launch_ring_mx_t<1, 8>(a, s) : launch_ring_mx_t<0, 8>(a, s);
 }
@@ -1075,6 +1122,25 @@
 inline TileCfg pick_tile(const avl_seg_op& op) {
     if (op.out_c <= 64) return {256, 64};
     return {128, 128};
+}
+
+template <bool G>
+int launch_ring_variant(const avl_seg_op& op, const GemmArgs& a, int m_image, const GatherArgs& ga, hipStream_t s) {
+    const bool can256 = a.N % 256 == 0 && op.w_rows % 256 == 0;
+    int v = op.w_layout;
+    if (v == 0) v = (can256 && ((m_image + 255) / 256) * (a.N / 256) >= 192) ? 3 : 2;
+    if (a.nsub == 2) {
+        if (v == 3 && can256) return launch_ring<f16, 2, 4, 8, 3, 2, 1, 2, G>(a, a.M, ga, s);
+        return launch_ring<f16, 4, 2, 4, 3, 2, 1, 3, G>(a, a.M, ga, s);
+    }
+    if (a.nsub == 3) {
+        if (v == 3 && can256) return launch_ring<f16, 2, 4, 8, 2, 3, 1, 2, G>(a, a.M, ga, s);
+        return launch_ring<f16, 4, 2, 4, 3, 3, 1, 3, G>(a, a.M, ga, s);
+    }
+    const bool bf = op.dtype == AVL_BF16;
+    if (v == 3 && can256) return bf ? launch_ring<bf16, 2, 4, 8, 2, 1, 0, 2, G>(a, a.M, ga, s) : launch_ring<f16, 2, 4, 8, 2, 1, 0, 2, G>(a, a.M, ga, s);
+    if (v == 4) return bf ? launch_ring<bf16, 2, 2, 8, 3, 1, 0, 3, G>(a, a.M, ga, s) : launch_ring<f16, 2, 2, 8, 3, 1, 0, 3, G>(a, a.M, ga, s);
+    return bf ? launch_ring<bf16, 4, 2, 4, 3, 1, 0, 3, G>(a, a.M, ga, s) : launch_ring<f16, 4, 2, 4, 3, 1, 0, 3, G>(a, a.M, ga, s);
 }
 
 }
@@ -1107,6 +1173,7 @@
     AVL_REQUIRE(op.w_layout == 0 || is_half(op.dtype), "GEMM w_layout %d forces a tile configuration of the 16-bit kernels: dtype %d", op.w_layout, op.dtype);
     if (op.bias_per_image && op_batch(op) > 1) {
         AVL_REQUIRE(op.w_split != 2 && !op.in3, "GEMM: a per-image bias is not supported by the MX GEMM");
+        AVL_REQUIRE(op.gather_stride < 2, "GEMM: a per-image bias together with a row gather");
         for (int n = 0; n < op.batch; ++n) {
             const avl_seg_op v = gemm_image_op(op, n);
             AVL_REQUIRE(v.in_rows >= (op.out_h * op.out_w + 255) / 256 * 256,
@@ -1118,6 +1185,19 @@
     }
     const int M = op.out_h * op.out_w * op_batch(op), K = op.in_c, N = op.out_c;
     AVL_REQUIRE(M > 0 && N > 0 && K > 0, "GEMM M/N/K = %d/%d/%d", M, N, K);
+    AVL_REQUIRE(op.gather_stride >= 0, "GEMM gather_stride %d", op.gather_stride);
+    if (op.gather_stride >= 2) {
+        const int gs = op.gather_stride;
+        AVL_REQUIRE(op.gather_h > 0 && op.gather_w > 0 && op.out_h == (op.gather_h - 1) / gs + 1 && op.out_w == (op.gather_w - 1) / gs + 1,
+                    "GEMM row gather: a %d x %d map at stride %d is not the %d x %d output", op.gather_h, op.gather_w, gs, op.out_h, op.out_w);
+        AVL_REQUIRE((long long)op_batch(op) * op.gather_h * op.gather_w < (1LL << 31), "GEMM row gather: more than 2^31 source rows");
+        if (op.w_split != 2) {
+            if (!ring_eligible(op))
+                return set_error(AVL_E_UNSUPPORTED, "GEMM row gather needs a 16-bit ring GEMM (16-bit output, out_c %d %% 128 == 0)", N);
+            AVL_REQUIRE((long long)op.in_rows >= (long long)op_batch(op) * op.gather_h * op.gather_w,
+                        "GEMM row gather reads %lld rows, input has %d allocated", (long long)op_batch(op) * op.gather_h * op.gather_w, op.in_rows);
+        }
+    }
     AVL_REQUIRE(op.in_h * op.in_w == op.out_h * op.out_w, "GEMM in/out pixel counts differ (%d vs %d)", op.in_h * op.in_w, op.out_h * op.out_w);
     AVL_REQUIRE((K * es) % 128 == 0, "GEMM K = %d is not a multiple of %d", K, 128 / es);
     AVL_REQUIRE(op.in_ld >= K && (op.in_ld * es) % 16 == 0, "GEMM in_ld %d", op.in_ld);
@@ -1143,11 +1223,23 @@
                     "AVL_MX_RES_LO needs in2, in2_mx (bundle of a dense [out_rows][N] residual) and no in2_lo");
         AVL_REQUIRE(!(op.mx_flags & AVL_MX_OUT_LO) || op.out_mx, "AVL_MX_OUT_LO without out_mx");
         AVL_REQUIRE(!(op.mx_flags & AVL_MX_IN_LO) || !op.in_lo, "AVL_MX_IN_LO together with in_lo");
-        if (op.in3) {
+        AVL_REQUIRE(!op.in3_lo || op.in3, "in3_lo without in3");
+        if (op.in3 && op.in3_lo) {
+            AVL_REQUIRE(!op.in3_mx && op.in3_c > 0 && op.in3_c % 256 == 0 && op.in3_ld >= op.in3_c && (op.in3_ld * 2) % 16 == 0,
+                        "second GEMM input as planes: no in3_mx, in3_c %d (multiple of 256), in3_ld %d", op.in3_c, op.in3_ld);
+            AVL_REQUIRE((reinterpret_cast<uintptr_t>(op.in3) | reinterpret_cast<uintptr_t>(op.in3_lo)) % 16 == 0, "second GEMM input must be 16-byte aligned");
+            const long long need = op.gather_stride >= 2 ? (long long)op_batch(op) * op.gather_h * op.gather_w : (long long)M;
+            AVL_REQUIRE(op.in3_rows >= need, "second GEMM input as planes: %lld rows are read, in3_rows %d", need, op.in3_rows);
+            AVL_REQUIRE((long long)op.in3_rows * op.in3_ld * 2 < 0xffffff00LL && (long long)op.w_rows * (K + 3LL * op.in3_c) * 2 < 0xffffff00LL,
+                        "MX GEMM operand larger than 4 GB");
+        } else if (op.in3) {
+            AVL_REQUIRE(op.gather_stride < 2, "the strided row gather of a second GEMM input needs its plane form (in3_lo)");
             AVL_REQUIRE(op.in3_mx && op.in3_c > 0 && op.in3_c % 256 == 0 && op.in3_ld == op.in3_c,
                         "second GEMM input: in3_mx, in3_c %d (multiple of 256), dense rows (in3_ld %d)", op.in3_c, op.in3_ld);
             AVL_REQUIRE(!op.in_lo || (op.mx_flags & AVL_MX_IN_LO), "a second GEMM input needs both inputs' lo parts in their bundles (AVL_MX_IN_LO) or none");
             AVL_REQUIRE((reinterpret_cast<uintptr_t>(op.in3) | reinterpret_cast<uintptr_t>(op.in3_mx)) % 16 == 0, "second GEMM input must be 16-byte aligned");
+        } else {
+            AVL_REQUIRE(op.gather_stride < 2, "the MX GEMM gathers the rows of a second input only (in3 + in3_lo)");
         }
         AVL_REQUIRE((long long)op.in_rows * K * 2 < 0xffffff00LL && (long long)op.w_rows * K * 2 < 0xffffff00LL, "MX GEMM operand larger than 4 GB");
         AVL_REQUIRE((long long)op.out_rows * op.out_ld * 2 < (1LL << 31) && (!op.in2 || (long long)op.out_rows * op.in2_ld * 2 < (1LL << 31)) &&
@@ -1204,11 +1296,20 @@
             a.K = (int)(K1 + K2);
             mx.g.K = a.K;
             mx.A2 = op.in3; mx.lda2 = op.in3_ld; mx.ldaq2 = (int)(K2 / 2);
-            abundle(op.in3_mx, op.in_rows, K2, mx.Aq2, mx.As2);
-            mx.a_srows2 = op.in_rows;
-        }
+            if (op.in3_lo) {
+                mx.A2lo = op.in3_lo;
+                const bool gs = op.gather_stride >= 2;
+                mx.ga = GatherArgs{gs ? op.gather_stride : 1, op.out_w, op.out_h * op.out_w, gs ? op.gather_w : op.out_w,
+                                   gs ? op.gather_h * op.gather_w : op.out_h * op.out_w};
+            } else {
+                abundle(op.in3_mx, op.in_rows, K2, mx.Aq2, mx.As2);
+                mx.a_srows2 = op.in_rows;
+            }
+        }
+        mx.ldw16 = (int)((K1 + (op.in3_lo ? 3 : 1) * K2) * 2);
+        mx.ldwq = (int)((op.in3_lo ? K1 : K1 + K2) / 2);
         {
-            const long long KT = K1 + K2;
+            const long long KT = op.in3_lo ? K1 : K1 + K2;
             const char* b = static_cast<const char*>(op.w_mx);
             const long long P = (long long)op.w_rows * (KT / 2), S = (KT / 256) * op.w_rows * 8;
             mx.Wq[0] = b; mx.Ws[0] = b + P; mx.Wq[1] = b + P + S; mx.Ws[1] = b + 2 * P + S;
@@ -1242,22 +1343,11 @@
     const int mtiles = (a.M + t.bm - 1) / t.bm;
     a.ntiles = (a.N + t.bn - 1) / t.bn;
     if (ring_eligible(op)) {
-        const bool can256 = a.N % 256 == 0 && op.w_rows % 256 == 0;
-        int v = op.w_layout;
-        if (v == 0) v = (can256 && ((m_image + 255) / 256) * (a.N / 256) >= 192) ? 3 : 2;
-        if (a.nsub == 2) {
-            if (v == 3 && can256) return launch_ring<f16, 2, 4, 8, 3, 2, 1, 2>(a, a.M, s);
-            return launch_ring<f16, 4, 2, 4, 3, 2, 1>(a, a.M, s);
-        }
-        if (a.nsub == 3) {
-            if (v == 3 && can256) return launch_ring<f16, 2, 4, 8, 2, 3, 1>(a, a.M, s);
-            return launch_ring<f16, 4, 2, 4, 3, 3, 1>(a, a.M, s);
-        }
-        const bool bf = op.dtype == AVL_BF16;
-        if (v == 3 && can256) return bf ? launch_ring<bf16, 2, 4, 8, 2>(a, a.M, s) : launch_ring<f16, 2, 4, 8, 2>(a, a.M, s);
-        if (v == 4) return bf ? launch_ring<bf16, 2, 2, 8, 3>(a, a.M, s) : launch_ring<f16, 2, 2, 8, 3>(a, a.M, s);
-        return bf ? launch_ring<bf16, 4, 2, 4, 3>(a, a.M, s) : launch_ring<f16, 4, 2, 4, 3>(a, a.M, s);
-    }
+        if (op.gather_stride >= 2)
+            return launch_ring_variant<true>(op, a, m_image, GatherArgs{op.gather_stride, op.out_w, op.out_h * op.out_w, op.gather_w, op.gather_h * op.gather_w}, s);
+        return launch_ring_variant<false>(op, a, m_image, GatherArgs{}, s);
+    }
+    AVL_REQUIRE(op.gather_stride < 2, "GEMM: the strided row gather needs a ring GEMM");
     if (op.dtype == AVL_BF16) {
         if (t.bn == 64) return launch_cfg<bf16, 4, 1>(a, mtiles, s);
         return launch_cfg<bf16, 2, 2>(a, mtiles, s);
diff --git a/vision_semantic_segmentation_amd/csrc/seg_plan.hip b/vision_semantic_segmentation_amd/csrc/seg_plan.hip
--- a/vision_semantic_segmentation_amd/csrc/seg_plan.hip
+++ b/vision_semantic_segmentation_amd/csrc/seg_plan.hip
@@ -67,7 +67,7 @@
                 const double k_all = op.in_c + (op.in3 ? op.in3_c : 0);
                 const double e_w = op.w_split == 2 ? es + 2.0 * (0.5 + 1.0 / 32.0) : es * (op.w_split ? 2.0 : 1.0);
                 const double e_res = act_bytes(es, op.in2_lo != nullptr, (op.mx_flags & AVL_MX_RES_LO) != 0, false);
-                bytes += (double)op.out_c * k_all * e_w + (op.in2 ? out_pix * op.out_c * e_res : 0.0) + (op.in3 ? in_pix * op.in3_c * e_in : 0.0);
+                bytes += (double)op.out_c * k_all * e_w + (op.in2 ? out_pix * op.out_c * e_res : 0.0) + (op.in3 ? in_pix * op.in3_c * (op.in3_lo ? 2.0 * es : e_in) : 0.0);
             }
             if (op.out_f32) {
                 bytes += out_pix * op.out_c * (4 - es);
diff --git a/vision_semantic_segmentation_amd/network.py b/vision_semantic_segmentation_amd/network.py
--- a/vision_semantic_segmentation_amd/network.py
+++ b/vision_semantic_segmentation_amd/network.py
@@ -30,6 +30,8 @@
         ("batch", C.c_int32), ("bias_per_image", C.c_int32),
         ("in_format", C.c_int32),
         ("raw_batch", C.c_int32),
+        ("in3_lo", C.c_void_p), ("in3_rows", C.c_int32),
+        ("gather_stride", C.c_int32), ("gather_h", C.c_int32), ("gather_w", C.c_int32),
     ]
 
 
@@ -484,7 +486,7 @@
 class SegNet(object):
 
     ROW_PAD = 256
-    MIXED_OPTS = ("conv1_split", "conv2_split", "mx", "trunk_fp4", "fuse_ds", "gconv_mx", "dw_exact", "layer1_lo", "fuse_block", "full_split", "fuse_decoder", "fuse_classifier")
+    MIXED_OPTS = ("conv1_split", "conv2_split", "mx", "trunk_fp4", "fuse_ds", "fuse_ds_strided", "gconv_mx", "dw_exact", "layer1_lo", "fuse_block", "full_split", "fuse_decoder", "fuse_classifier")
 
     def __init__(self, state, height, width, precision="bf16", device=None, num_classes=19, output_stride=8, fuse_dwpw=True, raw_frame=None,
                  part=None, backbone=DEFAULT_BACKBONE, batch=1, input_format="u8_hwc", raw_batch=False, **mixed_opts):
@@ -531,6 +533,7 @@
         self.mixed_mx = self.mixed and mixed_opts.get("mx", True)
         self.mixed_trunk_fp4 = mixed_opts.get("trunk_fp4", True)
         self.mixed_fuse_ds = mixed_opts.get("fuse_ds", True)
+        self.mixed_fuse_ds_strided = mixed_opts.get("fuse_ds_strided", True)
         self.mixed_fuse_classifier = mixed_opts.get("fuse_classifier", True)
         self.mixed_fuse_decoder = mixed_opts.get("fuse_decoder", True)
         self.mixed_dw_exact = mixed_opts.get("dw_exact", True)
@@ -646,18 +649,27 @@
         return dict(mx_flags=flags)
 
     def _gemm(self, name, src, hw, cin, w, b, dst, dst_col=0, relu=True, res=None, out_f32=False, bias_dev=None,
-              read_lo=True, src2=None, w2=None, b2=None, labels=None, bias_per_image=False):
+              read_lo=True, src2=None, w2=None, b2=None, labels=None, bias_per_image=False, gather=None):
         h, wd = hw
         cout = w.shape[0]
         w_rows = _round_up(cout, 256)
         wp = _zero_pad(w.reshape(cout, cin), w_rows)
+        planes2 = src2 is not None and src2.lo is not None
         if src2 is not None:
-            wp = torch.cat([wp, _zero_pad(w2, w_rows)], dim=1)
+            if not planes2:
+                wp = torch.cat([wp, _zero_pad(w2, w_rows)], dim=1)
             b = b + b2
         in_lo = self._lo(src) if (self.mixed and read_lo) else 0
-        use_mx = not out_f32 and self._mx_gemm(src, cin, cout)
+        use_mx = not out_f32 and self._mx_gemm(src, cin, cout) and (gather is None or planes2)
         assert src2 is None or use_mx, "%s: a second input needs the MX GEMM" % name
-        if use_mx:
+        assert gather is None or planes2 or src2 is None, "%s: only a plane-form second input is gathered" % name
+        if use_mx and planes2:
+            def pack_planes():
+                hi, bun = pack_mx_weights(wp)
+                return torch.cat([hi, pack_split_rows(_zero_pad(w2, w_rows), 3)], dim=1).contiguous(), bun
+            whi, bundle = _cached_pack((self._fp, self.backbone, name, "mx+planes", tuple(wp.shape), tuple(w2.shape)), pack_planes)
+            wdev, w_mx = self._dev(whi, torch.float16), self._dev(bundle, torch.uint8)
+        elif use_mx:
             whi, bundle = _cached_pack((self._fp, self.backbone, name, "mx", tuple(wp.shape)), lambda: pack_mx_weights(wp))
             wdev, w_mx = self._dev(whi, torch.float16), self._dev(bundle, torch.uint8)
         elif self.mixed:
@@ -675,12 +687,17 @@
         if res is not None:
             rp, rld, _ = self._view(res)
             f.update(in2=rp, in2_ld=rld)
+        if gather is not None:
+            f.update(gather_stride=gather[0], gather_h=gather[1][0], gather_w=gather[1][1])
         if self.mixed:
             f.update(w_split=1, in_lo=in_lo, out_lo=self._lo(dst, dst_col), in2_lo=self._lo(res))
         if use_mx:
             flags = AVL_MX_IN_LO if (src.lo_fp4 and read_lo) else 0
             f.update(w_split=2, w_mx=w_mx.data_ptr(), in_mx=src.mx.data_ptr())
-            if src2 is not None:
+            if planes2:
+                assert src2.lo is not None and src2.hi.shape[1] == w2.shape[1] and w2.shape[1] % 256 == 0
+                f.update(in3=src2.hi.data_ptr(), in3_lo=src2.lo.data_ptr(), in3_c=src2.hi.shape[1], in3_ld=src2.hi.shape[1], in3_rows=src2.hi.shape[0])
+            elif src2 is not None:
                 assert src2.mx_ready(w2.shape[1]) and src2.lo_fp4 == src.lo_fp4 and src2.lo is None and src.lo is None
                 f.update(in3=src2.hi.data_ptr(), in3_mx=src2.mx.data_ptr(), in3_c=src2.hi.shape[1], in3_ld=src2.hi.shape[1])
             if isinstance(res, Act) and res.lo_fp4:
@@ -872,7 +889,8 @@
         y = self._act(ohw[0] * ohw[1], cout, split=self.mixed and blk.trunk_lo, mx=True, lo_fp4=trunk_fp4)
         if idn is None:
             wd, bd = fold_bn(st, p + ".downsample.0.weight", p + ".downsample.1")
-            self._gemm(p + ".conv3+downsample", t2, ohw, width, w, b, y, relu=True, src2=x, w2=wd.reshape(cout, cin), b2=bd)
+            self._gemm(p + ".conv3+downsample", t2, ohw, width, w, b, y, relu=True, src2=x, w2=wd.reshape(cout, cin), b2=bd,
+                       gather=(blk.s, blk.hw) if blk.s != 1 else None)
         else:
             self._gemm(p + ".conv3", t2, ohw, width, w, b, y, relu=True, res=idn)
         self._release(t2)
@@ -916,8 +934,16 @@
         if (blk.s == 1 and self.mixed_fuse_ds and x.lo_fp4 and t2.lo_fp4 and self._mx_gemm(x, cin, cout)
                 and self._mx_gemm(t2, blk.width, cout)):
             return None
+        if (blk.s != 1 and self.mixed_fuse_ds and self.mixed_fuse_ds_strided and self.mixed_conv1_split and x.lo is not None
+                and t2.lo_fp4 and x.hi.shape[1] == cin and self.mixed_mx and cin % 256 == 0 and self._mx_gemm(t2, blk.width, cout)):
+            return None
         w, b = fold_bn(st, p + ".downsample.0.weight", p + ".downsample.1")
         src = x
+        if blk.s != 1 and self.half and cout % 128 == 0 and x.hi.shape[1] == cin:
+            idn = self._act(ohw[0] * ohw[1], cout, split=self.mixed and blk.trunk_lo)
+            self._gemm(p + ".downsample", x, ohw, cin, w, b, idn, relu=False, read_lo=self.mixed_conv1_split and x.lo is not None,
+                       gather=(blk.s, blk.hw))
+            return idn
         if blk.s != 1:
             keep_lo = self.mixed_conv1_split and x.lo is not None
             src = self._act(ohw[0] * ohw[1], cin, split=keep_lo)
```

Result: no change. 223.7 (median of 5 runs) (+0.5%).
